# GianniLunardi/VBOC

Hardware: AMD Instinct MI355X
Metric: VBOC boundary OCP solves/sec, triple pendulum, 1/2/4/8 MI355X (higher is better)
Workload: dtype f64

## Files before the change

vboc_amd/csrc/coop.h:

```cpp
#pragma once

#ifndef VBOC_NSF
#define VBOC_NSF 4
#endif
#ifndef VBOC_DF
#define VBOC_DF 2
#endif
#ifndef VBOC_NSV
#define VBOC_NSV 8
#endif
#ifndef VBOC_DV
#define VBOC_DV 6
#endif

namespace vboc {

typedef double dbl2 __attribute__((ext_vector_type(2)));
typedef double dbl4 __attribute__((ext_vector_type(4)));
typedef __attribute__((address_space(1))) dbl2 gdbl2;
typedef __attribute__((address_space(1))) void gvoid;
typedef __attribute__((address_space(3))) void lvoid;

__host__ __device__ constexpr int even_up(int v) { return (v + 1) & ~1; }
#ifndef VBOC_REC_ALIGN
#define VBOC_REC_ALIGN 2
#endif
__host__ __device__ constexpr int rec_up(int v) { return (v + VBOC_REC_ALIGN - 1) / VBOC_REC_ALIGN * VBOC_REC_ALIGN; }

template <int NQ>
struct WaveLayout {
  static constexpr int NX = 2 * NQ, NU = NQ, NZ = 3 * NQ, M0 = NQ + 1;
  static constexpr bool IN_FIRST = NQ <= 3;
  static constexpr int OA = 0, OB = OA + NX * NX, P0 = OB + NX * NU, OE = IN_FIRST ? P0 : P0 + 4 * NZ, OD = OE + NX,
                       ODA = OD + NZ, OZ = IN_FIRST ? ODA + NZ : P0, ODZ = OZ + NZ, OQL = ODZ + NZ, OQU = OQL + NZ,
                       OK = P0 + 6 * NZ + NX, OKF = OK + NU * NX,
                       OLR = IN_FIRST ? OKF + NU + NU * NQ : OKF + NU, OM = IN_FIRST ? OKF + NU : OLR + NU * NU,
                       OY = OKF + NU + NU * NU + NU * NQ, OPE = OY + NU * NQ, OC = OPE + NX,
                       OACL = OC + NX, OX = OACL + NX * NX, OU = OX + NX, OPI = OU + NU, OLL = OPI + NX,
                       OLU = OLL + NZ, OWPI = OLU + NZ, REC = rec_up(OWPI + NX);
  static_assert((IN_FIRST ? OQU : ODA) + NZ == OK, "the fields before K are A, B, e, D, DA, z, dz, lambda_l, lambda_u");
  static_assert(IN_FIRST ? (OM == OKF + NU && OLR == OM + NU * NQ && OY == OLR + NU * NU)
                         : (OLR == OKF + NU && OM == OLR + NU * NU && OY == OM + NU * NQ), "K, k_f, M / chol(Ru), Y");
  static constexpr int W_FAC = OC, W_FIN = even_up(ODA), W_FINV = even_up(ODA + NZ), LO_VEC = OPE, W_VEC = OX - OPE,
                       LO_FWD = OC, W_FWD = OX - OC, W_COS = even_up(OQU + NZ);
  static constexpr int P_FAC = (W_FAC + 127) / 128, P_VEC = (W_VEC + 127) / 128, P_FWD = (W_FWD + 127) / 128,
                       P_COS = (W_COS + 127) / 128;
  static constexpr int P_VMAX = P_VEC > P_FWD ? (P_VEC > P_COS ? P_VEC : P_COS) : (P_FWD > P_COS ? P_FWD : P_COS);
  static constexpr int RSF = NQ <= 3 ? 256 : 128 * P_FAC, NSF = VBOC_NSF, DF = VBOC_DF,
                       RSV = NQ <= 3 ? 128 : 128 * P_VMAX, NSV = VBOC_NSV, DV = VBOC_DV;
  static constexpr int RING_D = NSF * RSF > NSV * RSV ? NSF * RSF : NSV * RSV;
  static constexpr int S_CAP = 4;
  static constexpr int S_VEC = NQ <= 3 ? (64 / (W_VEC / 2) < S_CAP ? 64 / (W_VEC / 2) : S_CAP) : 1,
                       S_FWD = NQ <= 3 ? (64 / (W_FWD / 2) < S_CAP ? 64 / (W_FWD / 2) : S_CAP) : 1, SLACK = S_CAP;
  static_assert(NQ > 3 || (S_VEC * W_VEC <= RSV && S_FWD * W_FWD <= RSV && (NSV & (NSV - 1)) == 0),
                "grouped windows fit one ring slot");
  static_assert(OB % 2 == 0 && OZ % 2 == 0 && OD % 2 == 0 && OK % 2 == 0 && OPE % 2 == 0 && OC % 2 == 0 &&
                    OACL % 2 == 0 && OX % 2 == 0,
                "16-byte aligned field ranges");
  static_assert(W_FAC <= RSF && W_VEC <= RSV && W_FWD <= RSV && W_COS <= RSV, "ring windows fit their slots");
  static_assert(NSF >= DF + 2 && NSV >= DV + 2, "a slot is refilled >= 2 stages after its last read");
  static constexpr int RING = 0, F0 = RING + RING_D, LR0 = F0 + NX * M0, MM0 = LR0 + M0 * M0, Y0 = MM0 + M0 * NQ,
                       PE0 = Y0 + M0 * NQ, P = PE0 + NX, PA = P + NX * NX, PB = PA + NX * NX, APA = PB + NX * NU,
                       RU = APA + NX * NX, S = RU + NU * NU, PI = S + NU * NX, PV = PI + NX * NQ, DXV = PV + 2 * NX,
                       SC = DXV + 2 * NX, LINE = SC + NQ * NQ, ZERO = LINE + NQ, TRASH = ZERO + 16, PAR = TRASH + 64,
                       XS = even_up(PAR + Par<NQ>::COUNT);
  static_assert(M0 * NX <= NX * NX, "stage-0 B'P reuses the PA scratch");
  static constexpr size_t lds_bytes(int nmax) { return ((size_t)XS + (size_t)(nmax + 1) * NX) * sizeof(double); }
  static constexpr size_t region_doubles(int nmax) { return (size_t)REC * (nmax + 1 + SLACK); }
};

struct Dsc {
  int x1, sx1, y1, sy1, x2, sx2, y2, sy2, ini, d1, d2;
  unsigned rel;
  double sg;
};
enum : unsigned { RX1 = 1, RY1 = 2, RX2 = 4, RY2 = 8, RINI = 16, RD1 = 32, RD2 = 64 };

__device__ __forceinline__ double uni(double v) {
  const unsigned long long b = (unsigned long long)__double_as_longlong(v);
  const unsigned lo = __builtin_amdgcn_readfirstlane((unsigned)b);
  const unsigned hi = __builtin_amdgcn_readfirstlane((unsigned)(b >> 32));
  return __longlong_as_double((long long)(((unsigned long long)hi << 32) | lo));
}
__device__ __forceinline__ void vreg(double& v) { asm volatile("" : "+v"(v)); }
__device__ __forceinline__ double rdlane(double v, int lane) {
  const unsigned long long b = (unsigned long long)__double_as_longlong(v);
  const unsigned lo = __builtin_amdgcn_readlane((unsigned)b, lane);
  const unsigned hi = __builtin_amdgcn_readlane((unsigned)(b >> 32), lane);
  return __longlong_as_double((long long)(((unsigned long long)hi << 32) | lo));
}
__device__ __forceinline__ double dbl_of(unsigned hi, unsigned lo) {
  return __longlong_as_double((long long)(((unsigned long long)hi << 32) | lo));
}
template <bool P32>
__device__ __forceinline__ void wswap(double v, double& a, double& b) {
  const unsigned long long u = (unsigned long long)__double_as_longlong(v);
  const unsigned l = (unsigned)u, h = (unsigned)(u >> 32);
  if constexpr (P32) {
    const auto lo = __builtin_amdgcn_permlane32_swap(l, l, false, false);
    const auto hi = __builtin_amdgcn_permlane32_swap(h, h, false, false);
    a = dbl_of(hi[0], lo[0]); b = dbl_of(hi[1], lo[1]);
  } else {
    const auto lo = __builtin_amdgcn_permlane16_swap(l, l, false, false);
    const auto hi = __builtin_amdgcn_permlane16_swap(h, h, false, false);
    a = dbl_of(hi[0], lo[0]); b = dbl_of(hi[1], lo[1]);
  }
}
template <int CTRL>
__device__ __forceinline__ double dppd(double v) {
  const unsigned long long u = (unsigned long long)__double_as_longlong(v);
  const int l = __builtin_amdgcn_update_dpp(0, (int)(unsigned)u, CTRL, 0xF, 0xF, false);
  const int h = __builtin_amdgcn_update_dpp(0, (int)(unsigned)(u >> 32), CTRL, 0xF, 0xF, false);
  return dbl_of((unsigned)h, (unsigned)l);
}
template <class OP>
__device__ __forceinline__ double wred(double v, OP op) {
  double a, b;
  wswap<true>(v, a, b);
  v = op(a, b);
  wswap<false>(v, a, b);
  v = op(a, b);
  v = op(v, dppd<0x128>(v));
  v = op(v, dppd<0x124>(v));
  v = op(v, dppd<0x4E>(v));
  v = op(v, dppd<0xB1>(v));
  return uni(v);
}
__device__ __forceinline__ double wsum(double v) {
  return wred(v, [](double x, double y) { return x + y; });
}
__device__ __forceinline__ double wmaxd(double v) {
  return wred(v, [](double x, double y) { return fmax(x, y); });
}
__device__ __forceinline__ double wmind(double v) {
  return wred(v, [](double x, double y) { return fmin(x, y); });
}

__device__ __forceinline__ void lsync() {
  __builtin_amdgcn_fence(__ATOMIC_RELEASE, "wavefront");
  __builtin_amdgcn_wave_barrier();
  __builtin_amdgcn_fence(__ATOMIC_ACQUIRE, "wavefront");
}

template <int n>
__device__ __forceinline__ bool chol_inv(double (&A)[n * n], double (&id)[n]) {
  bool ok = true;
  UNR for (int j = 0; j < n; ++j) {
    double sj = A[j * n + j];
    UNR for (int k = 0; k < j; ++k) sj -= A[j * n + k] * A[j * n + k];
    ok = ok && (sj > 0.0);
    const double x = sj > 0.0 ? sj : 1.0;
    double r = __builtin_amdgcn_rsq(x);
    UNR for (int it = 0; it < 2; ++it) {
      const double e = fma(-(0.5 * x) * r, r, 0.5);
      r = fma(r, e, r);
    }
    A[j * n + j] = x * r;
    id[j] = r;
    UNR for (int i = j + 1; i < n; ++i) {
      double tt = A[i * n + j];
      UNR for (int k = 0; k < j; ++k) tt -= A[i * n + k] * A[j * n + k];
      A[i * n + j] = tt * r;
    }
  }
  return ok;
}
template <int n>
__device__ __forceinline__ void solve_inv(const double (&L)[n * n], const double (&id)[n], double (&b)[n]) {
  UNR for (int i = 0; i < n; ++i) {
    double tt = b[i];
    UNR for (int k = 0; k < i; ++k) tt -= L[i * n + k] * b[k];
    b[i] = tt * id[i];
  }
  UNR for (int i = n - 1; i >= 0; --i) {
    double tt = b[i];
    UNR for (int k = i + 1; k < n; ++k) tt -= L[k * n + i] * b[k];
    b[i] = tt * id[i];
  }
}

__device__ __forceinline__ void tri(int u, int& i, int& j) {
  i = 0;
  while ((i + 1) * (i + 2) / 2 <= u) ++i;
  j = u - i * (i + 1) / 2;
}

__device__ unsigned long long g_wave_prof[16];
#ifdef VBOC_COOP_PROF
#define CPROF_DECL unsigned long long cp0 = 0, cp1 = 0, cp2 = 0, cp3 = 0, cp4 = 0, cp5 = 0, cp6 = 0, cp7 = 0, cp8 = 0; \
  unsigned long long cp_t = __builtin_amdgcn_s_memtime();
#define CPROF(i) { const unsigned long long n_ = __builtin_amdgcn_s_memtime(); cp##i += n_ - cp_t; cp_t = n_; }
#define CPROF_FLUSH(sq, ip) if (t == 0) { atomicAdd(&g_wave_prof[0], cp0); atomicAdd(&g_wave_prof[1], cp1); \
  atomicAdd(&g_wave_prof[2], cp2); atomicAdd(&g_wave_prof[3], cp3); atomicAdd(&g_wave_prof[4], cp4); \
  atomicAdd(&g_wave_prof[5], cp5); atomicAdd(&g_wave_prof[6], cp6); atomicAdd(&g_wave_prof[7], cp7); \
  atomicAdd(&g_wave_prof[8], cp8); atomicAdd(&g_wave_prof[9], (unsigned long long)(sq)); \
  atomicAdd(&g_wave_prof[10], (unsigned long long)(ip)); }
#else
#define CPROF_DECL
#define CPROF(i)
#define CPROF_FLUSH(sq, ip)
#endif
#if defined(VBOC_COOP_PROF) && defined(VBOC_PROF_SPLIT)
#define SPROF_DECL(P) unsigned long long sp0 = 0, sp1 = 0, sp2 = 0, sp3 = 0, sp4 = 0, sp_t = 0; \
  constexpr bool sp_on = (VBOC_PROF_SPLIT == (P)); if (sp_on) sp_t = __builtin_amdgcn_s_memtime();
#define SPROF(i) if (sp_on) { const unsigned long long n_ = __builtin_amdgcn_s_memtime(); sp##i += n_ - sp_t; sp_t = n_; }
#define SPROF_FLUSH if (sp_on && t == 0) { atomicAdd(&g_wave_prof[11], sp0); atomicAdd(&g_wave_prof[12], sp1); \
  atomicAdd(&g_wave_prof[13], sp2); atomicAdd(&g_wave_prof[14], sp3); atomicAdd(&g_wave_prof[15], sp4); }
#else
#define SPROF_DECL(P)
#define SPROF(i)
#define SPROF_FLUSH
#endif
#ifndef VBOC_REPEAT
#define VBOC_REPEAT 0
#endif

#define VREP(id, stmt) do { stmt; if constexpr (VBOC_REPEAT == (id)) { stmt; } } while (0)

#ifndef VBOC_FUSE
#define VBOC_FUSE 31
#endif

template <int NQ, bool FM = false, bool HC = false>
struct Coop {
  using L = WaveLayout<NQ>;
  using HL = Lane<NQ>;
  static_assert(!HC || (!FM && NQ >= 2 && NQ <= 3), "path constraint: pendulum chains, VALU factorisation");
  using PF = Par<NQ>;
  static constexpr int NX = 2 * NQ, NU = NQ, NZ = 3 * NQ, M0 = NQ + 1, REC = L::REC;
  static constexpr bool FUSE_OK = FM && NQ <= 3 && !HC;
  static constexpr bool FAC1 = FUSE_OK && (VBOC_FUSE & 1), PFUSE = FUSE_OK && (VBOC_FUSE & 2),
                        CCORR = FUSE_OK && (VBOC_FUSE & 4), KFM = FUSE_OK && (VBOC_FUSE & 8);
  static constexpr int OA = L::OA, OB = L::OB, OZ = L::OZ, ODZ = L::ODZ, OQL = L::OQL, OQU = L::OQU,
                       OE = L::OE, OK = L::OK, OKF = L::OKF, OLR = L::OLR, OM = L::OM, OY = L::OY,
                       OPE = L::OPE, OD = L::OD, ODA = L::ODA, OC = L::OC, OACL = L::OACL, OX = L::OX, OU = L::OU,
                       OPI = L::OPI,
                       OLL = L::OLL, OLU = L::OLU, OWPI = L::OWPI;

  double* s;
  gdouble* g;
  const Work& w;
  const Opts& o;
  int t;
  int N;
  double rs, rd0, e00, mu, nbox;

  unsigned lds0;
  gdouble* gh = nullptr;
  int pause_at = -1;

  __device__ Coop(double* s_, gdouble* g_, const Work& w_, const Opts& o_, int t_)
      : s(s_), g(g_), w(w_), o(o_), t(t_), N(0),
        lds0((unsigned)__builtin_amdgcn_readfirstlane((int)(unsigned)(size_t)(lvoid*)s_)) {}

  __device__ __forceinline__ void fresh() { asm volatile("" : "+v"(t)); }

  __device__ __forceinline__ gdouble& st(int k, int off) const { return g[(long long)k * REC + off]; }
  __device__ __forceinline__ gdouble& hcr(int k, int f) const { return gh[(long long)k * HL::FHC + f]; }
  __device__ __forceinline__ bool hc_on(int k) const { return HC && k >= 1 && k < N; }
  __device__ __forceinline__ double hc_eval(const double* x, double* grad) const {
    constexpr double l = Chain<NQ>::l;
    double X = 0.0, Y = 0.0;
    UNR for (int j = 0; j < NQ; ++j) { X += l * sin(x[j]); Y += l * cos(x[j]); }
    const double dx = X - o.hxc, dy = Y - o.hyc;
    if (grad) {
      UNR for (int j = 0; j < NQ; ++j) grad[j] = 2.0 * dx * (l * cos(x[j])) - 2.0 * dy * (l * sin(x[j]));
    }
    return dx * dx + dy * dy;
  }
  template <bool CORR>
  __device__ __forceinline__ void hc_dir(int k, const double* d, double smu, double& dtl, double& dtu, double& dql,
                                         double& dqu) const {
    double cd = 0.0;
    UNR for (int j = 0; j < NQ; ++j) cd += hcr(k, HL::HG + j) * d[j];
    const double htl = hcr(k, HL::HTL), htu = hcr(k, HL::HTU), hql = hcr(k, HL::HQL), hqu = hcr(k, HL::HQU);
    const double rl = rs * hcr(k, HL::HR0L), ru = rs * hcr(k, HL::HR0U);
    const double rcl = CORR ? smu - htl * hql - hcr(k, HL::HATL) * hcr(k, HL::HAQL) : -htl * hql;
    const double rcu = CORR ? smu - htu * hqu - hcr(k, HL::HATU) * hcr(k, HL::HAQU) : -htu * hqu;
    dtl = cd + rl;
    dtu = ru - cd;
    dql = (rcl - hql * dtl) / htl;
    dqu = (rcu - hqu * dtu) / htu;
  }
  __device__ __forceinline__ double& par(int f) const { return s[L::PAR + f]; }
  __device__ __forceinline__ static constexpr int fslot(int slot) { return L::RING + slot * L::RSF; }
  __device__ __forceinline__ static constexpr int vslot(int slot) { return L::RING + slot * L::RSV; }

  template <int TAG>
  __device__ __forceinline__ void dma(int k, int lo, int W, int dst, int part) const {
    const int nc = W / 2;
    const int c = part * 64 + t < nc ? part * 64 + t : nc - 1;
    const gdouble* src = g + (long long)k * REC + lo + 2 * c;
    const unsigned lds = lds0 + 8u * (unsigned)(dst + part * 128);
    unsigned keep;
    asm volatile("s_mov_b32 %0, m0\n\ts_mov_b32 m0, %2\n\ts_nop 0\n\tglobal_load_lds_dwordx4 %1, off\n\ts_mov_b32 m0, %0"
                 : "=&s"(keep)
                 : "v"(src), "s"(lds)
                 : "memory");
  }
  __device__ __forceinline__ void dma_s(const gdouble* base, unsigned voff, int dst) const {
    const unsigned lds = lds0 + 8u * (unsigned)dst;
    const unsigned long long b = (unsigned long long)(size_t)base;
    const unsigned long long bs = ((unsigned long long)(unsigned)__builtin_amdgcn_readfirstlane((int)(unsigned)(b >> 32)) << 32) |
                                  (unsigned)__builtin_amdgcn_readfirstlane((int)(unsigned)b);
    unsigned keep;
    asm volatile("s_mov_b32 %0, m0\n\ts_mov_b32 m0, %3\n\ts_nop 4\n\tglobal_load_lds_dwordx4 %1, %2\n\t"
                 "s_mov_b32 m0, %0"
                 : "=&s"(keep)
                 : "v"(voff), "s"(bs), "s"(lds)
                 : "memory");
  }
  template <int LO, int W, int S>
  __device__ __forceinline__ unsigned grp_off() const {
    constexpr int CH = W / 2;
    const int u = t / CH < S ? t / CH : S - 1;
    const int c = t - u * CH < CH ? t - u * CH : CH - 1;
    return 8u * (unsigned)(u * REC + LO + 2 * c);
  }
  template <int N>
  __device__ __forceinline__ static void vmwait() {
    asm volatile("s_waitcnt vmcnt(%0)" ::"n"(N) : "memory");
  }
  __device__ __forceinline__ static void settle() {
    __builtin_amdgcn_s_waitcnt(0x0F70);
  }
  template <int LO, int HI>
  __device__ __forceinline__ void ring_wb(int slot, int k) const {
    static_assert((HI - LO) / 2 <= 64 && LO % 2 == 0, "one 16-B chunk per lane");
    const dbl2* src = (const dbl2*)(s + fslot(slot));
    gdbl2* dst = (gdbl2*)(g + (long long)k * REC);
    if constexpr (NQ <= 3) {
      constexpr int NCH = (HI - LO) / 2;
      const int c = t < NCH ? t : NCH - 1;
      dst[LO / 2 + c] = src[LO / 2 + c];
      return;
    }
    if (t < (HI - LO) / 2) dst[LO / 2 + t] = src[LO / 2 + t];
  }


  __device__ __forceinline__ bool box(int k, int i, double& lb, double& ub) const {
    lb = -1.0; ub = 1.0;
    if (k == 0) {
      if (i == 0) { lb = par(PF::SLB); ub = par(PF::SUB); return true; }
      if (i < M0) { lb = par(PF::ULB + i - 1); ub = par(PF::UUB + i - 1); return true; }
      return false;
    }
    if (k == N) {
      if (i < NQ) { lb = par(PF::QNLB + i); ub = par(PF::QNUB + i); return true; }
      return false;
    }
    if (i < NX) { lb = par(PF::XLB + i); ub = par(PF::XUB + i); }
    else { lb = par(PF::ULB + i - NX); ub = par(PF::UUB + i - NX); }
    return true;
  }
  __device__ __forceinline__ double dz_init(double lb, double ub, double z) const {
    const double Lo = lb - z, U = ub - z, del = o.push * (U - Lo);
    return fmin(fmax(0.0, Lo + del), U - del);
  }
  __device__ __forceinline__ double cgrad(int k, int i) const { return (k == 0 && i == 0) ? par(PF::CS) : 0.0; }

  template <int LO, int C>
  __device__ __forceinline__ void ldr(int k, double (&d)[2 * C]) const {
    static_assert(LO % 2 == 0, "16-byte aligned range");
    const gdbl2* src = (const gdbl2*)(g + (long long)k * REC + LO);
    UNR for (int c = 0; c < C; ++c) {
      const dbl2 v = src[c];
      d[2 * c] = v.x;
      d[2 * c + 1] = v.y;
    }
  }
  static constexpr int NIP = (4 * NZ + 1) / 2;
  struct IP { double v[2 * NIP]; };
  __device__ __forceinline__ void ld_ip(int k, IP& r) const { ldr<OZ, NIP>(k, r.v); }
  template <int LO, int CNT, bool WIDE = !L::IN_FIRST>
  struct Cov {
    static_assert(LO >= OD && LO + CNT <= OD + 2 * NZ, "a part of the D / DA slots");
    static constexpr int B = WIDE ? OD : (LO & ~1), OFF = LO - B, C = WIDE ? (2 * NZ + 1) / 2 : (OFF + CNT + 1) / 2;
    double v[2 * C];
  };
  template <int LO, int CNT>
  __device__ __forceinline__ void ldc(int k, Cov<LO, CNT>& c) const { ldr<Cov<LO, CNT>::B, Cov<LO, CNT>::C>(k, c.v); }

  struct CS { double tl, tu, itl, itu, ql, qu, dz; bool bx; };
  __device__ __forceinline__ CS comp_r(const IP& r, int k, int i) const {
    CS c;
    double lb, ub;
    c.bx = box(k, i, lb, ub);
    const double z = r.v[i];
    c.dz = r.v[NZ + i]; c.ql = r.v[2 * NZ + i]; c.qu = r.v[3 * NZ + i];
    c.tl = c.dz - (lb - z); c.tu = (ub - z) - c.dz;
    c.itl = c.bx ? 1.0 / c.tl : 0.0;
    c.itu = c.bx ? 1.0 / c.tu : 0.0;
    return c;
  }
  __device__ __forceinline__ CS comp(int k, int i) const {
    CS c;
    double lb, ub;
    c.bx = box(k, i, lb, ub);
    const double z = st(k, OZ + i);
    c.dz = st(k, ODZ + i); c.ql = st(k, OQL + i); c.qu = st(k, OQU + i);
    c.tl = c.dz - (lb - z); c.tu = (ub - z) - c.dz;
    c.itl = c.bx ? 1.0 / c.tl : 0.0;
    c.itu = c.bx ? 1.0 / c.tu : 0.0;
    return c;
  }
  __device__ __forceinline__ static void corr_rhs(const CS& c, double da, double smu, double& rl, double& ru) {
    const double dlla = -c.ql - c.ql * da * c.itl, dlua = -c.qu + c.qu * da * c.itu;
    rl = smu - c.tl * c.ql - da * dlla;
    ru = smu - c.tu * c.qu + da * dlua;
  }

  __device__ __forceinline__ void dnull(Dsc& d) const {
    d.x1 = d.y1 = d.x2 = d.y2 = d.ini = L::ZERO;
    d.sx1 = d.sy1 = d.sx2 = d.sy2 = 0;
    d.d1 = d.d2 = L::TRASH + t;
    d.rel = 0;
    d.sg = 1.0;
  }
  static constexpr int TXC = NX * (NX + 1) / 2, TUC = NU * (NU + 1) / 2, TMC = M0 * (M0 + 1) / 2;
  static constexpr int imax(int a, int b) { return a > b ? a : b; }
  static constexpr int OUTMAX =
      imax(imax(imax(NX * NX + NX * NU + NX + NQ, TXC + TUC + NU * NX + NU * NQ), imax(TXC + NX * NQ + NQ * NQ,
                                                                                      M0 * NX + M0 * NQ + NX + NQ)),
           imax(TMC, NQ * NQ));
  static constexpr int RD = (OUTMAX + 63) / 64;

  template <int L1, int L2, int R>
  __device__ __forceinline__ void dstep(const Dsc (&dd)[R], int kb) const {
    double res[R];
    UNR for (int rr = 0; rr < R; ++rr) {
      const Dsc& d = dd[rr];
      auto ad = [&](int a, unsigned bit) { return a + ((d.rel & bit) ? kb : 0); };
      const int x1 = ad(d.x1, RX1), y1 = ad(d.y1, RY1), x2 = ad(d.x2, RX2), y2 = ad(d.y2, RY2);
      double a1[L1 > 0 ? L1 : 1], b1[L1 > 0 ? L1 : 1], a2[L2 > 0 ? L2 : 1], b2[L2 > 0 ? L2 : 1];
      UNR for (int q = 0; q < L1; ++q) { a1[q] = s[x1 + q * d.sx1]; b1[q] = s[y1 + q * d.sy1]; }
      UNR for (int q = 0; q < L2; ++q) { a2[q] = s[x2 + q * d.sx2]; b2[q] = s[y2 + q * d.sy2]; }
      const double r0 = s[ad(d.ini, RINI)];
      __builtin_amdgcn_sched_barrier(0);
      double s1 = 0.0, s2 = 0.0;
      UNR for (int q = 0; q < L1; ++q) s1 += a1[q] * b1[q];
      UNR for (int q = 0; q < L2; ++q) s2 += a2[q] * b2[q];
      res[rr] = r0 + d.sg * s1 + s2;
    }
    lsync();
    UNR for (int rr = 0; rr < R; ++rr) {
      const Dsc& d = dd[rr];
      auto ad = [&](int a, unsigned bit) { return a + ((d.rel & bit) ? kb : 0); };
      s[ad(d.d1, RD1)] = res[rr];
      s[ad(d.d2, RD2)] = res[rr];
    }
    lsync();
  }
  template <int n>
  __device__ __forceinline__ bool sstep(int ru, int ldst, int rb, int rstr, int db, int dstr, double sgn) const {
    double Lm[n * n], id[n], b[n];
    UNR for (int a = 0; a < n; ++a) b[a] = s[rb + a * rstr];
    UNR for (int e = 0; e < n * n; ++e) Lm[e] = s[ru + e];
    const bool ok = chol_inv<n>(Lm, id);
    solve_inv<n>(Lm, id, b);
    lsync();
    UNR for (int a = 0; a < n; ++a) s[db + a * dstr] = sgn * b[a];
    if (t == 0) {
      UNR for (int e = 0; e < n * n; ++e) s[ldst + e] = Lm[e];
    }
    lsync();
    return ok;
  }

  __device__ __forceinline__ void desc_mid(Dsc (&dd1)[RD], Dsc (&dd2)[RD], Dsc (&dd4)[RD]) const {
    UNR for (int rr = 0; rr < RD; ++rr) desc_mid1(dd1[rr], dd2[rr], dd4[rr], t + 64 * rr);
  }
  __device__ __forceinline__ void desc_mid1(Dsc& d1, Dsc& d2, Dsc& d4, const int lane) const {
    constexpr int P = L::P, PA = L::PA, PB = L::PB, APA = L::APA, RU = L::RU, S = L::S, PI = L::PI, SC = L::SC,
                  LINE = L::LINE;
    constexpr int TX = NX * (NX + 1) / 2, TU = NU * (NU + 1) / 2;
    dnull(d1); dnull(d2); dnull(d4);
    int u = lane;
    if (u < NX * NX) {
      const int i = u / NX, j = u % NX;
      d1.x1 = P + i * NX; d1.sx1 = 1; d1.y1 = OA + j; d1.sy1 = NX; d1.rel = RY1; d1.d1 = d1.d2 = PA + u;
    } else if ((u -= NX * NX) < NX * NU) {
      const int i = u / NU, a = u % NU;
      d1.x1 = P + i * NX; d1.sx1 = 1; d1.y1 = OB + a; d1.sy1 = NU; d1.rel = RY1; d1.d1 = d1.d2 = PB + u;
    } else if ((u -= NX * NU) < NX) {
      d1.x1 = P + u * NX; d1.sx1 = 1; d1.y1 = OE; d1.sy1 = 1; d1.sg = rs; d1.d1 = d1.d2 = OPE + u;
      d1.rel = RY1 | RD1 | RD2;
    } else if ((u -= NX) < NQ) {
      d1.x1 = PI + u; d1.sx1 = NQ; d1.y1 = OE; d1.sy1 = 1; d1.sg = rs; d1.ini = d1.d1 = d1.d2 = LINE + u; d1.rel = RY1;
    }
    u = lane;
    if (u < TX) {
      int i, j;
      tri(u, i, j);
      d2.x1 = OA + i; d2.sx1 = NX; d2.y1 = PA + j; d2.sy1 = NX; d2.rel = RX1;
      if (HC && i < NQ && j < NQ) { d2.ini = OK + i * NQ + j; d2.rel |= RINI; }
      else if (i == j) { d2.ini = OD + i; d2.rel |= RINI; }
      d2.d1 = APA + i * NX + j; d2.d2 = APA + j * NX + i;
    } else if ((u -= TX) < TU) {
      int a, c;
      tri(u, a, c);
      d2.x1 = OB + a; d2.sx1 = NU; d2.y1 = PB + c; d2.sy1 = NU; d2.rel = RX1;
      if (a == c) { d2.ini = OD + NX + a; d2.rel |= RINI; }
      d2.d1 = RU + a * NU + c; d2.d2 = RU + c * NU + a;
    } else if ((u -= TU) < NU * NX) {
      const int a = u / NX, j = u % NX;
      d2.x1 = PB + a; d2.sx1 = NU; d2.y1 = OA + j; d2.sy1 = NX; d2.rel = RY1; d2.d1 = d2.d2 = S + u;
    } else if ((u -= NU * NX) < NU * NQ) {
      const int a = u / NQ, j = u % NQ;
      d2.x1 = OB + a; d2.sx1 = NU; d2.y1 = PI + j; d2.sy1 = NQ; d2.rel = RX1 | RD1 | RD2; d2.d1 = d2.d2 = OY + u;
    }
    u = lane;
    if (u < TX) {
      int i, j;
      tri(u, i, j);
      d4.x2 = S + i; d4.sx2 = NX; d4.y2 = OK + j; d4.sy2 = NX; d4.rel = RY2;
      d4.ini = APA + i * NX + j; d4.d1 = P + i * NX + j; d4.d2 = P + j * NX + i;
    } else if ((u -= TX) < NX * NQ) {
      const int i = u / NQ, j = u % NQ;
      d4.x1 = OA + i; d4.sx1 = NX; d4.y1 = PI + j; d4.sy1 = NQ;
      d4.x2 = OK + i; d4.sx2 = NX; d4.y2 = OY + j; d4.sy2 = NQ;
      d4.rel = RX1 | RX2 | RY2; d4.d1 = d4.d2 = PI + u;
    } else if ((u -= NX * NQ) < NQ * NQ) {
      const int i = u / NQ, j = u % NQ;
      d4.x2 = OY + i; d4.sx2 = NQ; d4.y2 = OM + j; d4.sy2 = NQ; d4.rel = RX2 | RY2;
      d4.ini = d4.d1 = d4.d2 = SC + u;
    }
  }
// ... 121 lines not shown
        }
        UNR for (int a = 0; a < NU; ++a) uk[a] = rec[OU + a];
        rk4_sens<NQ>(h, xk, uk, x1, [&](int i, int c, double v) {
          if (c < NX) rec[OA + i * NX + c] = v;
          else rec[OB + i * NU + (c - NX)] = v;
        });
        UNR for (int i = 0; i < NX; ++i) {
          const double b = x1[i] - st(k + 1, OX + i);
          rec[OE + i] = b;
          eq = fmax(eq, fabs(b));
        }
        if (k == 0) {
          rec[OZ] = sv;
          UNR for (int a = 0; a < NU; ++a) rec[OZ + 1 + a] = uk[a];
          UNR for (int i = M0; i < NZ; ++i) rec[OZ + i] = 0.0;
        } else {
          UNR for (int i = 0; i < NX; ++i) rec[OZ + i] = xk[i];
          UNR for (int a = 0; a < NU; ++a) rec[OZ + NX + a] = uk[a];
        }
        double pik[NX];
        UNR for (int i = 0; i < NX; ++i) pik[i] = rec[OPI + i];
        if (k == 0) {
          double F[NX * M0];
          UNR for (int i = 0; i < NX; ++i) {
            double tt = 0.0;
            UNR for (int j = 0; j < NQ; ++j) tt += rec[OA + i * NX + NQ + j] * par(PF::DIR + j);
            F[i * M0] = tt;
            UNR for (int a = 0; a < NU; ++a) F[i * M0 + 1 + a] = rec[OB + i * NU + a];
          }
          UNR for (int e = 0; e < NX * M0; ++e) s[L::F0 + e] = F[e];
          UNR for (int c = 0; c < M0; ++c) {
            double gr = (c == 0 ? par(PF::CS) : 0.0) - rec[OLL + c] + rec[OLU + c];
            UNR for (int r = 0; r < NX; ++r) gr += F[r * M0 + c] * pik[r];
            stt = fmax(stt, fabs(gr));
          }
        } else {
          double pprev[NX];
          UNR for (int i = 0; i < NX; ++i) pprev[i] = st(k - 1, OPI + i);
          double hg[NQ], hmul = 0.0;
          if constexpr (HC) {
            const double hv = hc_eval(xk, hg);
            hcr(k, HL::HV) = hv;
            UNR for (int j = 0; j < NQ; ++j) hcr(k, HL::HG + j) = hg[j];
            const double hll = hcr(k, HL::HLL), hlu = hcr(k, HL::HLU);
            hmul = hlu - hll;
            inq = fmax(inq, fmax(o.hlh - hv, hv - o.huh));
            cp = fmax(cp, fmax(fabs(hll * (hv - o.hlh)), fabs(hlu * (o.huh - hv))));
          }
          UNR for (int c = 0; c < NZ; ++c) {
            double gr = -rec[OLL + c] + rec[OLU + c];
            if (c < NX) {
              UNR for (int r = 0; r < NX; ++r) gr += rec[OA + r * NX + c] * pik[r];
              gr -= pprev[c];
              if constexpr (HC) {
                if (c < NQ) gr += hg[c < NQ ? c : 0] * hmul;
              }
            } else {
              UNR for (int r = 0; r < NX; ++r) gr += rec[OB + r * NU + (c - NX)] * pik[r];
            }
            stt = fmax(stt, fabs(gr));
          }
        }
        UNR for (int c = 0; c < NZ; ++c) {
          double lb, ub;
          if (!box(k, c, lb, ub)) continue;
          const double z = rec[OZ + c], ll = rec[OLL + c], lu = rec[OLU + c];
          inq = fmax(inq, fmax(lb - z, z - ub));
          cp = fmax(cp, fmax(fabs(ll * (z - lb)), fabs(lu * (ub - z))));
        }
      } else {
        UNR for (int i = 0; i < NX; ++i) rec[OZ + i] = rec[OX + i];
        UNR for (int i = NX; i < NZ; ++i) rec[OZ + i] = 0.0;
        UNR for (int c = 0; c < NX; ++c) {
          const double z = rec[OX + c];
          double gr = -rec[OLL + c] + rec[OLU + c] - st(N - 1, OPI + c);
          if (c >= NQ) {
            gr += par(PF::NU_ + c - NQ);
            eq = fmax(eq, fabs(z - par(PF::VFIN + c - NQ)));
          }
          stt = fmax(stt, fabs(gr));
          if (c < NQ) {
            const double lb = par(PF::QNLB + c), ub = par(PF::QNUB + c);
            const double ll = rec[OLL + c], lu = rec[OLU + c];
            inq = fmax(inq, fmax(lb - z, z - ub));
            cp = fmax(cp, fmax(fabs(ll * (z - lb)), fabs(lu * (ub - z))));
          }
        }
      }
    }
    rstat = wmaxd(stt); req = wmaxd(eq); rineq = wmaxd(inq); rcomp = wmaxd(cp);
    __syncthreads();
  }

  __device__ __forceinline__ void qp_init() {
    fresh();
    double musum = 0.0, nb = 0.0, rd = 0.0, e0 = 0.0;
    for (int k = t; k <= N; k += 64) {
      gdouble* rec = &g[(long long)k * REC];
      double dz[NZ];
      UNR for (int i = 0; i < NZ; ++i) {
        double lb, ub, ql = 0.0, qu = 0.0, d0 = 0.0;
        if (box(k, i, lb, ub)) {
          const double z = rec[OZ + i], Lo = lb - z, U = ub - z;
          d0 = dz_init(lb, ub, z);
          ql = o.mu0 / (d0 - Lo);
          qu = o.mu0 / (U - d0);
          musum += o.mu0 + o.mu0;
          nb += 2.0;
        }
        dz[i] = d0;
        rec[ODZ + i] = d0; rec[OQL + i] = ql; rec[OQU + i] = qu;
        if (!(HC && i < NQ && k >= 1 && k < N)) rd = fmax(rd, fabs(o.lm * d0 + cgrad(k, i) - ql + qu));
      }
      if constexpr (HC) {
        if (hc_on(k)) {
          double hg[NQ], gd = 0.0;
          UNR for (int j = 0; j < NQ; ++j) { hg[j] = hcr(k, HL::HG + j); gd += hg[j] * dz[j]; }
          const double hv = hcr(k, HL::HV), Lh = o.hlh - hv, Uh = o.huh - hv;
          const double tl = fmax(gd - Lh, o.push), tu = fmax(Uh - gd, o.push);
          const double ql = o.mu0 / tl, qu = o.mu0 / tu;
          const double r0l = gd - Lh - tl, r0u = Uh - gd - tu;
          hcr(k, HL::HTL) = tl; hcr(k, HL::HTU) = tu; hcr(k, HL::HQL) = ql; hcr(k, HL::HQU) = qu;
          hcr(k, HL::HR0L) = r0l; hcr(k, HL::HR0U) = r0u;
          musum += tl * ql + tu * qu;
          nb += 2.0;
          e0 = fmax(e0, fmax(fabs(r0l), fabs(r0u)));
          UNR for (int i = 0; i < NQ; ++i)
            rd = fmax(rd, fabs(o.lm * dz[i] + cgrad(k, i) - rec[OQL + i] + rec[OQU + i] + hg[i] * (qu - ql)));
        }
      }
      if (k < N) {
        const gdouble* rn = &g[(long long)(k + 1) * REC];
        UNR for (int i = 0; i < NX; ++i) {
          double lb, ub, dn = 0.0;
          if (box(k + 1, i, lb, ub)) dn = dz_init(lb, ub, rn[OZ + i]);
          double tt = rec[OE + i] - dn;
          if (k == 0) {
            UNR for (int a = 0; a < M0; ++a) tt += s[L::F0 + i * M0 + a] * dz[a];
          } else {
            UNR for (int q = 0; q < NX; ++q) tt += rec[OA + i * NX + q] * dz[q];
            UNR for (int a = 0; a < NU; ++a) tt += rec[OB + i * NU + a] * dz[NX + a];
          }
          rec[OE + i] = tt;
          e0 = fmax(e0, fabs(tt));
        }
      } else {
        UNR for (int j = 0; j < NQ; ++j) {
          const double e = par(PF::VFIN + j) - rec[OZ + NQ + j] - dz[NQ + j];
          par(PF::E0N + j) = e;
          e0 = fmax(e0, fabs(e));
          par(PF::QNU + j) = 0.0;
        }
      }
    }
    nbox = wsum(nb);
    mu = wsum(musum) / nbox;
    rd0 = wmaxd(rd);
    e00 = wmaxd(e0);
    rs = 1.0;
    __syncthreads();
  }

  __device__ __forceinline__ int qp_check() const {
    if (!isfinite(mu)) return -1;
    if (mu < o.qp_tol_comp && rs * rd0 < o.qp_tol_stat && rs * e00 < o.qp_tol_eq) return 0;
    return 1;
  }

  __device__ __forceinline__ void prep_from(const IP& r, int k, gdouble* rec) const {
    UNR for (int i = 0; i < NZ; ++i) {
      const CS c = comp_r(r, k, i);
      rec[OD + i] = o.lm + (c.bx ? c.ql * c.itl + c.qu * c.itu : 0.0);
      rec[ODA + i] = o.lm * c.dz + cgrad(k, i);
    }
  }
  __device__ __forceinline__ void prep_pred() {
    fresh();
    for (int k = t; k <= N; k += 64) {
      IP r;
      ld_ip(k, r);
      __builtin_amdgcn_sched_barrier(0);
      gdouble* rec = &g[(long long)k * REC];
      prep_from(r, k, rec);
      if constexpr (HC) {
        if (hc_on(k)) {
          const double htl = hcr(k, HL::HTL), htu = hcr(k, HL::HTU), hql = hcr(k, HL::HQL), hqu = hcr(k, HL::HQU);
          const double sig = hql / htl + hqu / htu;
          const double gam = hql * (rs * hcr(k, HL::HR0L)) / htl - hqu * (rs * hcr(k, HL::HR0U)) / htu;
          double hg[NQ];
          UNR for (int j = 0; j < NQ; ++j) hg[j] = hcr(k, HL::HG + j);
          UNR for (int i = 0; i < NQ; ++i) {
            UNR for (int j = 0; j < NQ; ++j)
              rec[OK + i * NQ + j] = (i == j ? (double)rec[OD + i] : 0.0) + sig * hg[i] * hg[j];
            rec[ODA + i] += hg[i] * gam;
          }
        }
      }
    }
    __syncthreads();
  }
  __device__ __forceinline__ void prep_corr(double smu) {
    fresh();
    for (int k = t; k <= N; k += 64) {
      IP r;
      Cov<ODA, NZ> da;
      ld_ip(k, r);
      ldc(k, da);
      __builtin_amdgcn_sched_barrier(0);
      gdouble* rec = &g[(long long)k * REC];
      double gv[NZ];
      UNR for (int i = 0; i < NZ; ++i) {
        const CS c = comp_r(r, k, i);
        double gg = o.lm * c.dz + cgrad(k, i);
        if (c.bx) {
          double rl, ru;
          corr_rhs(c, da.v[da.OFF + i], smu, rl, ru);
          gg += -c.ql - rl * c.itl + c.qu + ru * c.itu;
        }
        rec[OD + i] = gg;
        gv[i] = gg;
      }
      if constexpr (CCORR) {
        if (k >= 1 && k < N) vec_const(k, gv);
      }
      if constexpr (HC) {
        if (hc_on(k)) {
          const double htl = hcr(k, HL::HTL), htu = hcr(k, HL::HTU), hql = hcr(k, HL::HQL), hqu = hcr(k, HL::HQU);
          const double rl = rs * hcr(k, HL::HR0L), ru = rs * hcr(k, HL::HR0U);
          const double rcl = smu - htl * hql - hcr(k, HL::HATL) * hcr(k, HL::HAQL);
          const double rcu = smu - htu * hqu - hcr(k, HL::HATU) * hcr(k, HL::HAQU);
          const double gam = -hql + hqu - (rcl - hql * rl) / htl + (rcu - hqu * ru) / htu;
          UNR for (int j = 0; j < NQ; ++j) rec[OD + j] += hcr(k, HL::HG + j) * gam;
        }
      }
    }
    __syncthreads();
  }

  __device__ __forceinline__ bool factor() {
    fresh();
    for (int e = t; e < NX * NX; e += 64) {
      const int i = e / NX, j = e % NX;
      s[L::P + e] = (i == j) ? (double)st(N, OD + i) : 0.0;
    }
    for (int e = t; e < NX * NQ; e += 64) {
      const int i = e / NQ, j = e % NQ;
      s[L::PI + e] = (i == NQ + j) ? 1.0 : 0.0;
    }
    for (int e = t; e < NQ * NQ; e += 64) s[L::SC + e] = 0.0;
    if (t < NQ) s[L::LINE + t] = 0.0;
    constexpr int P = L::P_FAC;
    auto fdma = [&](int j) {
      const int kk = N - 1 - j >= 0 ? N - 1 - j : 0;
      UNR for (int part = 0; part < P; ++part) dma<1>(kk, 0, L::W_FAC, fslot(j % L::NSF), part);
    };
    __syncthreads();
    settle();
    fdma(0);
    fdma(1);
    bool ok = true;
    Dsc d1[RD], d2[RD], d4[RD];
    desc_mid(d1, d2, d4);
    SPROF_DECL(1)
    for (int j = 0; j < N; ++j) {
      const int k = N - 1 - j, kb = fslot(j % L::NSF);
      if (j >= 1) ring_wb<OK, OC>((j - 1) % L::NSF, k + 1);
      fdma(j + 2);
      SPROF(4)
      vmwait<2 * P>();
      SPROF(3)
      if (k >= 1) {
        dstep<NX, 0>(d1, kb);
        SPROF(0)
        dstep<NX, 0>(d2, kb);
        SPROF(1)
        int rb = L::ZERO, rstr = 0, db = L::TRASH + t, dstr = 0;
        double sgn = 1.0;
        if (t < NX) { rb = L::S + t; rstr = NX; db = kb + OK + t; dstr = NX; sgn = -1.0; }
        else if (t < NX + NQ) { rb = kb + OY + (t - NX); rstr = NQ; db = kb + OM + (t - NX); dstr = NQ; }
        const bool okk = sstep<NU>(L::RU, kb + OLR, rb, rstr, db, dstr, sgn);
        ok = ok && okk;
        dstep<NX, NU>(d4, kb);
        SPROF(2)
      } else {
        Dsc z1[RD], z2[RD], z4[RD];
        desc_s0(z1, z2, z4);
        dstep<NX, 0>(z1, kb);
        dstep<NX, 0>(z2, kb);
        int rb = L::ZERO, rstr = 0, db = L::TRASH + t, dstr = 0;
        if (t < NQ) { rb = L::Y0 + t; rstr = NQ; db = L::MM0 + t; dstr = NQ; }
        const bool ok0 = sstep<M0>(L::LR0, L::LR0, rb, rstr, db, dstr, 1.0);
        ok = ok && ok0;
        dstep<0, M0>(z4, kb);
      }
      lsync();
      SPROF(4)
    }
    SPROF_FLUSH
    __syncthreads();
    return ok;
  }

  static constexpr int CE = NX + NU, CP = CE + 1;
#ifndef VBOC_ACL_FUSED_NQ
#define VBOC_ACL_FUSED_NQ (1 << 3)
#endif
  static constexpr bool ACL_FUSED = FM && ((VBOC_ACL_FUSED_NQ >> NQ) & 1);
  static constexpr int FJUNK = L::OX;
  static constexpr bool MFMA_OK = (NX <= 8) && (CP + NQ <= 16) && (FJUNK + 2 * NX + 2 <= L::RSF);
  static constexpr int HR0 = NX >> 2;
#ifndef VBOC_RINV
#define VBOC_RINV 1
#endif
  static constexpr bool RINV = VBOC_RINV && FM && NU == 3;
  static constexpr bool VFUSE = FAC1 && ACL_FUSED && RINV && (VBOC_FUSE & 16);
  static_assert(!VFUSE || (L::W_FINV <= OK && L::W_FINV <= 128), "VFUSE: A .. DA in one LDS-DMA, in front of the outputs");
  static_assert(((NX + NU - 1) >> 2) <= HR0 + 1, "H_u spans two accumulator registers");
  __device__ __forceinline__ static constexpr int hrow(int row) { return (row & 3) + 4 * ((row >> 2) - HR0); }
  __device__ __forceinline__ void acl_slot(int sl) {
    const int kb = fslot(sl);
    const int tt = t < NX * NX ? t : NX * NX - 1;
    const int q = tt / NX, i = tt - q * NX;
    double av = s[kb + OA + q * NX + i], bv[NU], kv[NU];
    UNR for (int c = 0; c < NU; ++c) { bv[c] = s[kb + OB + q * NU + c]; kv[c] = s[kb + OK + c * NX + i]; }
    __builtin_amdgcn_sched_barrier(0);
    UNR for (int c = 0; c < NU; ++c) av += bv[c] * kv[c];
    s[kb + OACL + tt] = av;
  }

  __device__ __forceinline__ bool factor_mfma() {
    static_assert(MFMA_OK, "stage blocks fit one 16x16 FP64 MFMA tile");
    fresh();
#if defined(VBOC_PROF_SPLIT) && VBOC_PROF_SPLIT == 5
    constexpr int FSPL = 5;
#else
    constexpr int FSPL = 4;
#endif
#define FS4(i) if constexpr (FSPL == 4) { SPROF(i) }
#define FS5(i) if constexpr (FSPL == 5) { SPROF(i) }
    SPROF_DECL(FSPL)
    const int c = t & 15, g = t >> 4;
    constexpr int HS = L::XS;
    dbl4 Dm;
    UNR for (int r = 0; r < 4; ++r) {
      const int row = g + 4 * r;
      double v = 0.0;
      if (row < NX && c == row) v = st(N, OD + row);
      if (row < NX && c >= CP && c < CP + NQ && row == NQ + (c - CP)) v = 1.0;
      Dm[r] = v;
    }
    constexpr int WF = VFUSE ? L::W_FINV : (FAC1 ? L::W_FIN : L::W_FAC), P = (WF + 127) / 128;
    static_assert(!FAC1 || P == 1, "the factorisation's inputs fit one LDS-DMA");
    auto fdma = [&](int j) {
      const int kk = N - 1 - j >= 0 ? N - 1 - j : 0;
      UNR for (int part = 0; part < P; ++part) dma<1>(kk, 0, WF, fslot(j % L::NSF), part);
    };
    int goff[2], gb[2];
    double gm[2];
    UNR for (int q = 0; q < 2; ++q) {
      const int row = 4 * q + g;
      int off = L::ZERO, b = 0;
      double m = 0.0;
      if (row < NX) {
        if (c < NX) { off = OA + row * NX + c; m = 1.0; b = 1; }
        else if (c < CE) { off = OB + row * NU + (c - NX); m = 1.0; b = 1; }
        else if (c == CE) { off = OE + row; m = rs; b = 1; }
      }
      goff[q] = off;
      gb[q] = b;
      gm[q] = m;
    }
    const int hoff = c < CE ? OD + c : L::ZERO, hb = c < CE ? 1 : 0;
    double hm[4], cm[4];
    UNR for (int r = 0; r < 4; ++r) {
      const int row = g + 4 * r;
      hm[r] = (c < CE && row == c) ? 1.0 : 0.0;
      cm[r] = (c >= CP && c < CP + NQ && (row == CE || (row >= CP && row < CP + NQ))) ? 1.0 : 0.0;
    }
    const double pim = (c >= CP && c < CP + NQ) ? 1.0 : 0.0;
    const bool zc = c < NX || (c >= CP && c < CP + NQ);
    double zm[NU];
    UNR for (int a = 0; a < NU; ++a) zm[a] = (zc && g == a) ? 1.0 : 0.0;
    const int kofs = (g == 0 && c < NX) ? OK + c : FJUNK;
    const int mofs = (g == 0 && c >= CP && c < CP + NQ) ? OM + (c - CP) : FJUNK;
    const int pofs = (c == CE) ? OPE + g : FJUNK;
    int yofs = FJUNK, ysrc = HS;
    if (t < NU * NQ) {
      const int a = t / NQ, jj = t % NQ, row = NX + a;
      yofs = OY + t;
      ysrc = HS + hrow(row) * 16 + CP + jj;
    }
    __syncthreads();
    settle();
    fdma(0);
    fdma(1);
    bool ok = true;
    double pcur = 0.0, kfv = 0.0;
    const int kfo = t < NU ? OKF + t : FJUNK;
    if constexpr (VFUSE) pcur = st(N, ODA + (t < NX ? t : NX - 1));
    auto vstep = [&](int sl) {
      const int kb = fslot(sl);
      const int i = t < NX ? t : NX - 1, a = t < NU ? t : NU - 1;
      double gu[NU], kk[NU], lr[NU], ac[NX], pe[NX], bb[NX];
      const double gx = s[kb + ODA + i], gua = s[kb + ODA + NX + a];
      UNR for (int q = 0; q < NU; ++q) {
        gu[q] = s[kb + ODA + NX + q];
        kk[q] = s[kb + OK + q * NX + i];
        lr[q] = s[kb + OLR + a * NU + q];
      }
      UNR for (int q = 0; q < NX; ++q) {
        ac[q] = s[kb + OACL + q * NX + i];
        pe[q] = s[kb + OPE + q];
        bb[q] = s[kb + OB + q * NU + a];
      }
      double pv[NX];
      UNR for (int q = 0; q < NX; ++q) pv[q] = rdlane(pcur, q);
      double c = gx;
      UNR for (int q = 0; q < NU; ++q) c += kk[q] * gu[q];
      UNR for (int q = 0; q < NX; ++q) c += ac[q] * pe[q];
      double p0 = c, p1 = 0.0;
      UNR for (int q = 0; q < NX; q += 2) p0 += ac[q] * pv[q];
      UNR for (int q = 1; q < NX; q += 2) p1 += ac[q] * pv[q];
      double x = gua;
      UNR for (int q = 0; q < NX; ++q) x += bb[q] * (pe[q] + pv[q]);
      double kf = 0.0;
      UNR for (int b = 0; b < NU; ++b) kf += lr[b] * rdlane(x, b);
      kfv = -kf;
      pcur = p0 + p1;
    };
    auto wb_prev = [&](int j, int k) {
      if constexpr (VFUSE) {
        acl_slot((j - 1) % L::NSF);
        vstep((j - 1) % L::NSF);
      } else if constexpr (ACL_FUSED) {
        acl_slot((j - 1) % L::NSF);
        ring_wb<OK, L::OX>((j - 1) % L::NSF, k + 1);
      } else {
        ring_wb<OK, OC>((j - 1) % L::NSF, k + 1);
      }
    };
    for (int j = 0; j < N - 1; ++j) {
      const int k = N - 1 - j, kb = fslot(j % L::NSF);
      if (j >= 1) wb_prev(j, k);
      FS5(0)
      fdma(j + 2);
      FS5(1)
      vmwait<2 * P>();
      FS4(0)
      FS5(2)
      const double r0 = s[kb * gb[0] + goff[0]], r1 = s[kb * gb[1] + goff[1]], hv = s[kb * hb + hoff];
      double g0 = r0 * gm[0], g1 = r1 * gm[1];
      vreg(g0);
      vreg(g1);
      double p0 = Dm[0], p1 = Dm[1];
      vreg(p0);
      vreg(p1);
      dbl4 pg = {0.0, 0.0, 0.0, 0.0};
      pg = __builtin_amdgcn_mfma_f64_16x16x4f64(p0, g0, pg, 0, 0, 0);
      pg = __builtin_amdgcn_mfma_f64_16x16x4f64(p1, g1, pg, 0, 0, 0);
      dbl4 h = {0.0, 0.0, 0.0, 0.0};
      UNR for (int r = 0; r < 4; ++r) h[r] = fma(Dm[r], cm[r], hv * hm[r]);
      double b0 = fma(Dm[0], pim, pg[0]), b1 = fma(Dm[1], pim, pg[1]);
      vreg(b0);
      vreg(b1);
      h = __builtin_amdgcn_mfma_f64_16x16x4f64(g0, b0, h, 0, 0, 0);
      h = __builtin_amdgcn_mfma_f64_16x16x4f64(g1, b1, h, 0, 0, 0);
      FS4(1)
      s[HS + g * 16 + c] = h[HR0];
      if (HR0 + 1 < 4) s[HS + (4 + g) * 16 + c] = h[HR0 + 1 < 4 ? HR0 + 1 : 3];
      double Lm[NU * NU], id[NU], hu[NU];
      UNR for (int a = 0; a < NU; ++a) {
        const int ia = hrow(NX + a);
        UNR for (int b = 0; b <= a; ++b) {
          const double v = s[HS + ia * 16 + NX + b];
          Lm[a * NU + b] = v;
          Lm[b * NU + a] = v;
        }
        hu[a] = s[HS + ia * 16 + c];
      }
      const double yv = s[ysrc];
      double w[NU];
      if constexpr (RINV) {
        const double a = Lm[0], b = Lm[1], c = Lm[2], d = Lm[4], e = Lm[5], f = Lm[8];
        const double c00 = d * f - e * e, c01 = c * e - b * f, c02 = b * e - c * d;
        const double c11 = a * f - c * c, c12 = b * c - a * e, c22 = a * d - b * b;
        const double det = a * c00 + b * c01 + c * c02;
        ok = ok && (a > 0.0) && (c22 > 0.0) && (det > 0.0);
        double r = __builtin_amdgcn_rcp(det);
        UNR for (int it = 0; it < 2; ++it) r = fma(r, fma(-det, r, 1.0), r);
        Lm[0] = c00 * r; Lm[1] = Lm[3] = c01 * r; Lm[2] = Lm[6] = c02 * r;
        Lm[4] = c11 * r; Lm[5] = Lm[7] = c12 * r; Lm[8] = c22 * r;
        UNR for (int i = 0; i < NU; ++i) w[i] = Lm[i * NU] * hu[0] + Lm[i * NU + 1] * hu[1] + Lm[i * NU + 2] * hu[2];
        double zs = 0.0, ws = 0.0;
        UNR for (int i = 0; i < NU; ++i) { zs = fma(hu[i], zm[i], zs); ws = fma(w[i], zm[i], ws); }
        double nz = -zs;
        vreg(ws);
        vreg(nz);
        Dm = __builtin_amdgcn_mfma_f64_16x16x4f64(nz, ws, h, 0, 0, 0);
      } else {
      const bool okk = chol_inv<NU>(Lm, id);
      ok = ok && okk;
      double z[NU], zs = 0.0;
      UNR for (int a = 0; a < NU; ++a) {
        double tt = hu[a];
        UNR for (int b = 0; b < a; ++b) tt -= Lm[a * NU + b] * z[b];
        z[a] = tt * id[a];
        zs = fma(z[a], zm[a], zs);
      }
      double nz = -zs;
      vreg(zs);
      vreg(nz);
      Dm = __builtin_amdgcn_mfma_f64_16x16x4f64(nz, zs, h, 0, 0, 0);
      UNR for (int a = NU - 1; a >= 0; --a) {
        double tt = z[a];
        UNR for (int b = a + 1; b < NU; ++b) tt -= Lm[b * NU + a] * w[b];
        w[a] = tt * id[a];
      }
      }
      asm volatile("" : "+v"(Dm));
      FS4(2)
      UNR for (int a = 0; a < NU; ++a) {
        s[kb + kofs + a * NX] = -w[a];
        s[kb + mofs + a * NQ] = w[a];
      }
      UNR for (int e = 0; e < NU * NU; ++e) s[kb + OLR + e] = Lm[e];
      s[kb + yofs] = yv;
      s[kb + pofs] = pg[0];
      s[kb + pofs + 4] = pg[1];
      if constexpr (VFUSE) {
        if (j >= 1) {
          s[fslot((j - 1) % L::NSF) + kfo] = kfv;
          ring_wb<OK, L::OX>((j - 1) % L::NSF, k + 1);
        }
      }
      lsync();
      FS4(3)
      FS5(3)
    }
    UNR for (int r = 0; r < 4; ++r) {
      const int row = g + 4 * r;
      if (row < NX && c < NX) s[L::P + row * NX + c] = Dm[r];
      if (row < NX && c >= CP && c < CP + NQ) s[L::PI + row * NQ + (c - CP)] = Dm[r];
      if (row >= CP && row < CP + NQ && c >= CP && c < CP + NQ) s[L::SC + (row - CP) * NQ + (c - CP)] = -Dm[r];
      if (row == CE && c >= CP && c < CP + NQ) s[L::LINE + (c - CP)] = Dm[r];
    }
    lsync();
    {
      const int j = N - 1, kb = fslot(j % L::NSF);
      if (j >= 1) {
        if constexpr (VFUSE) {
          acl_slot((j - 1) % L::NSF);
          vstep((j - 1) % L::NSF);
          s[fslot((j - 1) % L::NSF) + kfo] = kfv;
          ring_wb<OK, L::OX>((j - 1) % L::NSF, 1);
        } else if constexpr (ACL_FUSED) {
          acl_slot((j - 1) % L::NSF);
          ring_wb<OK, L::OX>((j - 1) % L::NSF, 1);
        } else {
          ring_wb<OK, OC>((j - 1) % L::NSF, 1);
        }
      }
      if constexpr (VFUSE) {
        if (t < NX) s[L::PV + t] = pcur;
      }
      vmwait<0>();
      Dsc z1[RD], z2[RD], z4[RD];
      desc_s0(z1, z2, z4);
      dstep<NX, 0>(z1, kb);
      dstep<NX, 0>(z2, kb);
      int rb = L::ZERO, rstr = 0, db = L::TRASH + t, dstr = 0;
      if (t < NQ) { rb = L::Y0 + t; rstr = NQ; db = L::MM0 + t; dstr = NQ; }
      const bool ok0 = sstep<M0>(L::LR0, L::LR0, rb, rstr, db, dstr, 1.0);
      ok = ok && ok0;
      dstep<0, M0>(z4, kb);
      lsync();
    }
    __syncthreads();
    SPROF(4)
    SPROF_FLUSH
#undef FS4
#undef FS5
    return ok;
  }

  __device__ __forceinline__ void acl_pass() {
    fresh();
    constexpr int NAB = (NX * NX + NX * NU) / 2, NKK = (NU * NX) / 2;
    for (int k = 1 + t; k < N; k += 64) {
      double ab[2 * NAB], kk[2 * NKK];
      ldr<OA, NAB>(k, ab);
      ldr<OK, NKK>(k, kk);
      __builtin_amdgcn_sched_barrier(0);
      gdbl2* dst = (gdbl2*)(g + (long long)k * REC + OACL);
      UNR for (int e = 0; e < NX * NX; e += 2) {
        double v[2];
        UNR for (int h2 = 0; h2 < 2; ++h2) {
          const int q = (e + h2) / NX, i = (e + h2) % NX;
          double a = ab[q * NX + i];
          UNR for (int c = 0; c < NU; ++c) a += ab[NX * NX + q * NU + c] * kk[c * NX + i];
          v[h2] = a;
        }
        dbl2 vv;
        vv.x = v[0];
        vv.y = v[1];
        dst[e / 2] = vv;
      }
    }
    __syncthreads();
  }

  __device__ __forceinline__ void vec_const(int k, const double* gv) const {
    constexpr int NKK = (NU * NX) / 2;
    double kk[2 * NKK], ac[NX * NX], pe[NX];
    ldr<OK, NKK>(k, kk);
    ldr<OACL, NX * NX / 2>(k, ac);
    ldr<OPE, NX / 2>(k, pe);
    gdbl2* dst = (gdbl2*)(g + (long long)k * REC + OC);
    double cv[NX];
    UNR for (int i = 0; i < NX; ++i) {
      double c = gv[i];
      UNR for (int q = 0; q < NU; ++q) c += kk[q * NX + i] * gv[NX + q];
      UNR for (int q = 0; q < NX; ++q) c += ac[q * NX + i] * pe[q];
      cv[i] = c;
    }
    UNR for (int i = 0; i < NX; i += 2) {
      dbl2 vv;
      vv.x = cv[i];
      vv.y = cv[i + 1];
      dst[i / 2] = vv;
    }
  }
  template <int OG, bool PRE = true, bool SWEPT = false>
  __device__ __forceinline__ bool vec(double (&w0)[M0], double (&nun)[NQ]) {
    fresh();
    SPROF_DECL(2)
    if constexpr (PRE && !SWEPT) {
      constexpr int NKK = (NU * NX) / 2;
      for (int k = 1 + t; k < N; k += 64) {
        Cov<OG, NZ> gg;
        double kk[2 * NKK], ac[NX * NX], pe[NX];
        ldc(k, gg);
        ldr<OK, NKK>(k, kk);
        ldr<OACL, NX * NX / 2>(k, ac);
        ldr<OPE, NX / 2>(k, pe);
        __builtin_amdgcn_sched_barrier(0);
        constexpr int go = Cov<OG, NZ>::OFF;
        gdbl2* dst = (gdbl2*)(g + (long long)k * REC + OC);
        double cv[NX];
        UNR for (int i = 0; i < NX; ++i) {
          double c = gg.v[go + i];
          UNR for (int q = 0; q < NU; ++q) c += kk[q * NX + i] * gg.v[go + NX + q];
          UNR for (int q = 0; q < NX; ++q) c += ac[q * NX + i] * pe[q];
          cv[i] = c;
        }
        UNR for (int i = 0; i < NX; i += 2) {
          dbl2 vv;
          vv.x = cv[i];
          vv.y = cv[i + 1];
          dst[i / 2] = vv;
        }
      }
      __syncthreads();
    }
    SPROF(0)
    if constexpr (!SWEPT) {
    double pcur = st(N, OG + (t < NX ? t : NX - 1));
    if (t < NX) s[L::PV + t] = pcur;
    const int cnt = N - 1;
    __syncthreads();
    if constexpr (L::S_VEC > 1) {
      constexpr int S = L::S_VEC, W = L::W_VEC;
      const int ng = (cnt + S - 1) / S;
      const unsigned voff = grp_off<L::LO_VEC, W, S>();
      auto gdma = [&](int j) {
        const int G = ng - 1 - j >= 0 ? ng - 1 - j : 0;
        dma_s(g + (long long)(1 + G * S) * REC, voff, vslot(j & (L::NSV - 1)));
      };
      const int i = t < NX ? t : NX - 1;
      const int xm = t < NX ? NX : 0, xb = t < NX ? L::XS + t : L::TRASH + t;
      double pv[NX];
      UNR for (int q = 0; q < NX; ++q) pv[q] = rdlane(pcur, q);
      settle();
      if (ng >= 1) {
        UNR for (int d = 0; d < L::DV; ++d) gdma(d);
      }
      for (int j = 0; j < ng; ++j) {
        const int G = ng - 1 - j;
        gdma(j + L::DV);
        double acl[S][NX], cc[S], pe[S];
        vmwait<L::DV>();
        const int kb = vslot(j & (L::NSV - 1));
        UNR for (int u = 0; u < S; ++u) {
          UNR for (int q = 0; q < NX; ++q) acl[u][q] = s[kb + u * W + (OACL - OPE) + q * NX + i];
          cc[u] = s[kb + u * W + (OC - OPE) + i];
          pe[u] = s[kb + u * W + i];
        }
        __builtin_amdgcn_sched_barrier(0);
        UNR for (int u = S - 1; u >= 0; --u) {
          const int k = 1 + G * S + u;
          if (k > cnt) continue;
          double p0 = cc[u], p1 = 0.0;
          UNR for (int q = 0; q < NX; q += 2) p0 += acl[u][q] * pv[q];
          UNR for (int q = 1; q < NX; q += 2) p1 += acl[u][q] * pv[q];
          s[xb + k * xm] = pe[u] + pcur;
          pcur = p0 + p1;
          UNR for (int q = 0; q < NX; ++q) pv[q] = rdlane(pcur, q);
        }
      }
    } else {
    constexpr int PV = L::P_VEC;
    auto vdma = [&](int j) {
      const int kk = N - 1 - j >= 1 ? N - 1 - j : 1;
      UNR for (int part = 0; part < PV; ++part) dma<2>(kk, L::LO_VEC, L::W_VEC, vslot(j % L::NSV), part);
    };
    auto vld = [&](int kb, double (&acl)[NX], double& cc, double& pe) {
      const int i = t < NX ? t : NX - 1;
      UNR for (int q = 0; q < NX; ++q) acl[q] = s[kb + (OACL - OPE) + q * NX + i];
      cc = s[kb + (OC - OPE) + i];
      pe = s[kb + i];
    };
    double acl[NX], cc = 0.0, pe = 0.0;
    settle();
    if (cnt >= 1) {
      UNR for (int d = 0; d < L::DV; ++d) vdma(d);
      vmwait<(L::DV - 1) * PV>();
      vld(vslot(0), acl, cc, pe);
    }
    double pv[NX];
    UNR for (int q = 0; q < NX; ++q) pv[q] = rdlane(pcur, q);
    for (int j = 0; j < cnt; ++j) {
      const int k = N - 1 - j;
      vdma(j + L::DV);
      vmwait<(L::DV - 1) * PV>();
      double an[NX], cn, pn;
      vld(vslot((j + 1) % L::NSV), an, cn, pn);
      __builtin_amdgcn_sched_barrier(0);
      double p0 = cc, p1 = 0.0;
      UNR for (int q = 0; q < NX; q += 2) p0 += acl[q] * pv[q];
      UNR for (int q = 1; q < NX; q += 2) p1 += acl[q] * pv[q];
      if (t < NX) s[L::XS + k * NX + t] = pe + pcur;
      pcur = p0 + p1;
      UNR for (int q = 0; q < NX; ++q) pv[q] = rdlane(pcur, q);
      UNR for (int q = 0; q < NX; ++q) acl[q] = an[q];
      cc = cn;
      pe = pn;
    }
    }
    if (t < NX) s[L::PV + t] = pcur;
    __syncthreads();
    }
    SPROF(1)
    double lin[NQ];
    UNR for (int j = 0; j < NQ; ++j) lin[j] = 0.0;
    constexpr int NBB = (NX * NU + 1) / 2, NLY = (OPE - (OLR & ~1) + 1) / 2;
    if constexpr (SWEPT) {
      constexpr int F0_ = OKF & ~1, NF = (OKF + NU - F0_ + 1) / 2, Y0_ = OY & ~1, NY = (OPE - Y0_ + 1) / 2;
      for (int k = 1 + t; k < N; k += 64) {
        double kf[2 * NF], yy[2 * NY];
        ldr<F0_, NF>(k, kf);
        ldr<Y0_, NY>(k, yy);
        __builtin_amdgcn_sched_barrier(0);
        UNR for (int j = 0; j < NQ; ++j)
          UNR for (int a = 0; a < NU; ++a) lin[j] += yy[(OY - Y0_) + a * NQ + j] * kf[(OKF - F0_) + a];
      }
    } else
    for (int k = 1 + t; k < N; k += 64) {
      double bb[2 * NBB], ly[2 * NLY];
      Cov<OG + NX, NU> gg;
      ldr<OB, NBB>(k, bb);
      ldr<(OLR & ~1), NLY>(k, ly);
      ldc(k, gg);
      __builtin_amdgcn_sched_barrier(0);
      constexpr int LR_ = OLR - (OLR & ~1), Y_ = OY - (OLR & ~1);
      double r[NU], Lm[NU * NU];
      UNR for (int a = 0; a < NU; ++a) {
        double x = gg.v[gg.OFF + a];
        UNR for (int i = 0; i < NX; ++i) x += bb[i * NU + a] * s[L::XS + k * NX + i];
        r[a] = x;
      }
      UNR for (int e = 0; e < NU * NU; ++e) Lm[e] = ly[LR_ + e];
      if constexpr (RINV) {
        double q[NU];
        UNR for (int a = 0; a < NU; ++a) {
          q[a] = 0.0;
          UNR for (int b = 0; b < NU; ++b) q[a] += Lm[a * NU + b] * r[b];
        }
        UNR for (int a = 0; a < NU; ++a) r[a] = q[a];
      } else {
        chol_solve<NU>(Lm, r);
      }
      UNR for (int a = 0; a < NU; ++a) {
        r[a] = -r[a];
        st(k, OKF + a) = r[a];
      }
      UNR for (int j = 0; j < NQ; ++j)
        UNR for (int a = 0; a < NU; ++a) lin[j] += ly[Y_ + a * NQ + j] * r[a];
    }
    UNR for (int j = 0; j < NQ; ++j) lin[j] = wsum(lin[j]);
    SPROF(2)
    {
      double v[NX], Lm[M0 * M0];
      UNR for (int i = 0; i < NX; ++i) v[i] = s[L::PE0 + i] + s[L::PV + i];
      UNR for (int a = 0; a < M0; ++a) {
        double x = st(0, OG + a);
        UNR for (int i = 0; i < NX; ++i) x += s[L::F0 + i * M0 + a] * v[i];
        w0[a] = x;
      }
      UNR for (int e = 0; e < M0 * M0; ++e) Lm[e] = s[L::LR0 + e];
      chol_solve<M0>(Lm, w0);
      UNR for (int a = 0; a < M0; ++a) w0[a] = -w0[a];
      UNR for (int j = 0; j < NQ; ++j)
        UNR for (int a = 0; a < M0; ++a) lin[j] += s[L::Y0 + a * NQ + j] * w0[a];
    }
    double Sl[NQ * NQ];
    UNR for (int e = 0; e < NQ * NQ; ++e) Sl[e] = s[L::SC + e];
    const bool ok = chol<NQ>(Sl);
    UNR for (int j = 0; j < NQ; ++j) nun[j] = lin[j] + s[L::LINE + j] - rs * par(PF::E0N + j);
    chol_solve<NQ>(Sl, nun);
    __syncthreads();
    SPROF(3)
    SPROF_FLUSH
    return ok;
  }

  template <bool CORR>
  __device__ __forceinline__ void fwd(const double (&w0in)[M0], const double (&nun)[NQ], double smu, double& amax, double& c0,
                      double& c1, double& c2) {
    fresh();
    constexpr int OT = CORR ? OD : ODA;
#if defined(VBOC_PROF_SPLIT) && VBOC_PROF_SPLIT == 6
    constexpr int WSPL = 6;
#else
    constexpr int WSPL = 3;
#endif
#define W3(i) if constexpr (WSPL == 3) { SPROF(i) }
#define W6(i) if constexpr (WSPL == 6) { SPROF(i) }
    SPROF_DECL(WSPL)
    {
      double w0[M0];
      UNR for (int a = 0; a < M0; ++a) {
        double x = w0in[a];
        UNR for (int j = 0; j < NQ; ++j) x -= s[L::MM0 + a * NQ + j] * nun[j];
        w0[a] = x;
      }
      if (t == 0) {
        UNR for (int i = 0; i < NZ; ++i) st(0, OT + i) = i < M0 ? w0[i < M0 ? i : 0] : 0.0;

      }
      if (t < NX) {
        double x = rs * st(0, OE + t);
        UNR for (int a = 0; a < M0; ++a) x += s[L::F0 + t * M0 + a] * w0[a];
        s[L::XS + NX + t] = x;
        s[L::DXV + t] = x;
      }
    }
    W3(0)
    {
      constexpr int NBB = (NX * NU + 1) / 2, NFM = (OM + NU * NQ - OKF + 1) / 2;
      for (int k = 1 + t; k < N; k += 64) {
        double e[NX], bb[2 * NBB], fm[2 * NFM];
        ldr<OE, NX / 2>(k, e);
        ldr<OB, NBB>(k, bb);
        ldr<OKF, NFM>(k, fm);
        __builtin_amdgcn_sched_barrier(0);
        double kfm[NU];
        UNR for (int a = 0; a < NU; ++a) {
          double x = fm[a];
          UNR for (int j = 0; j < NQ; ++j) x -= fm[(OM - OKF) + a * NQ + j] * nun[j];
          kfm[a] = x;
        }
        if constexpr (KFM) {
          UNR for (int a = 0; a < NU; ++a) st(k, OKF + a) = kfm[a];
        }
        gdbl2* dst = (gdbl2*)(g + (long long)k * REC + OC);
        UNR for (int i = 0; i < NX; i += 2) {
          double v[2];
          UNR for (int h2 = 0; h2 < 2; ++h2) {
            double c = rs * e[i + h2];
            UNR for (int a = 0; a < NU; ++a) c += bb[(i + h2) * NU + a] * kfm[a];
            v[h2] = c;
          }
          dbl2 vv;
          vv.x = v[0];
          vv.y = v[1];
          dst[i / 2] = vv;
        }
      }
      __syncthreads();
    }
    W3(1)
    const int cnt = N - 1;
    __syncthreads();
    if constexpr (L::S_FWD > 1) {
      constexpr int S = L::S_FWD, W = L::W_FWD;
      const int ng = (cnt + S - 1) / S;
      const unsigned voff = grp_off<L::LO_FWD, W, S>();
      auto gdma = [&](int j) {
        const int G = j < ng ? j : ng - 1;
        dma_s(g + (long long)(1 + G * S) * REC, voff, vslot(j & (L::NSV - 1)));
      };
      const int i = t < NX ? t : NX - 1;
      const int xm = t < NX ? NX : 0, xb = t < NX ? L::XS + NX + t : L::TRASH + t;
      double dx[NX];
      UNR for (int q = 0; q < NX; ++q) dx[q] = s[L::DXV + q];
      settle();
      if (ng >= 1) {
        UNR for (int d = 0; d < L::DV; ++d) gdma(d);
      }
      for (int j = 0; j < ng; ++j) {
        gdma(j + L::DV);
        double acl[S][NX], cc[S];
        vmwait<L::DV>();
        const int kb = vslot(j & (L::NSV - 1));
        UNR for (int u = 0; u < S; ++u) {
          UNR for (int q = 0; q < NX; ++q) acl[u][q] = s[kb + u * W + (OACL - OC) + i * NX + q];
          cc[u] = s[kb + u * W + i];
        }
        __builtin_amdgcn_sched_barrier(0);
        UNR for (int u = 0; u < S; ++u) {
          const int k = 1 + j * S + u;
          if (k > cnt) break;
          double p0 = cc[u], p1 = 0.0;
          UNR for (int q = 0; q < NX; q += 2) p0 += acl[u][q] * dx[q];
          UNR for (int q = 1; q < NX; q += 2) p1 += acl[u][q] * dx[q];
          const double dn = p0 + p1;
          s[xb + k * xm] = dn;
          UNR for (int q = 0; q < NX; ++q) dx[q] = rdlane(dn, q);
        }
      }
    } else {
    constexpr int PW = L::P_FWD;
    auto wdma = [&](int j) {
      const int kk = 1 + j < N ? 1 + j : N - 1;
      UNR for (int part = 0; part < PW; ++part) dma<4>(kk, L::LO_FWD, L::W_FWD, vslot(j % L::NSV), part);
    };
    auto fld = [&](int kb, double (&acl)[NX], double& cc) {
      const int i = t < NX ? t : NX - 1;
      UNR for (int q = 0; q < NX; ++q) acl[q] = s[kb + (OACL - OC) + i * NX + q];
      cc = s[kb + i];
    };
    {
      double acl[NX], cc = 0.0;
      settle();
      if (cnt >= 1) {
        UNR for (int d = 0; d < L::DV; ++d) wdma(d);
        vmwait<(L::DV - 1) * PW>();
        fld(vslot(0), acl, cc);
      }
      double dx[NX];
      UNR for (int q = 0; q < NX; ++q) dx[q] = s[L::DXV + q];
      for (int j = 0; j < cnt; ++j) {
        const int k = 1 + j;
        wdma(j + L::DV);
        vmwait<(L::DV - 1) * PW>();
        double an[NX], cn;
        fld(vslot((j + 1) % L::NSV), an, cn);
        __builtin_amdgcn_sched_barrier(0);
        double p0 = cc, p1 = 0.0;
        UNR for (int q = 0; q < NX; q += 2) p0 += acl[q] * dx[q];
        UNR for (int q = 1; q < NX; q += 2) p1 += acl[q] * dx[q];
        const double dn = p0 + p1;
        if (t < NX) s[L::XS + (k + 1) * NX + t] = dn;
        UNR for (int q = 0; q < NX; ++q) dx[q] = rdlane(dn, q);
        UNR for (int q = 0; q < NX; ++q) acl[q] = an[q];
        cc = cn;
      }
    }
    }
    __syncthreads();
    W3(2)
    W6(4)
    typename Lane<NQ>::MinRatio mr{1.0, CORR ? o.tau : 1.0};
    double a0 = 0.0, a1 = 0.0, a2 = 0.0;
    constexpr int NKM = KFM ? (OKF + NU - OK + 1) / 2 : (OY - OK + 1) / 2;
    for (int k = t; k <= N; k += 64) {
      IP r;
      double km[2 * NKM];
      Cov<ODA, NZ> da;
      const int kk = (k > 0 && k < N) ? k : 1 < N ? 1 : 0;
      ld_ip(k, r);
      ldr<OK, NKM>(kk, km);
      if (CORR) ldc(k, da);
      __builtin_amdgcn_sched_barrier(0);
      W6(0)
      gdouble* rec = &g[(long long)k * REC];
      double d[NZ];
      if (k == 0) {
        UNR for (int i = 0; i < NZ; ++i) d[i] = rec[OT + i];
      } else {
        UNR for (int i = 0; i < NX; ++i) d[i] = s[L::XS + k * NX + i];
        UNR for (int a = 0; a < NU; ++a) {
          double x = 0.0;
          if (k < N) {
            x = km[OKF - OK + a];
            if constexpr (!KFM) {
              UNR for (int j = 0; j < NQ; ++j) x -= km[OM - OK + a * NQ + j] * nun[j];
            }
            UNR for (int i = 0; i < NX; ++i) x += km[a * NX + i] * d[i];
          }
          d[NX + a] = x;
        }
        UNR for (int i = 0; i < NZ; ++i) rec[OT + i] = d[i];
      }
      W6(1)
      UNR for (int i = 0; i < NZ; ++i) {
        const CS c = comp_r(r, k, i);
        if (!c.bx) continue;
        double dll, dlu;
        if (!CORR) {
          dll = -c.ql - c.ql * d[i] * c.itl;
          dlu = -c.qu + c.qu * d[i] * c.itu;
          a0 += c.tl * c.ql + c.tu * c.qu;
          a1 += c.tl * dll + d[i] * c.ql + c.tu * dlu - d[i] * c.qu;
          a2 += d[i] * dll - d[i] * dlu;
        } else {
          double rl, ru;
          corr_rhs(c, da.v[da.OFF + i], smu, rl, ru);
          dll = (rl - c.ql * d[i]) * c.itl;
          dlu = (ru + c.qu * d[i]) * c.itu;
        }
        mr.add(c.tl, d[i]);
        mr.add(c.tu, -d[i]);
        mr.add(c.ql, dll);
        mr.add(c.qu, dlu);
      }
      if constexpr (HC) {
        if (hc_on(k)) {
          double dtl, dtu, dql, dqu;
          hc_dir<CORR>(k, d, smu, dtl, dtu, dql, dqu);
          const double htl = hcr(k, HL::HTL), htu = hcr(k, HL::HTU), hql = hcr(k, HL::HQL), hqu = hcr(k, HL::HQU);
          if (!CORR) {
            hcr(k, HL::HATL) = dtl; hcr(k, HL::HATU) = dtu; hcr(k, HL::HAQL) = dql; hcr(k, HL::HAQU) = dqu;
            a0 += htl * hql + htu * hqu;
            a1 += htl * dql + dtl * hql + htu * dqu + dtu * hqu;
            a2 += dtl * dql + dtu * dqu;
          }
          mr.add(htl, dtl);
          mr.add(htu, dtu);
          mr.add(hql, dql);
          mr.add(hqu, dqu);
        }
      }
      W6(2)
    }
    amax = wmind(mr.value());
    c0 = wsum(a0); c1 = wsum(a1); c2 = wsum(a2);
    __syncthreads();
    W3(3)
    W6(3)
    SPROF_FLUSH
#undef W3
#undef W6
  }

  __device__ __forceinline__ void update(double alpha, double smu) {
    fresh();
    double musum = 0.0;
    for (int k = t; k <= N; k += 64) {
      IP r;
      double dd[2 * ((2 * NZ + 1) / 2)];
      ld_ip(k, r);
      ldr<OD, (2 * NZ + 1) / 2>(k, dd);
      __builtin_amdgcn_sched_barrier(0);
      gdouble* rec = &g[(long long)k * REC];
      IP rn;
      if constexpr (PFUSE) rn = r;
      UNR for (int i = 0; i < NZ; ++i) {
        const CS c = comp_r(r, k, i);
        const double d = dd[i];
        const double dzn = c.dz + alpha * d;
        rec[ODZ + i] = dzn;
        if constexpr (PFUSE) rn.v[NZ + i] = dzn;
        if (!c.bx) continue;
        double rl, ru;
        corr_rhs(c, dd[NZ + i], smu, rl, ru);
        const double dll = (rl - c.ql * d) * c.itl, dlu = (ru + c.qu * d) * c.itu;
        const double qln = c.ql + alpha * dll, qun = c.qu + alpha * dlu;
        rec[OQL + i] = qln;
        rec[OQU + i] = qun;
        if constexpr (PFUSE) { rn.v[2 * NZ + i] = qln; rn.v[3 * NZ + i] = qun; }
        musum += (c.tl + alpha * d) * qln + (c.tu - alpha * d) * qun;
      }
      if constexpr (PFUSE) prep_from(rn, k, rec);
      if constexpr (HC) {
        if (hc_on(k)) {
          double dtl, dtu, dql, dqu;
          hc_dir<true>(k, dd, smu, dtl, dtu, dql, dqu);
          const double tl = hcr(k, HL::HTL) + alpha * dtl, tu = hcr(k, HL::HTU) + alpha * dtu;
          const double ql = hcr(k, HL::HQL) + alpha * dql, qu = hcr(k, HL::HQU) + alpha * dqu;
          hcr(k, HL::HTL) = tl; hcr(k, HL::HTU) = tu; hcr(k, HL::HQL) = ql; hcr(k, HL::HQU) = qu;
          musum += tl * ql + tu * qu;
        }
      }
    }
    mu = wsum(musum) / nbox;
    __syncthreads();
  }

  __device__ __forceinline__ bool costate() {
    fresh();
    if constexpr (HC) {
      for (int k = 1 + t; k < N; k += 64) {
        const double m = hcr(k, HL::HQU) - hcr(k, HL::HQL);
        UNR for (int j = 0; j < NQ; ++j) st(k, OB + j) = hcr(k, HL::HG + j) * m;
      }
      __syncthreads();
    }
    bool fin = true;
    if (t < NX) {
      const int i = t;
      const double dz = st(N, ODZ + i);
      const double lam = o.lm * dz - st(N, OQL + i) + st(N, OQU + i) +
                         (i >= NQ ? par(PF::QNU + (i >= NQ ? i - NQ : 0)) : 0.0);
      s[L::XS + (N - 1) * NX + i] = lam;
      s[L::DXV + i] = lam;
      fin = isfinite(dz);
    }
    fin = __ballot(!fin) == 0ull;
    const int cnt = N - 1;
    __syncthreads();
    constexpr int PC = L::P_COS;
    auto cdma = [&](int j) {
      const int kk = N - 1 - j >= 1 ? N - 1 - j : 1;
      UNR for (int part = 0; part < PC; ++part) dma<8>(kk, 0, L::W_COS, vslot(j % L::NSV), part);
    };
    auto cterms = [&](int kb, double (&ac)[NX], double& cc) {
      const int i = t < NX ? t : NX - 1;
      cc = o.lm * s[kb + ODZ + i] - s[kb + OQL + i] + s[kb + OQU + i];
      if constexpr (HC) cc += i < NQ ? s[kb + OB + (i < NQ ? i : 0)] : 0.0;
      UNR for (int q = 0; q < NX; ++q) ac[q] = s[kb + OA + q * NX + i];
    };
    double ac[NX], cc = 0.0;
    settle();
    if (cnt >= 1) {
      UNR for (int d = 0; d < L::DV; ++d) cdma(d);
      vmwait<(L::DV - 1) * PC>();
      cterms(vslot(0), ac, cc);
    }
    for (int j = 0; j < cnt; ++j) {
      const int k = N - 1 - j;
      const int rb = L::DXV + (j & 1) * NX, wb = L::DXV + ((j + 1) & 1) * NX;
      cdma(j + L::DV);
      vmwait<(L::DV - 1) * PC>();
      double lam[NX], an[NX], cn;
      UNR for (int q = 0; q < NX; ++q) lam[q] = s[rb + q];
      cterms(vslot((j + 1) % L::NSV), an, cn);
      __builtin_amdgcn_sched_barrier(0);
      double p0 = cc, p1 = 0.0;
      UNR for (int q = 0; q < NX; q += 2) p0 += ac[q] * lam[q];
      UNR for (int q = 1; q < NX; q += 2) p1 += ac[q] * lam[q];
      const double x = p0 + p1;
      if (t < NX) {
        s[wb + t] = x;
        s[L::XS + (k - 1) * NX + t] = x;
      }
      UNR for (int q = 0; q < NX; ++q) ac[q] = an[q];
      cc = cn;
      lsync();
    }
    __syncthreads();
    for (int k = t; k < N; k += 64) {
      UNR for (int i = 0; i < NX; ++i) st(k, ODA + i) = s[L::XS + k * NX + i];
    }
    __syncthreads();
    return fin;
  }

  __device__ __forceinline__ void update_weights() {
    fresh();
    double lmax = 0.0;
    for (int k = t; k <= N; k += 64) {
      if (k < N) {
        UNR for (int i = 0; i < NX; ++i) st(k, OWPI + i) = Lane<NQ>::wupd(st(k, OWPI + i), st(k, ODA + i));
      }
      UNR for (int i = 0; i < NZ; ++i) lmax = fmax(lmax, fmax((double)st(k, OQL + i), (double)st(k, OQU + i)));
      if constexpr (HC) {
        if (hc_on(k)) lmax = fmax(lmax, fmax((double)hcr(k, HL::HQL), (double)hcr(k, HL::HQU)));
      }
    }
    lmax = wmaxd(lmax);
    if (t == 0) {
      UNR for (int j = 0; j < NQ; ++j) par(PF::WNU + j) = Lane<NQ>::wupd(par(PF::WNU + j), par(PF::QNU + j));
      par(PF::WBND) = Lane<NQ>::wupd(par(PF::WBND), lmax);
    }
    __syncthreads();
  }

  __device__ __forceinline__ double merit(double alpha) {
    fresh();
    const double h = par(PF::H);
    const double sv = par(PF::S) + alpha * st(0, ODZ);
    double val = 0.0, viol = 0.0;
    constexpr bool UNI = NQ == 4;
    for (int k0 = UNI ? 0 : t; k0 <= N; k0 += 64) {
      const bool live = !UNI || k0 + t <= N;
      const int k = UNI ? (live ? k0 + t : N) : k0;
      auto acc = [live](double& a, double x) { a = live ? a + x : a; };
      const gdouble* rec = &g[(long long)k * REC];
      UNR for (int i = 0; i < NZ; ++i) {
        double lb, ub;
        if (!box(k, i, lb, ub)) continue;
        const double v = rec[OZ + i] + alpha * rec[ODZ + i];
        acc(viol, fmax(0.0, lb - v) + fmax(0.0, v - ub));
      }
      if constexpr (HC) {
        if (hc_on(k)) {
          double xq[NQ];
          UNR for (int j = 0; j < NQ; ++j) xq[j] = rec[OZ + j] + alpha * rec[ODZ + j];
          const double hv = hc_eval(xq, nullptr);
          acc(viol, fmax(0.0, o.hlh - hv) + fmax(0.0, hv - o.huh));
        }
      }
      if (k > 0) {
        const gdouble* rp = &g[(long long)(k - 1) * REC];
        double xp[NX], up[NU], phi[NX];
        if (k == 1) {
          UNR for (int j = 0; j < NQ; ++j) { xp[j] = par(PF::Q0 + j); xp[NQ + j] = sv * par(PF::DIR + j); }
          UNR for (int a = 0; a < NU; ++a) up[a] = rp[OZ + 1 + a] + alpha * rp[ODZ + 1 + a];
        } else {
          UNR for (int i = 0; i < NX; ++i) xp[i] = rp[OZ + i] + alpha * rp[ODZ + i];
          UNR for (int a = 0; a < NU; ++a) up[a] = rp[OZ + NX + a] + alpha * rp[ODZ + NX + a];
        }
        rk4<NQ>(h, xp, up, phi);
        UNR for (int i = 0; i < NX; ++i) {
          const double xn = rec[OZ + i] + alpha * rec[ODZ + i];
          acc(val, rp[OWPI + i] * fabs(phi[i] - xn));
        }
        if (k == N) {
          UNR for (int j = 0; j < NQ; ++j)
            acc(val, par(PF::WNU + j) * fabs(rec[OZ + NQ + j] + alpha * rec[ODZ + NQ + j] - par(PF::VFIN + j)));
        }
      }
    }
    return par(PF::CS) * sv + par(PF::CCONST) + wsum(val) + par(PF::WBND) * wsum(viol);
  }

  __device__ __forceinline__ void apply(double alpha) {
    fresh();
    for (int k = t; k <= N; k += 64) {
      gdouble* rec = &g[(long long)k * REC];
      if (k == 0) {
        UNR for (int a = 0; a < NU; ++a) rec[OU + a] += alpha * rec[ODZ + 1 + a];
      } else {
        UNR for (int i = 0; i < NX; ++i) rec[OX + i] += alpha * rec[ODZ + i];
        if (k < N) {
          UNR for (int a = 0; a < NU; ++a) rec[OU + a] += alpha * rec[ODZ + NX + a];
        }
      }
      UNR for (int i = 0; i < NZ; ++i) {
        rec[OLL + i] += alpha * (rec[OQL + i] - rec[OLL + i]);
        rec[OLU + i] += alpha * (rec[OQU + i] - rec[OLU + i]);
      }
      if constexpr (HC) {
        if (hc_on(k)) {
          hcr(k, HL::HLL) += alpha * (hcr(k, HL::HQL) - hcr(k, HL::HLL));
          hcr(k, HL::HLU) += alpha * (hcr(k, HL::HQU) - hcr(k, HL::HLU));
        }
      }
      if (k < N) {
        UNR for (int i = 0; i < NX; ++i) rec[OPI + i] += alpha * (rec[ODA + i] - rec[OPI + i]);
      }
    }
    __syncthreads();
    if (t == 0) {
      par(PF::S) += alpha * st(0, ODZ);
      UNR for (int j = 0; j < NQ; ++j) par(PF::NU_ + j) += alpha * (par(PF::QNU + j) - par(PF::NU_ + j));
    }
    __syncthreads();
  }

  __device__ __forceinline__ void store(const Inputs& in, int pid, int status, int it, int qit) {
    fresh();
    constexpr int NXR = NX + 1;
    double* xo = in.xo + (long long)pid * (in.nmax + 1) * NXR;
    double* uo = in.uo + (long long)pid * in.nmax * NU;
    const double sv = par(PF::S), h = par(PF::H);
    for (int k = t; k <= N; k += 64) {
      UNR for (int i = 0; i < NX; ++i) {
        const double v = (k == 0) ? (i < NQ ? par(PF::Q0 + i) : sv * par(PF::DIR + (i - NQ + (i < NQ ? NQ : 0))))
                                  : (double)st(k, OX + i);
        xo[(long long)k * NXR + i] = v;
      }
      xo[(long long)k * NXR + NX] = h;
      if (k < N) {
        UNR for (int a = 0; a < NU; ++a) uo[(long long)k * NU + a] = st(k, OU + a);
      }
    }
    if (t == 0) {
      in.status[pid] = status;
      in.cost[pid] = par(PF::CS) * sv + par(PF::CCONST);
      in.sqp_iter[pid] = it;
      in.qp_iter[pid] = qit;
    }
  }

  template <bool PAUSE = false>
  __device__ __forceinline__ int run(int& it, int& qit) {
    for (int e = t; e < 16; e += 64) s[L::ZERO + e] = 0.0;
    __syncthreads();
    int status = -1;
    CPROF_DECL
    const int it0 = it;
    int qtot = 0;
    for (;;) {
      if constexpr (PAUSE) {
        if (it == pause_at) { status = -2; break; }
      }
      double rstat, req, rineq, rcomp;
      linearize(rstat, req, rineq, rcomp);
      CPROF(0)
      if (!isfinite(rstat) || !isfinite(req)) status = 1;
      else if (rstat < o.tol_stat && req < o.tol_eq && rineq < o.tol_ineq && rcomp < o.tol_comp) status = 0;
      else if (it >= o.max_iter) status = 2;
      if (status >= 0) break;
      qp_init();
      CPROF(1)
      int qcur = 0, qst = 1;
      double w0[M0], nun[NQ];
      for (;;) {
        int q = qp_check();
        if (q == 1 && qcur >= o.qp_max_iter) q = 2;
        if (q != 1) { qst = q; break; }
        if (!PFUSE || qcur == 0) VREP(1, prep_pred());
        CPROF(2)
        bool okf;
        if constexpr (FM) VREP(2, okf = factor_mfma());
        else VREP(2, okf = factor());
        if constexpr (!ACL_FUSED) VREP(3, acl_pass());
        CPROF(3)
        bool okv;
        VREP(4, (okv = vec<ODA, true, VFUSE>(w0, nun)));
        CPROF(4)
        if (!(okf && okv)) { qst = -1; break; }
        double aa, c0, c1, c2;
        VREP(5, fwd<false>(w0, nun, 0.0, aa, c0, c1, c2));
        CPROF(5)
        const double muaff = (c0 + aa * (c1 + aa * c2)) / nbox;
        double sig = muaff / mu;
        sig = fmin(1.0, sig * sig * sig);
        const double smu = sig * mu;
        VREP(6, prep_corr(smu));
        CPROF(2)
        bool okc;
        VREP(7, (okc = vec<OD, !CCORR>(w0, nun)));
        if (!okc) { qst = -1; break; }
        CPROF(4)
        double amax;
        VREP(8, fwd<true>(w0, nun, smu, amax, c0, c1, c2));
        CPROF(5)
        const double alpha = fmin(1.0, o.tau * amax);
        update(alpha, smu);
        if (t == 0) {
          UNR for (int j = 0; j < NQ; ++j) par(PF::QNU + j) += alpha * (nun[j] - par(PF::QNU + j));
        }
        __syncthreads();
        rs *= (1.0 - alpha);
        ++qcur;
        CPROF(6)
      }
      qit += qcur;
      qtot += qcur;
      if (qst < 0 || !costate()) { status = 4; break; }
      CPROF(7)
      update_weights();
      double alpha = 1.0;
      const double phi0 = merit(0.0);
      for (;;) {
        const double pa = merit(alpha);
        if (pa < phi0) break;
        if (alpha * o.alpha_red < o.alpha_min) break;
        alpha *= o.alpha_red;
      }
      apply(alpha);
      CPROF(8)
      ++it;
      if (!isfinite(par(PF::S))) { status = 1; break; }
    }
    CPROF_FLUSH(it - it0, qtot)
    (void)it0;
    return status;
  }
};


template <int NQ>
struct WavesPerEu { static constexpr int v = NQ <= 3 ? 2 : 1; };

template <int NQ, bool FM, bool HC = false>
__global__ __launch_bounds__(64) __attribute__((amdgpu_waves_per_eu(WavesPerEu<NQ>::v, WavesPerEu<NQ>::v)))
void k_wave(Work w, Opts o, Inputs in, SlotState ss, WaveJobs jb) {
  extern __shared__ __attribute__((aligned(16))) double smem[];
  const int t = (int)threadIdx.x;
  Coop<NQ, FM, HC> C(smem, gptr(jb.regions) + (long long)blockIdx.x * jb.region_doubles, w, o, t);
  if constexpr (HC) C.gh = gptr(jb.hc) + (long long)blockIdx.x * jb.hc_doubles;
  for (;;) {
    unsigned idx = 0;
    if (t == 0) idx = atomicAdd(jb.next, 1u);
    idx = (unsigned)__builtin_amdgcn_readfirstlane((int)__shfl((int)idx, 0));
    if (idx >= (unsigned)jb.count) break;
    int pid, it = 0, qit = 0;
    unsigned slot = 0;
    if (jb.list) {
      slot = (unsigned)__builtin_amdgcn_readfirstlane(jb.list[idx]);
      pid = ss(IS_PID, slot);
      it = ss(IS_IT, slot);
      qit = ss(IS_QIT, slot);
      C.from_slot(ss, slot);
    } else {
      pid = (int)idx;
      Lane<NQ> chk(w, o, 0u);
      if (!chk.supported(in, pid)) {
        if (t == 0) {
          in.status[pid] = 5;
          in.cost[pid] = NAN;
          in.sqp_iter[pid] = 0;
          in.qp_iter[pid] = 0;
          atomicAdd(ss.done, 1u);
        }
        continue;
      }
      if constexpr (HC) {
        double q0[NQ];
        UNR for (int j = 0; j < NQ; ++j) q0[j] = in.lbx0[(long long)pid * (2 * NQ + 1) + j];
        const double h0 = C.hc_eval(q0, nullptr);
        if (!(h0 >= o.hlh && h0 <= o.huh)) {
          if (t == 0) {
            in.status[pid] = 4;
            in.cost[pid] = NAN;
            in.sqp_iter[pid] = 0;
            in.qp_iter[pid] = 0;
            atomicAdd(ss.done, 1u);
          }
          continue;
        }
      }
      C.from_inputs(in, pid);
    }
    const int status = C.run(it, qit);
    C.store(in, pid, status, it, qit);
    __syncthreads();
    if (t == 0) {
      if (jb.list) {
        ss(IS_PID, slot) = -1;
        ss(IS_PH, slot) = 0;
      }
      atomicAdd(ss.done, 1u);
    }
  }
  if constexpr (NQ == 3 && FM && !HC && Coop<NQ, FM, HC>::VFUSE) asm volatile(".rept 96\n\ts_nop 0\n\t.endr");
}

__global__ void k_list(SlotState ss, int* list, unsigned* cnt) {
  const unsigned slot = blockIdx.x * blockDim.x + threadIdx.x;
  if (ss(IS_PID, slot) >= 0 && ss(IS_PH, slot) == 1) list[atomicAdd(cnt, 1u)] = (int)slot;
}

}
```

vboc_amd/csrc/vboc_solver.hip:

```cpp
#include <hip/hip_runtime.h>

#include <chrono>
#include <cmath>
#include <cstdlib>
#include <cstdio>
#include <cstring>
#include <string>
#include <vector>

#include "../../include/vboc.h"
#include "model.h"

#define UNR _Pragma("unroll")
#ifdef VBOC_WAVES
#define VBOC_WPE __attribute__((amdgpu_waves_per_eu(VBOC_WAVES, VBOC_WAVES)))
#else
#define VBOC_WPE
#endif

namespace vboc {

struct Opts {
  double tol_stat, tol_eq, tol_ineq, tol_comp;
  double qp_tol_stat, qp_tol_eq, qp_tol_comp;
// ... 1041 lines not shown
          gdouble& pi = at(w.PI, FPI, k, i);
          pi += alpha * (at(w.QPI, FPI, k, i) - pi);
        }
      }
    }
    UNR for (int j = 0; j < NQ; ++j) par(PF::NU_ + j) += alpha * (par(PF::QNU + j) - par(PF::NU_ + j));
  }
};

enum { IS_PID = 0, IS_IT, IS_QIT, IS_N, IS_PH, IS_QST, IS_QCUR, IS_COUNT };

struct SlotState {
  int* ist;
  unsigned* done;
  unsigned* qp_active;
  unsigned long long* work;
  long long S;
  __device__ __forceinline__ int& operator()(int f, unsigned slot) const { return ist[(long long)f * S + slot]; }
};

template <int NQ>
__device__ __forceinline__ void finish(Lane<NQ>& L, const Inputs& in, const SlotState& ss, int status) {
  const unsigned sl = L.slot;
  L.store_result(in, ss(IS_PID, sl), status, ss(IS_IT, sl), ss(IS_QIT, sl));
  ss(IS_PID, sl) = -1;
  ss(IS_PH, sl) = 0;
  atomicAdd(ss.done, 1u);
}

template <int NQ>
__global__ __launch_bounds__(256) void k_refill(Work w, Opts o, Inputs in, SlotState ss) {
  const unsigned slot = blockIdx.x * blockDim.x + threadIdx.x;
  const int lane = threadIdx.x & 63;
  int pid = ss(IS_PID, slot);
  const unsigned long long need = __ballot(pid == -1);
  if (!need) return;
  const int leader = __ffsll((unsigned long long)need) - 1;
  unsigned int base = 0;
  if (lane == leader) base = atomicAdd(in.head, (unsigned int)__popcll(need));
  base = __shfl(base, leader);
  if (pid != -1) return;
  const unsigned int cand = base + (unsigned)__popcll(need & ((1ull << lane) - 1ull));
  if (cand >= (unsigned int)in.B) {
    ss(IS_PID, slot) = -2;
    return;
  }
  Lane<NQ> L(w, o, slot);
  if (!L.supported(in, (int)cand)) {
    in.status[cand] = 5;
    in.cost[cand] = NAN;
    in.sqp_iter[cand] = 0;
    in.qp_iter[cand] = 0;
    atomicAdd(ss.done, 1u);
    ss(IS_PID, slot) = -1;
    return;
  }
  if (o.hc) {
    constexpr int NXR = 2 * NQ + 1;
    double q0[NQ];
    UNR for (int j = 0; j < NQ; ++j) q0[j] = in.lbx0[(long long)cand * NXR + j];
    const double h0 = L.hc_eval(q0, nullptr);
    if (!(h0 >= o.hlh && h0 <= o.huh)) {
      in.status[cand] = 4;
      in.cost[cand] = NAN;
      in.sqp_iter[cand] = 0;
      in.qp_iter[cand] = 0;
      atomicAdd(ss.done, 1u);
      ss(IS_PID, slot) = -1;
      return;
    }
  }
  L.load(in, (int)cand);
  ss(IS_PID, slot) = (int)cand;
  ss(IS_IT, slot) = 0;
  ss(IS_QIT, slot) = 0;
  ss(IS_N, slot) = L.N;
  ss(IS_PH, slot) = 1;
}

template <int NQ>
__device__ __forceinline__ bool prologue(Lane<NQ>& L, const SlotState& ss, int ph) {
  const bool act = ss(IS_PH, L.slot) == ph;
  L.N = act ? ss(IS_N, L.slot) : 0;
  L.Nw = wave_max(L.N);
  return act;
}

template <int NQ>
__global__ __launch_bounds__(256) VBOC_WPE void k_sens(Work w, Opts o, Inputs in, SlotState ss) {
  Lane<NQ> L(w, o, blockIdx.x * blockDim.x + threadIdx.x);
  if (!prologue(L, ss, 1)) return;
  L.sens();
}

template <int NQ>
__global__ __launch_bounds__(256) VBOC_WPE void k_resid(Work w, Opts o, Inputs in, SlotState ss) {
  Lane<NQ> L(w, o, blockIdx.x * blockDim.x + threadIdx.x);
  if (!prologue(L, ss, 1)) return;
  double rstat, req, rineq, rcomp;
  L.residuals(rstat, req, rineq, rcomp);
  int status = -1;
  if (!isfinite(rstat) || !isfinite(req)) status = 1;
  else if (rstat < o.tol_stat && req < o.tol_eq && rineq < o.tol_ineq && rcomp < o.tol_comp) status = 0;
  else if (ss(IS_IT, L.slot) >= o.max_iter) status = 2;
  if (status >= 0) finish(L, in, ss, status);
  else ss(IS_PH, L.slot) = 2;
}

template <int NQ>
__device__ __forceinline__ bool qp_prologue(Lane<NQ>& L, const SlotState& ss) {
  const bool act = ss(IS_PH, L.slot) == 2 && ss(IS_QST, L.slot) == 1;
  L.N = act ? ss(IS_N, L.slot) : 0;
  L.Nw = wave_max(L.N);
  if (act) L.qp_load_scalars();
  return act;
}

template <int NQ>
__global__ __launch_bounds__(256) VBOC_WPE void k_qp_init(Work w, Opts o, Inputs in, SlotState ss) {
  Lane<NQ> L(w, o, blockIdx.x * blockDim.x + threadIdx.x);
  if (!prologue(L, ss, 2)) return;
  L.qp_init();
  ss(IS_QST, L.slot) = 1;
  ss(IS_QCUR, L.slot) = 0;
  atomicAdd(ss.qp_active, 1u);
}

template <int NQ>
__global__ __launch_bounds__(256) VBOC_WPE void k_qp_factor(Work w, Opts o, Inputs in, SlotState ss) {
  Lane<NQ> L(w, o, blockIdx.x * blockDim.x + threadIdx.x);
  const bool act = qp_prologue(L, ss);
  int st = 0;
  if (act) {
    st = L.qp_check();
    if (st == 1 && ss(IS_QCUR, L.slot) >= o.qp_max_iter) st = 2;
  }
  unsigned long long n = (act && st == 1) ? (unsigned long long)(L.N - 1) : 0ull;
  UNR for (int off = 32; off >= 1; off >>= 1) n += __shfl_xor(n, off);
  if ((threadIdx.x & 63) == 0 && n) atomicAdd(ss.work, n);
  if (!act) return;
  if (st == 1 && !L.qp_factor()) st = -1;
  if (st != 1) {
    ss(IS_QST, L.slot) = st;
    atomicSub(ss.qp_active, 1u);
  }
}

template <int NQ>
__global__ __launch_bounds__(256) VBOC_WPE void k_qp_fpred(Work w, Opts o, Inputs in, SlotState ss) {
  Lane<NQ> L(w, o, blockIdx.x * blockDim.x + threadIdx.x);
  if (!qp_prologue(L, ss)) return;
  L.qp_fpred();
}

template <int NQ>
__global__ __launch_bounds__(256) VBOC_WPE void k_qp_bcorr(Work w, Opts o, Inputs in, SlotState ss) {
  Lane<NQ> L(w, o, blockIdx.x * blockDim.x + threadIdx.x);
  if (!qp_prologue(L, ss)) return;
  if (!L.qp_bcorr()) {
    ss(IS_QST, L.slot) = -1;
    atomicSub(ss.qp_active, 1u);
  }
}

template <int NQ>
__global__ __launch_bounds__(256) VBOC_WPE void k_qp_fcorr(Work w, Opts o, Inputs in, SlotState ss) {
  Lane<NQ> L(w, o, blockIdx.x * blockDim.x + threadIdx.x);
  if (!qp_prologue(L, ss)) return;
  L.qp_fcorr();
}

template <int NQ>
__global__ __launch_bounds__(256) VBOC_WPE void k_qp_update(Work w, Opts o, Inputs in, SlotState ss) {
  Lane<NQ> L(w, o, blockIdx.x * blockDim.x + threadIdx.x);
  if (!qp_prologue(L, ss)) return;
  L.qp_update();
  ss(IS_QCUR, L.slot) += 1;
}

template <int NQ>
__global__ __launch_bounds__(256) VBOC_WPE void k_qp_fin(Work w, Opts o, Inputs in, SlotState ss) {
  Lane<NQ> L(w, o, blockIdx.x * blockDim.x + threadIdx.x);
  if (!prologue(L, ss, 2)) return;
  ss(IS_QIT, L.slot) += ss(IS_QCUR, L.slot);
  const int qs = ss(IS_QST, L.slot);
  if (qs < 0 || !L.qp_costate()) finish(L, in, ss, 4);
  else ss(IS_PH, L.slot) = 3;
}

template <int NQ>
__global__ __launch_bounds__(256) VBOC_WPE void k_ls(Work w, Opts o, Inputs in, SlotState ss) {
  Lane<NQ> L(w, o, blockIdx.x * blockDim.x + threadIdx.x);
  if (!prologue(L, ss, 3)) return;
  L.update_weights();
  const double phi0 = L.merit(0.0);
  double alpha = 1.0;
  for (;;) {
    const double pa = L.merit(alpha);
    if (pa < phi0) break;
    if (alpha * o.alpha_red < o.alpha_min) break;
    alpha *= o.alpha_red;
  }
  L.apply_step(alpha);
  ss(IS_IT, L.slot) += 1;
  if (!isfinite((double)L.par(Par<NQ>::S))) finish(L, in, ss, 1);
  else ss(IS_PH, L.slot) = 1;
}

__global__ void k_slots_init(int* ist, long long S) {
  const long long i = (long long)blockIdx.x * blockDim.x + threadIdx.x;
  if (i >= S) return;
  ist[IS_PID * S + i] = -1;
  ist[IS_PH * S + i] = 0;
  ist[IS_N * S + i] = 0;
}

template <int NQ>
__global__ __launch_bounds__(256) void rk4_kernel(int B, double T, const double* __restrict__ x,
                                                  const double* __restrict__ u, double* __restrict__ xo) {
  const int b = blockIdx.x * blockDim.x + threadIdx.x;
  if (b >= B) return;
  constexpr int NX = 2 * NQ;
  double xi[NX], ui[NQ], x1[NX];
  UNR for (int i = 0; i < NX; ++i) xi[i] = x[(long long)b * NX + i];
  UNR for (int a = 0; a < NQ; ++a) ui[a] = u[(long long)b * NQ + a];
  rk4<NQ>(T, xi, ui, x1);
  UNR for (int i = 0; i < NX; ++i) xo[(long long)b * NX + i] = x1[i];
}

template <int NQ>
__global__ __launch_bounds__(256) void rk4_sens_kernel(int B, double T, const double* __restrict__ x,
                                                       const double* __restrict__ u, double* __restrict__ xo,
                                                       double* __restrict__ A, double* __restrict__ Bm) {
  const int b = blockIdx.x * blockDim.x + threadIdx.x;
  if (b >= B) return;
  constexpr int NX = 2 * NQ;
  double xi[NX], ui[NQ], x1[NX];
  UNR for (int i = 0; i < NX; ++i) xi[i] = x[(long long)b * NX + i];
  UNR for (int a = 0; a < NQ; ++a) ui[a] = u[(long long)b * NQ + a];
  rk4_sens<NQ>(T, xi, ui, x1, [&](int i, int c, double v) {
    if (c < NX) A[(long long)b * NX * NX + i * NX + c] = v;
    else Bm[(long long)b * NX * NQ + i * NQ + (c - NX)] = v;
  });
  UNR for (int i = 0; i < NX; ++i) xo[(long long)b * NX + i] = x1[i];
}

struct WaveJobs {
  const int* list;
  int count;
  unsigned* next;
  double* regions;
  long long region_doubles;
  double* hc = nullptr;
  long long hc_doubles = 0;
};

}

#include "coop.h"
#include "ft.h"
#include "dg.h"
#include "hjr.h"

using namespace vboc;
static thread_local std::string g_err;
static int fail(int code, const std::string& msg) {
  g_err = msg;
  return code;
}
#define HIPCHK(expr)                                                                          \
  do {                                                                                        \
    hipError_t e_ = (expr);                                                                   \
    if (e_ != hipSuccess) return fail(VBOC_ERR_HIP, std::string(#expr ": ") + hipGetErrorString(e_)); \
  } while (0)

struct vboc_solver {
  int nq, nmax, device;
  long long slots;
  Opts o;
  Work w;
  void* pool = nullptr;
  size_t pool_bytes = 0;
  unsigned int* head = nullptr;
  int* ist = nullptr;
  unsigned int* host_done = nullptr;
  hipEvent_t ev0 = nullptr, ev1 = nullptr;
  int launches = 0;
  bool profile = false;
  std::vector<hipEvent_t> pev;
  int npev = 0;
  double fact_ms = 0.0;
  long long fact_calls = 0;
  unsigned long long fact_stages = 0;
  void* stage = nullptr;
  size_t stage_bytes = 0;
  int* list = nullptr;
  double coop_threshold = 8192;
  bool wave_all = true;
  bool factor_mfma = true;
  double* regions = nullptr;
  long long n_regions = 0, region_doubles = 0, group_cap = 0;
  double mall_mib = 256.0;
  size_t wave_lds = 0;
  bool coop_ok = false;
  long long coop_count = 0;
  double* ft_regions = nullptr;
  size_t ft_bytes = 0;
  double* dg_scratch = nullptr;
  size_t dg_bytes = 0;
  DgJobs* dg_jobs = nullptr;
  Inputs* dg_in = nullptr;
  TtJobs* tt_jobs = nullptr;
  bool tt_attr[2] = {false, false};
  bool dg_attr[4] = {false, false, false, false};
  int dg_fail_mod = 0;
  bool dg_speculate = true;
  int dg_spec_early = 0;
  int dg_spec_pause = 300;
  int dg_spec_first = 2;
  bool dg_spec_crit = false;
  int dg_spec_window = 0;
  double* wave_hc = nullptr;
  long long wave_hc_doubles = 0;
  bool hc_wave = true;
  void* dg_spec = nullptr;
  size_t dg_spec_bytes = 0;
  void* mpc_buf = nullptr;
  size_t mpc_bytes = 0;
  void* al_buf = nullptr;
  size_t al_bytes = 0;
  bool dg_park = true;
  int dg_park_window = 0;
  int dg_park_hi = 100;
  int dg_round = 0;
  void* dg_park_buf = nullptr;
  size_t dg_park_bytes = 0;
  bool dg_busy = false;
  long long last_groups = 0;
};

static void default_opts(Opts& o) {
  o.tol_stat = 1e-3; o.tol_eq = 1e-6; o.tol_ineq = 1e-6; o.tol_comp = 1e-6;
  o.qp_tol_stat = 1e-3; o.qp_tol_eq = 1e-8; o.qp_tol_comp = 1e-8;
  o.alpha_min = 1e-2; o.alpha_red = 0.3; o.lm = 1e-5;
  o.mu0 = 1.0; o.push = 1e-2; o.tau = 0.995;
  o.max_iter = 1000; o.qp_max_iter = 100;
  o.hc = 0; o.hxc = o.hyc = o.hlh = o.huh = 0.0;
}

static int par_count(int nq) {
  return nq == 1 ? Par<1>::COUNT : (nq == 2 ? Par<2>::COUNT : (nq == 3 ? Par<3>::COUNT : Par<4>::COUNT));
}

static inline size_t ev(size_t f) { return (f + 1) & ~(size_t)1; }

static size_t work_doubles_per_slot(int nq, int nmax) {
  const size_t NX = 2 * nq, NU = nq, NZ = 3 * nq, M0 = nq + 1;
  const size_t per_stage = ev(NX)  + ev(NU) + ev(NX)  + 2 * ev(NZ) + ev(NX)  + ev(NX * NX) +
                           ev(NX * NU) + ev(NX) + 3 * ev(NZ) + ev(NX)  + ev(NU * NX) + ev(NU) + ev(NU * NU) +
                           2 * ev(NU * nq) + ev(NX)  + 2 * ev(NZ) + ev(NX);
  const size_t per_slot = ev(NX * M0) + ev(M0 * M0) + 2 * ev(M0 * nq) + ev(NX) + ev(par_count(nq));
  return per_stage * (size_t)(nmax + 1) + per_slot;
}

static hipError_t prof_flush(vboc_solver* h, hipStream_t st) {
  if (!h->npev) return hipSuccess;
  hipError_t e = hipStreamSynchronize(st);
  if (e != hipSuccess) return e;
  for (int i = 0; i < h->npev; ++i) {
    float f = 0.f;
    e = hipEventElapsedTime(&f, h->pev[2 * i], h->pev[2 * i + 1]);
    if (e != hipSuccess) return e;
    h->fact_ms += f;
  }
  h->fact_calls += h->npev;
  h->npev = 0;
  return hipSuccess;
}

template <int NQ>
static hipError_t launch_round(vboc_solver* h, dim3 grid, dim3 block, hipStream_t st, const Work& w, const Opts& o,
                               const Inputs& in, const SlotState& ss) {
  hipLaunchKernelGGL(k_refill<NQ>, grid, block, 0, st, w, o, in, ss);
  hipLaunchKernelGGL(k_sens<NQ>, grid, block, 0, st, w, o, in, ss);
  hipLaunchKernelGGL(k_resid<NQ>, grid, block, 0, st, w, o, in, ss);
  hipError_t e = hipMemsetAsync(ss.qp_active, 0, sizeof(unsigned), st);
  if (e != hipSuccess) return e;
  hipLaunchKernelGGL(k_qp_init<NQ>, grid, block, 0, st, w, o, in, ss);
  h->launches += 5;
  for (int it = 0; it <= o.qp_max_iter; ++it) {
    if (h->profile) {
      if ((size_t)(2 * h->npev + 2) > h->pev.size()) {
        e = prof_flush(h, st);
        if (e != hipSuccess) return e;
      }
      e = hipEventRecord(h->pev[2 * h->npev], st);
      if (e != hipSuccess) return e;
    }
    hipLaunchKernelGGL(k_qp_factor<NQ>, grid, block, 0, st, w, o, in, ss);
    if (h->profile) {
      e = hipEventRecord(h->pev[2 * h->npev + 1], st);
      if (e != hipSuccess) return e;
      ++h->npev;
    }
    ++h->launches;
    if (it >= 6 && (it & 1) == 0) {
      e = hipMemcpyAsync(h->host_done + 1, ss.qp_active, sizeof(unsigned), hipMemcpyDeviceToHost, st);
      if (e == hipSuccess) e = hipStreamSynchronize(st);
      if (e != hipSuccess) return e;
      if (h->host_done[1] == 0) break;
    }
    if (it == o.qp_max_iter) break;
    hipLaunchKernelGGL(k_qp_fpred<NQ>, grid, block, 0, st, w, o, in, ss);
    hipLaunchKernelGGL(k_qp_bcorr<NQ>, grid, block, 0, st, w, o, in, ss);
    hipLaunchKernelGGL(k_qp_fcorr<NQ>, grid, block, 0, st, w, o, in, ss);
    hipLaunchKernelGGL(k_qp_update<NQ>, grid, block, 0, st, w, o, in, ss);
    h->launches += 4;
  }
  hipLaunchKernelGGL(k_qp_fin<NQ>, grid, block, 0, st, w, o, in, ss);
  hipLaunchKernelGGL(k_ls<NQ>, grid, block, 0, st, w, o, in, ss);
  h->launches += 2;
  return hipGetLastError();
}

template <int NQ>
static int launch_ft(vboc_solver* h, const Inputs& in, hipStream_t st, const MpcArgs& mp = MpcArgs{}) {
  const long long rd = mp.on ? FtL<NQ, true>::region_doubles(in.nmax) : FtL<NQ, false>::region_doubles(in.nmax);
  long long groups = in.B < 1024 ? in.B : 1024;
  const size_t need = (size_t)groups * (size_t)rd * sizeof(double);
  if (need > h->ft_bytes) {
    if (h->ft_regions) (void)hipFree(h->ft_regions);
    h->ft_regions = nullptr;
    h->ft_bytes = 0;
    if (hipMalloc(&h->ft_regions, need) != hipSuccess) return -1;
    h->ft_bytes = need;
  }
  if constexpr (NQ == 3) {
    if (mp.on) {
      hipLaunchKernelGGL((k_ft<NQ, true>), dim3((unsigned)groups), dim3(64), 0, st, h->o, in, h->ft_regions, rd, h->head,
                         mp);
      return hipGetLastError() == hipSuccess ? 0 : -2;
    }
  }
  if (mp.on) return -2;
  hipLaunchKernelGGL((k_ft<NQ, false>), dim3((unsigned)groups), dim3(64), 0, st, h->o, in, h->ft_regions, rd, h->head,
                     mp);
  return hipGetLastError() == hipSuccess ? 0 : -2;
}

static long long wave_group_budget(const vboc_solver* h, int nmax) {
  const long long hot = (long long)(h->nq == 1 ? WaveLayout<1>::OX
                                    : (h->nq == 2 ? WaveLayout<2>::OX : (h->nq == 3 ? WaveLayout<3>::OX : WaveLayout<4>::OX))) *
                        (long long)(nmax + 1) * (long long)sizeof(double);
  const long long g = (long long)(0.92 * h->mall_mib * 1024.0 * 1024.0) / (hot > 0 ? hot : 1);
  return g < 256 ? 256 : g;
}

static hipError_t launch_wave(vboc_solver* h, const WaveJobs& jb, long long jobs, hipStream_t st, const Work& w,
                              const Inputs& in, const SlotState& ss) {
  long long groups = jobs < h->n_regions ? jobs : h->n_regions;
  const long long cap = h->group_cap > 0 ? h->group_cap : (h->mall_mib > 0 ? wave_group_budget(h, in.nmax) : 0);
  if (cap > 0 && groups > cap) groups = cap;
  if (groups < 1) return hipSuccess;
  h->last_groups = groups;
  const dim3 grid((unsigned)groups), block(64);
  switch (h->nq) {
    case 1:
      if (h->factor_mfma) hipLaunchKernelGGL((k_wave<1, true>), grid, block, h->wave_lds, st, w, h->o, in, ss, jb);
      else hipLaunchKernelGGL((k_wave<1, false>), grid, block, h->wave_lds, st, w, h->o, in, ss, jb);
      break;
    case 2:
      if (h->o.hc) hipLaunchKernelGGL((k_wave<2, false, true>), grid, block, h->wave_lds, st, w, h->o, in, ss, jb);
      else if (h->factor_mfma) hipLaunchKernelGGL((k_wave<2, true>), grid, block, h->wave_lds, st, w, h->o, in, ss, jb);
      else hipLaunchKernelGGL((k_wave<2, false>), grid, block, h->wave_lds, st, w, h->o, in, ss, jb);
      break;
    case 3:
      if (h->factor_mfma) hipLaunchKernelGGL((k_wave<3, true>), grid, block, h->wave_lds, st, w, h->o, in, ss, jb);
      else hipLaunchKernelGGL((k_wave<3, false>), grid, block, h->wave_lds, st, w, h->o, in, ss, jb);
      break;
    default: hipLaunchKernelGGL((k_wave<4, false>), grid, block, h->wave_lds, st, w, h->o, in, ss, jb); break;
  }
  return hipGetLastError();
}

template <int NQ, bool FM>
static hipError_t launch_dg(vboc_solver* h, const DgJobs& J, const Inputs& in, long long groups, hipStream_t st,
                           bool testing = false) {
  const void* fn = testing ? (const void*)k_ts<NQ, FM> : (const void*)k_dg<NQ, FM>;
  bool& attr = h->dg_attr[(FM ? 1 : 0) + (testing ? 2 : 0)];
  if (!attr) {
    hipError_t e = hipFuncSetAttribute(fn, hipFuncAttributeMaxDynamicSharedMemorySize, (int)h->wave_lds);
    if (e != hipSuccess) return e;
    attr = true;
  }
  WaveJobs jb{nullptr, J.count, J.next, h->regions, h->region_doubles};
  hipError_t e = hipMemcpyAsync(h->dg_jobs, &J, sizeof(DgJobs), hipMemcpyHostToDevice, st);
  if (e == hipSuccess) e = hipMemcpyAsync(h->dg_in, &in, sizeof(Inputs), hipMemcpyHostToDevice, st);
  if (e == hipSuccess) e = hipStreamSynchronize(st);
  if (e != hipSuccess) return e;
  if (testing)
    hipLaunchKernelGGL((k_ts<NQ, FM>), dim3((unsigned)groups), dim3(64), h->wave_lds, st, h->w, h->o, in,
                       (const Inputs*)h->dg_in, (const DgJobs*)h->dg_jobs, jb);
  else
    hipLaunchKernelGGL((k_dg<NQ, FM>), dim3((unsigned)groups), dim3(64), h->wave_lds, st, h->w, h->o, in,
                       (const Inputs*)h->dg_in, (const DgJobs*)h->dg_jobs, jb);
  return hipGetLastError();
}

template <int NQ, bool FM, bool HC>
static hipError_t launch_tt(vboc_solver* h, const TtJobs& J, const Inputs& in, long long groups, hipStream_t st) {
  const void* fn = (const void*)k_tt<NQ, FM, HC>;
  bool& attr = h->tt_attr[NQ == 4 ? 1 : 0];
  if (!attr) {
    hipError_t e = hipFuncSetAttribute(fn, hipFuncAttributeMaxDynamicSharedMemorySize, (int)h->wave_lds);
    if (e != hipSuccess) return e;
    attr = true;
  }
  WaveJobs jb{nullptr, J.count, J.next, h->regions, h->region_doubles, HC ? h->wave_hc : nullptr,
              HC ? h->wave_hc_doubles : 0};
  hipError_t e = hipMemcpyAsync(h->tt_jobs, &J, sizeof(TtJobs), hipMemcpyHostToDevice, st);
  if (e == hipSuccess) e = hipMemcpyAsync(h->dg_in, &in, sizeof(Inputs), hipMemcpyHostToDevice, st);
  if (e == hipSuccess) e = hipStreamSynchronize(st);
  if (e != hipSuccess) return e;
  hipLaunchKernelGGL((k_tt<NQ, FM, HC>), dim3((unsigned)groups), dim3(64), h->wave_lds, st, h->w, h->o, in,
                     (const Inputs*)h->dg_in, (const TtJobs*)h->tt_jobs, jb);
  return hipGetLastError();
}

static bool busy(const vboc_solver* h, const char* who) {
  if (!h || !h->dg_busy) return false;
  fail(VBOC_ERR_ARG, std::string(who) + ": a vboc_data_generation_async launch is still running on this handle "
                                        "(call vboc_data_generation_wait first)");
  return true;
}

extern "C" {

const char* vboc_last_error(void) { return g_err.c_str(); }

int vboc_create(int nq, int nmax, int slots, int device, vboc_handle* out) {
  if (!out) return fail(VBOC_ERR_ARG, "vboc_create: out is NULL");
  *out = nullptr;
  if (nq < 1 || nq > 4) return fail(VBOC_ERR_ARG, "vboc_create: nq must be 1, 2, 3 (pendulum chains) or 4 (UR5)");
  if (nmax < 1) return fail(VBOC_ERR_ARG, "vboc_create: nmax must be >= 1");
  HIPCHK(hipSetDevice(device));
  vboc_solver* h = new vboc_solver();
  h->nq = nq; h->nmax = nmax; h->device = device;
  h->factor_mfma = nq <= 3;
  default_opts(h->o);
  if (nq == 4) {
    h->o.lm = 1e-2;
    h->coop_threshold = 0;
  }
  if (slots <= 0) slots = 64 * 1024;
  if (slots > (1 << 30)) return fail(VBOC_ERR_ARG, "vboc_create: too many slots");
  slots = ((slots + 255) / 256) * 256;
  h->slots = slots;
  const size_t per_slot = work_doubles_per_slot(nq, nmax);
  h->pool_bytes = per_slot * (size_t)slots * sizeof(double);
  hipError_t e = hipMalloc(&h->pool, h->pool_bytes);
  if (e != hipSuccess) {
    delete h;
    return fail(VBOC_ERR_NOMEM, std::string("vboc_create: hipMalloc workspace: ") + hipGetErrorString(e));
  }
  e = hipMalloc((void**)&h->head, 256);
  if (e == hipSuccess) e = hipMalloc((void**)&h->ist, sizeof(int) * IS_COUNT * (size_t)slots);
  if (e == hipSuccess) e = hipMalloc((void**)&h->list, sizeof(int) * (size_t)slots);
  if (e == hipSuccess) e = hipHostMalloc((void**)&h->host_done, 64);
  if (e != hipSuccess) {
    vboc_destroy(h);
    return fail(VBOC_ERR_NOMEM, "vboc_create: hipMalloc queue / slot state");
  }
  (void)hipEventCreate(&h->ev0);
  (void)hipEventCreate(&h->ev1);
  {
    const void* fn = nq == 1 ? (const void*)k_wave<1, false>
                             : (nq == 2 ? (const void*)k_wave<2, false>
                                        : (nq == 3 ? (const void*)k_wave<3, false> : (const void*)k_wave<4, false>));
    h->wave_lds = nq == 1 ? WaveLayout<1>::lds_bytes(nmax)
                          : (nq == 2 ? WaveLayout<2>::lds_bytes(nmax)
                                     : (nq == 3 ? WaveLayout<3>::lds_bytes(nmax) : WaveLayout<4>::lds_bytes(nmax)));
    h->region_doubles = nq == 1 ? (long long)WaveLayout<1>::region_doubles(nmax)
                                : (nq == 2 ? (long long)WaveLayout<2>::region_doubles(nmax)
                                           : (nq == 3 ? (long long)WaveLayout<3>::region_doubles(nmax)
                                                      : (long long)WaveLayout<4>::region_doubles(nmax)));
    int per_cu = 0, cus = 0;
    hipDeviceProp_t prop;
    if (hipOccupancyMaxActiveBlocksPerMultiprocessor(&per_cu, fn, 64, h->wave_lds) == hipSuccess &&
        hipGetDeviceProperties(&prop, device) == hipSuccess) {
      cus = prop.multiProcessorCount;
    }
    (void)hipGetLastError();
    if (per_cu < 1) per_cu = 1;
    if (cus < 1) cus = 256;
    h->n_regions = (long long)per_cu * cus;
    if (h->n_regions > 16384) h->n_regions = 16384;
    if (h->wave_lds > 160 * 1024) h->n_regions = 0;
    h->coop_ok = h->n_regions > 0 &&
                 hipFuncSetAttribute(fn, hipFuncAttributeMaxDynamicSharedMemorySize, (int)h->wave_lds) == hipSuccess &&
                 hipMalloc((void**)&h->regions, sizeof(double) * (size_t)h->region_doubles * (size_t)h->n_regions) ==
                     hipSuccess;
    (void)hipGetLastError();
  }
  const int NX = 2 * nq, NU = nq, NZ = 3 * nq, M0 = nq + 1;
  const size_t st = (size_t)(nmax + 1) * slots;
  double* p = (double*)h->pool;
  auto take = [&](size_t fields_per_stage) { double* r = p; p += ev(fields_per_stage) * st; return r; };
  auto take0 = [&](size_t fields) { double* r = p; p += ev(fields) * (size_t)slots; return r; };
  Work& w = h->w;
  w.S = slots;
  w.HC = nullptr;
  w.X = take(NX); w.U = take(NU); w.PI = take(NX); w.LL = take(NZ); w.LU = take(NZ); w.WPI = take(NX);
  w.A = take(NX * NX); w.Bm = take(NX * NU); w.BD = take(NX);
  w.DZ = take(NZ); w.QL = take(NZ); w.QU = take(NZ); w.E0 = take(NX);
  w.K = take(NU * NX); w.KF = take(NU); w.LR = take(NU * NU); w.M = take(NU * nq); w.Y = take(NU * nq);
  w.PE = take(NX); w.D = take(NZ); w.DAFF = take(NZ); w.QPI = take(NX);
  w.F0 = take0(NX * M0); w.LR0 = take0(M0 * M0); w.M0 = take0(M0 * nq); w.Y0 = take0(M0 * nq); w.PE0 = take0(NX);
  w.PAR = take0(par_count(nq));
  if ((size_t)((char*)p - (char*)h->pool) != h->pool_bytes) {
    vboc_destroy(h);
    return fail(VBOC_ERR_ARG, "vboc_create: internal workspace size mismatch");
  }
  *out = h;
  return VBOC_OK;
}

int vboc_destroy(vboc_handle h) {
  if (!h) return VBOC_OK;
  (void)hipSetDevice(h->device);
  if (h->dg_busy && h->ev1) (void)hipEventSynchronize(h->ev1);
  if (h->pool) (void)hipFree(h->pool);
  if (h->head) (void)hipFree(h->head);
  if (h->ist) (void)hipFree(h->ist);
  if (h->w.HC) (void)hipFree(h->w.HC);
  if (h->wave_hc) (void)hipFree(h->wave_hc);
  if (h->list) (void)hipFree(h->list);
  if (h->regions) (void)hipFree(h->regions);
  if (h->host_done) (void)hipHostFree(h->host_done);
  if (h->stage) (void)hipFree(h->stage);
  if (h->ft_regions) (void)hipFree(h->ft_regions);
  if (h->dg_scratch) (void)hipFree(h->dg_scratch);
  if (h->dg_jobs) (void)hipFree(h->dg_jobs);
  if (h->dg_in) (void)hipFree(h->dg_in);
  if (h->tt_jobs) (void)hipFree(h->tt_jobs);
  if (h->dg_spec) (void)hipFree(h->dg_spec);
  if (h->dg_park_buf) (void)hipFree(h->dg_park_buf);
  if (h->mpc_buf) (void)hipFree(h->mpc_buf);
  if (h->al_buf) (void)hipFree(h->al_buf);
  if (h->ev0) (void)hipEventDestroy(h->ev0);
  if (h->ev1) (void)hipEventDestroy(h->ev1);
  for (auto ev : h->pev) (void)hipEventDestroy(ev);
  delete h;
  return VBOC_OK;
}

int vboc_set_option(vboc_handle h, const char* f, double v) {
  if (busy(h, "vboc_set_option")) return VBOC_ERR_ARG;
  if (!h || !f) return fail(VBOC_ERR_ARG, "vboc_set_option: NULL argument");
  Opts& o = h->o;
  const std::string s(f);
  if (s == "nlp_solver_tol_stat") o.tol_stat = v;
  else if (s == "nlp_solver_tol_eq") o.tol_eq = v;
  else if (s == "nlp_solver_tol_ineq") o.tol_ineq = v;
  else if (s == "nlp_solver_tol_comp") o.tol_comp = v;
  else if (s == "nlp_solver_max_iter") o.max_iter = (int)v;
  else if (s == "qp_solver_iter_max") o.qp_max_iter = (int)v;
  else if (s == "qp_solver_tol_stat") o.qp_tol_stat = v;
  else if (s == "qp_solver_tol_eq") o.qp_tol_eq = v;
  else if (s == "qp_solver_tol_comp") o.qp_tol_comp = v;
  else if (s == "levenberg_marquardt") o.lm = v;
  else if (s == "alpha_min") o.alpha_min = v;
  else if (s == "alpha_reduction") o.alpha_red = v;
  else if (s == "ipm_mu0") o.mu0 = v;
  else if (s == "ipm_push") o.push = v;
  else if (s == "ipm_tau") o.tau = v;
  else if (s == "coop_threshold") h->coop_threshold = v;
  else if (s == "wave_all") {
    h->wave_all = v != 0.0;
  }
  else if (s == "factor_mfma") h->factor_mfma = v != 0.0 && h->nq <= 3;
  else if (s == "wave_groups") h->group_cap = (long long)v;
  else if (s == "mall_mib") h->mall_mib = v;
  else if (s == "dg_fail_mod") h->dg_fail_mod = (int)v;
  else if (s == "dg_speculate") h->dg_speculate = v != 0.0;
  else if (s == "dg_spec_early") h->dg_spec_early = v > 0.0 ? (int)v : 0;
  else if (s == "dg_spec_pause") h->dg_spec_pause = v > 0.0 ? (int)v : 0;
  else if (s == "dg_spec_first") h->dg_spec_first = v >= 2.0 ? 2 : (v != 0.0 ? 1 : 0);
  else if (s == "dg_spec_crit") h->dg_spec_crit = v != 0.0;
  else if (s == "dg_spec_window") h->dg_spec_window = v > 0.0 ? (v < 9.0 ? (int)v : 9) : 0;
  else if (s == "dg_park") h->dg_park = v != 0.0;
  else if (s == "dg_park_window") h->dg_park_window = v > 0.0 ? (int)v : 0;
  else if (s == "dg_park_hi") h->dg_park_hi = v > 0.0 ? (int)v : 0;
  else if (s == "dg_round") h->dg_round = v > 0.0 ? (int)v : 0;
  else if (s == "hc_wave") h->hc_wave = v != 0.0;
  else if (s == "profile_kernels") {
    h->profile = v != 0.0;
    if (h->profile && h->pev.empty()) {
      h->pev.resize(2 * 4096);
      for (auto& ev : h->pev)
        if (hipEventCreate(&ev) != hipSuccess) return fail(VBOC_ERR_HIP, "vboc_set_option: hipEventCreate");
    }
  } else return fail(VBOC_ERR_ARG, "vboc_set_option: unknown field '" + s + "'");
  return VBOC_OK;
}

int vboc_get_option(vboc_handle h, const char* f, double* v) {
  if (!h || !f || !v) return fail(VBOC_ERR_ARG, "vboc_get_option: NULL argument");
  const Opts& o = h->o;
  const std::string s(f);
  if (s == "nlp_solver_tol_stat") *v = o.tol_stat;
  else if (s == "nlp_solver_tol_eq") *v = o.tol_eq;
  else if (s == "nlp_solver_tol_ineq") *v = o.tol_ineq;
  else if (s == "nlp_solver_tol_comp") *v = o.tol_comp;
  else if (s == "nlp_solver_max_iter") *v = o.max_iter;
  else if (s == "qp_solver_iter_max") *v = o.qp_max_iter;
  else if (s == "qp_solver_tol_stat") *v = o.qp_tol_stat;
  else if (s == "qp_solver_tol_eq") *v = o.qp_tol_eq;
  else if (s == "qp_solver_tol_comp") *v = o.qp_tol_comp;
  else if (s == "levenberg_marquardt") *v = o.lm;
  else if (s == "alpha_min") *v = o.alpha_min;
  else if (s == "alpha_reduction") *v = o.alpha_red;
  else if (s == "ipm_mu0") *v = o.mu0;
  else if (s == "ipm_push") *v = o.push;
  else if (s == "ipm_tau") *v = o.tau;
  else if (s == "coop_threshold") *v = h->coop_threshold;
  else if (s == "coop_available") *v = h->coop_ok ? 1.0 : 0.0;
  else if (s == "wave_all") *v = h->wave_all ? 1.0 : 0.0;
  else if (s == "dg_speculate") *v = h->dg_speculate ? 1.0 : 0.0;
  else if (s == "dg_spec_early") *v = (double)h->dg_spec_early;
  else if (s == "dg_spec_pause") *v = (double)h->dg_spec_pause;
  else if (s == "dg_spec_first") *v = (double)h->dg_spec_first;
  else if (s == "dg_spec_crit") *v = h->dg_spec_crit ? 1.0 : 0.0;
  else if (s == "dg_spec_window") *v = (double)h->dg_spec_window;
  else if (s == "dg_park") *v = h->dg_park ? 1.0 : 0.0;
  else if (s == "dg_park_window") *v = (double)h->dg_park_window;
  else if (s == "dg_park_hi") *v = (double)h->dg_park_hi;
  else if (s == "dg_round") *v = (double)h->dg_round;
  else if (s == "hc_wave") *v = h->hc_wave ? 1.0 : 0.0;
  else if (s == "factor_mfma") *v = h->factor_mfma ? 1.0 : 0.0;
  else if (s == "wave_groups") *v = (double)h->n_regions;
  else if (s == "last_groups") *v = (double)h->last_groups;
  else if (s == "dg_busy") *v = h->dg_busy ? 1.0 : 0.0;
  else if (s == "mall_mib") *v = h->mall_mib;
  else if (s == "coop_problems") *v = (double)h->coop_count;
  else if (s == "slots") *v = (double)h->slots;
  else if (s == "workspace_bytes") *v = (double)h->pool_bytes;
  else return fail(VBOC_ERR_ARG, "vboc_get_option: unknown field '" + s + "'");
  return VBOC_OK;
}

int vboc_set_path_constraint(vboc_handle h, int kind, double x_c, double y_c, double lh, double uh) {
  if (busy(h, "vboc_set_path_constraint")) return VBOC_ERR_ARG;
  if (!h) return fail(VBOC_ERR_ARG, "vboc_set_path_constraint: NULL handle");
  if (kind == 0) { h->o.hc = 0; return VBOC_OK; }
  if (kind != 1) return fail(VBOC_ERR_ARG, "vboc_set_path_constraint: unknown kind");
  if (h->nq != 2 && h->nq != 3)
    return fail(VBOC_ERR_UNSUPPORTED, "vboc_set_path_constraint: the keep-out circle needs a pendulum chain (nq 2 or 3)");
  if (!(lh <= uh)) return fail(VBOC_ERR_ARG, "vboc_set_path_constraint: lh > uh");
  if (!h->w.HC) {
    const size_t f = h->nq == 2 ? (size_t)Lane<2>::FHC : (size_t)Lane<3>::FHC;
    HIPCHK(hipSetDevice(h->device));
    const hipError_t e = hipMalloc((void**)&h->w.HC, sizeof(double) * ev(f) * (size_t)(h->nmax + 1) * (size_t)h->slots);
    if (e != hipSuccess) {
      h->w.HC = nullptr;
      return fail(VBOC_ERR_NOMEM, "vboc_set_path_constraint: hipMalloc constraint rows");
    }
  }
  if (!h->wave_hc && h->coop_ok && h->nq == 2) {
    const long long f = (long long)Lane<2>::FHC;
    h->wave_hc_doubles = f * (long long)(h->nmax + 1);
    if (hipMalloc((void**)&h->wave_hc, sizeof(double) * (size_t)h->wave_hc_doubles * (size_t)h->n_regions) != hipSuccess) {
      h->wave_hc = nullptr;
      (void)hipGetLastError();
    }
  }
  h->o.hc = 1; h->o.hxc = x_c; h->o.hyc = y_c; h->o.hlh = lh; h->o.huh = uh;
  return VBOC_OK;
}

int vboc_solve_batch(vboc_handle h, const vboc_batch_t* b, void* stream) {
  if (busy(h, "vboc_solve_batch")) return VBOC_ERR_ARG;
  if (!h || !b) return fail(VBOC_ERR_ARG, "vboc_solve_batch: NULL argument");
  if (b->B < 0) return fail(VBOC_ERR_ARG, "vboc_solve_batch: B < 0");
  if (b->nmax > h->nmax || b->nmax < 1)
    return fail(VBOC_ERR_ARG, "vboc_solve_batch: batch nmax exceeds the handle's nmax");
  if (b->B == 0) { h->launches = 0; return VBOC_OK; }
  const void* ptrs[] = {b->N, b->x_guess, b->u_guess, b->p, b->lbx, b->ubx, b->lbu, b->ubu, b->lbx_0, b->ubx_0,
                        b->lbx_e, b->ubx_e, b->status, b->x_out, b->u_out, b->cost, b->sqp_iter, b->qp_iter};
  for (const void* q : ptrs)
    if (!q) return fail(VBOC_ERR_ARG, "vboc_solve_batch: NULL array in batch");
  HIPCHK(hipSetDevice(h->device));
  hipStream_t st = (hipStream_t)stream;
  Inputs in;
  in.B = b->B; in.nmax = b->nmax; in.N = b->N;
  in.xg = b->x_guess; in.ug = b->u_guess; in.p = b->p; in.lbx = b->lbx; in.ubx = b->ubx; in.lbu = b->lbu;
  in.ubu = b->ubu; in.lbx0 = b->lbx_0; in.ubx0 = b->ubx_0; in.lbxe = b->lbx_e; in.ubxe = b->ubx_e;
  in.status = b->status; in.xo = b->x_out; in.uo = b->u_out; in.cost = b->cost; in.sqp_iter = b->sqp_iter;
  in.qp_iter = b->qp_iter; in.head = h->head;
  HIPCHK(hipMemsetAsync(h->head, 0, 256, st));
  h->fact_ms = 0.0;
  h->fact_calls = 0;
  h->fact_stages = 0;
  h->npev = 0;
  h->coop_count = 0;
  long long lanes = ((long long)b->B + 255) / 256 * 256;
  if (lanes > h->slots) lanes = h->slots;
  Work w = h->w;
  SlotState ss{h->ist, h->head + 1, h->head + 2, (unsigned long long*)(h->head + 4), h->slots};
  const dim3 grid((unsigned)(lanes / 256)), block(256);
  HIPCHK(hipEventRecord(h->ev0, st));
  const bool hc_ok = !h->o.hc || (h->hc_wave && h->wave_hc);
  if (h->wave_all && h->coop_ok && hc_ok) {
    WaveJobs jb{nullptr, b->B, h->head, h->regions, h->region_doubles, h->wave_hc, h->wave_hc_doubles};
    h->launches = 1;
    h->coop_count = b->B;
    HIPCHK(launch_wave(h, jb, (long long)b->B, st, w, in, ss));
    HIPCHK(hipEventRecord(h->ev1, st));
    HIPCHK(hipStreamSynchronize(st));
    HIPCHK(hipMemcpy(h->host_done, h->head + 1, sizeof(unsigned), hipMemcpyDeviceToHost));
    if (*h->host_done != (unsigned)b->B) return fail(VBOC_ERR_HIP, "vboc_solve_batch: wave solver did not finish");
    return VBOC_OK;
  }
  hipLaunchKernelGGL(k_slots_init, dim3((unsigned)((h->slots + 255) / 256)), block, 0, st, h->ist, h->slots);
  const int chunk = 4;
  long long rounds = 0;
  h->launches = 1;
  const bool progress = getenv("VBOC_PROGRESS") != nullptr;
  auto t_start = std::chrono::steady_clock::now();
  unsigned last_print = 0;
  for (;;) {
    for (int r = 0; r < chunk; ++r) {
      hipError_t le;
      switch (h->nq) {
        case 1: le = launch_round<1>(h, grid, block, st, w, h->o, in, ss); break;
        case 2: le = launch_round<2>(h, grid, block, st, w, h->o, in, ss); break;
        case 3: le = launch_round<3>(h, grid, block, st, w, h->o, in, ss); break;
        default: le = launch_round<4>(h, grid, block, st, w, h->o, in, ss); break;
      }
      if (le != hipSuccess) return fail(VBOC_ERR_HIP, std::string("vboc_solve_batch: ") + hipGetErrorString(le));
    }
    rounds += chunk;
    HIPCHK(hipGetLastError());
    HIPCHK(hipMemcpyAsync(h->host_done + 4, h->head, 2 * sizeof(unsigned), hipMemcpyDeviceToHost, st));
    HIPCHK(hipStreamSynchronize(st));
    h->host_done[0] = h->host_done[5];
    const unsigned pulled = h->host_done[4] < (unsigned)b->B ? h->host_done[4] : (unsigned)b->B;
    if (h->coop_ok && h->coop_threshold > 0 && !h->o.hc && h->host_done[4] >= (unsigned)b->B &&
        (double)(pulled - h->host_done[0]) <= h->coop_threshold && h->host_done[0] < (unsigned)b->B) {
      HIPCHK(hipMemsetAsync(h->head + 3, 0, sizeof(unsigned), st));
      hipLaunchKernelGGL(k_list, grid, block, 0, st, ss, h->list, h->head + 3);
      HIPCHK(hipMemcpyAsync(h->host_done + 2, h->head + 3, sizeof(unsigned), hipMemcpyDeviceToHost, st));
      HIPCHK(hipStreamSynchronize(st));
      const unsigned n = h->host_done[2];
      h->coop_count = n;
      if (n) {
        HIPCHK(hipMemsetAsync(h->head + 5, 0, sizeof(unsigned), st));
        WaveJobs jb{h->list, (int)n, h->head + 5, h->regions, h->region_doubles};
        HIPCHK(launch_wave(h, jb, (long long)n, st, w, in, ss));
        h->launches += 2;
      }
      HIPCHK(hipMemcpyAsync(h->host_done, h->head + 1, sizeof(unsigned), hipMemcpyDeviceToHost, st));
      HIPCHK(hipStreamSynchronize(st));
      if (progress) {
        const double ms = std::chrono::duration<double, std::milli>(std::chrono::steady_clock::now() - t_start).count();
        fprintf(stderr, "[vboc] %.1f ms cooperative tail: %u problems, done %u / %d\n", ms, n, *h->host_done, b->B);
      }
      if (*h->host_done < (unsigned)b->B) return fail(VBOC_ERR_HIP, "vboc_solve_batch: cooperative tail did not finish");
    }
    if (progress && (*h->host_done - last_print >= (unsigned)b->B / 20 || *h->host_done >= (unsigned)b->B ||
                     rounds % 64 == 0)) {
      const double ms = std::chrono::duration<double, std::milli>(std::chrono::steady_clock::now() - t_start).count();
      fprintf(stderr, "[vboc] %.1f ms rounds %lld done %u / %d\n", ms, rounds, *h->host_done, b->B);
      last_print = *h->host_done;
    }
    if (*h->host_done >= (unsigned)b->B) break;
    if (rounds > 4LL * (h->o.max_iter + 2) * ((b->B + lanes - 1) / lanes + 1))
      return fail(VBOC_ERR_HIP, "vboc_solve_batch: solver did not drain (internal error)");
  }
  HIPCHK(hipGetLastError());
  HIPCHK(hipEventRecord(h->ev1, st));
  if (h->profile) HIPCHK(prof_flush(h, st));
  HIPCHK(hipMemcpyAsync(&h->fact_stages, h->head + 4, sizeof(unsigned long long), hipMemcpyDeviceToHost, st));
  HIPCHK(hipStreamSynchronize(st));
  return VBOC_OK;
}

int vboc_debug_counters(unsigned long long* out16) {
  if (!out16) return fail(VBOC_ERR_ARG, "vboc_debug_counters: NULL argument");
  HIPCHK(hipMemcpyFromSymbol(out16, HIP_SYMBOL(g_wave_prof), 16 * sizeof(unsigned long long)));
  static const unsigned long long zero[16] = {0};
  HIPCHK(hipMemcpyToSymbol(HIP_SYMBOL(g_wave_prof), zero, sizeof(zero)));
  return VBOC_OK;
}

int vboc_last_kernel_ms(vboc_handle h, double* ms, int* launches) {
  if (!h || !ms) return fail(VBOC_ERR_ARG, "vboc_last_kernel_ms: NULL argument");
  float f = 0.0f;
  HIPCHK(hipEventSynchronize(h->ev1));
  HIPCHK(hipEventElapsedTime(&f, h->ev0, h->ev1));
  *ms = f;
// ... 32 lines not shown
  in.ubu = b->ubu; in.lbx0 = b->lbx_0; in.ubx0 = b->ubx_0; in.lbxe = b->lbx_e; in.ubxe = b->ubx_e;
  in.status = b->status; in.xo = b->x_out; in.uo = b->u_out; in.cost = b->cost; in.sqp_iter = b->sqp_iter;
  in.qp_iter = b->qp_iter; in.head = h->head;
  HIPCHK(hipMemsetAsync(h->head, 0, 256, st));
  HIPCHK(hipEventRecord(h->ev0, st));
  int rc;
  switch (h->nq) {
    case 1: rc = launch_ft<1>(h, in, st); break;
    case 2: rc = launch_ft<2>(h, in, st); break;
    case 3: rc = launch_ft<3>(h, in, st); break;
    default: return fail(VBOC_ERR_UNSUPPORTED, "vboc_solve_batch_ft: the free-time OCP is defined for the pendulum chains only");
  }
  if (rc == -1) return fail(VBOC_ERR_NOMEM, "vboc_solve_batch_ft: hipMalloc of the stage regions");
  if (rc) return fail(VBOC_ERR_HIP, std::string("vboc_solve_batch_ft: ") + hipGetErrorString(hipGetLastError()));
  HIPCHK(hipEventRecord(h->ev1, st));
  h->launches = 1;
  return VBOC_OK;
}

static int solve_host(vboc_handle h, const vboc_batch_t* b, bool ft) {
  if (!h || !b) return fail(VBOC_ERR_ARG, "vboc_solve_batch_host: NULL argument");
  if (b->B == 0) return VBOC_OK;
  HIPCHK(hipSetDevice(h->device));
  const int nq = h->nq, NXR = 2 * nq + 1, NU = nq, NP = nq + 1;
  const size_t B = b->B, Nn = b->nmax;
  const size_t sz_xg = B * (Nn + 1) * NXR, sz_ug = B * Nn * NU;
  const size_t dbl = sz_xg * 2 + sz_ug * 2 + B * NP + B * NXR * 6 + B * NU * 2 + B ;
  const size_t ints = B * 4;
  const size_t need = dbl * sizeof(double) + ints * sizeof(int) + 256;
  if (need > h->stage_bytes) {
    if (h->stage) (void)hipFree(h->stage);
    h->stage = nullptr;
    h->stage_bytes = 0;
    hipError_t e = hipMalloc(&h->stage, need);
    if (e != hipSuccess) return fail(VBOC_ERR_NOMEM, "vboc_solve_batch_host: hipMalloc staging");
    h->stage_bytes = need;
  }
  double* d = (double*)h->stage;
  hipError_t cerr = hipSuccess;
  auto put = [&](const double* src, size_t n) -> double* {
    double* r = d;
    d += n;
    if (src && cerr == hipSuccess) cerr = hipMemcpy(r, src, n * sizeof(double), hipMemcpyHostToDevice);
    return r;
  };
  vboc_batch_t db = *b;
  db.x_guess = put(b->x_guess, sz_xg);
  db.u_guess = put(b->u_guess, sz_ug);
  db.p = put(b->p, B * NP);
  db.lbx = put(b->lbx, B * NXR); db.ubx = put(b->ubx, B * NXR);
  db.lbu = put(b->lbu, B * NU); db.ubu = put(b->ubu, B * NU);
  db.lbx_0 = put(b->lbx_0, B * NXR); db.ubx_0 = put(b->ubx_0, B * NXR);
  db.lbx_e = put(b->lbx_e, B * NXR); db.ubx_e = put(b->ubx_e, B * NXR);
  db.x_out = put(b->x_out, sz_xg);
  db.u_out = put(b->u_out, sz_ug);
  db.cost = put(nullptr, B);
  int* ip = (int*)d;
  db.N = ip; ip += B;
  db.status = ip; ip += B;
  db.sqp_iter = ip; ip += B;
  db.qp_iter = ip; ip += B;
  HIPCHK(cerr);
  HIPCHK(hipMemcpy((void*)db.N, b->N, B * sizeof(int), hipMemcpyHostToDevice));
  int rc = ft ? vboc_solve_batch_ft(h, &db, nullptr) : vboc_solve_batch(h, &db, nullptr);
  if (rc) return rc;
  HIPCHK(hipDeviceSynchronize());
  HIPCHK(hipMemcpy(b->x_out, db.x_out, sz_xg * sizeof(double), hipMemcpyDeviceToHost));
  HIPCHK(hipMemcpy(b->u_out, db.u_out, sz_ug * sizeof(double), hipMemcpyDeviceToHost));
  HIPCHK(hipMemcpy(b->cost, db.cost, B * sizeof(double), hipMemcpyDeviceToHost));
  HIPCHK(hipMemcpy(b->status, db.status, B * sizeof(int), hipMemcpyDeviceToHost));
  HIPCHK(hipMemcpy(b->sqp_iter, db.sqp_iter, B * sizeof(int), hipMemcpyDeviceToHost));
  HIPCHK(hipMemcpy(b->qp_iter, db.qp_iter, B * sizeof(int), hipMemcpyDeviceToHost));
  return VBOC_OK;
}

__global__ void k_mpc_prep(int B, int N, int nq, double hstep, const double* __restrict__ x0,
                           const double* __restrict__ xg6, const double* lbx, const double* ubx, const double* lbu,
                           const double* ubu, const double* lbxe, const double* ubxe, double* xg7, double* lbx7,
                           double* ubx7, double* lbu_b, double* ubu_b, double* lbx0, double* ubx0, double* lbxe7,
                           double* ubxe7, double* p, int* Nb) {
  const int n2 = 2 * nq, nx = n2 + 1;
  const long long tot = (long long)B * (N + 1);
  for (long long e = blockIdx.x * (long long)blockDim.x + threadIdx.x; e < tot; e += (long long)gridDim.x * blockDim.x) {
    const long long b = e / (N + 1);
    for (int i = 0; i < n2; ++i) xg7[e * nx + i] = xg6[e * n2 + i];
    xg7[e * nx + n2] = hstep;
    if (e % (N + 1) == 0) {
      Nb[b] = N;
      for (int i = 0; i < n2; ++i) {
        lbx7[b * nx + i] = lbx[i]; ubx7[b * nx + i] = ubx[i];
        lbxe7[b * nx + i] = lbxe[i]; ubxe7[b * nx + i] = ubxe[i];
        lbx0[b * nx + i] = ubx0[b * nx + i] = x0[b * n2 + i];
      }
      lbx7[b * nx + n2] = lbxe7[b * nx + n2] = -INFINITY;
      ubx7[b * nx + n2] = ubxe7[b * nx + n2] = INFINITY;
      lbx0[b * nx + n2] = ubx0[b * nx + n2] = hstep;
      for (int a = 0; a < nq; ++a) { lbu_b[b * nq + a] = lbu[a]; ubu_b[b * nq + a] = ubu[a]; }
      for (int a = 0; a <= nq; ++a) p[b * (nq + 1) + a] = 0.0;
    }
  }
}
__global__ void k_mpc_strip(long long tot, int nq, const double* __restrict__ xo7, double* __restrict__ xo6) {
  const int n2 = 2 * nq, nx = n2 + 1;
  for (long long e = blockIdx.x * (long long)blockDim.x + threadIdx.x; e < tot; e += (long long)gridDim.x * blockDim.x)
    for (int i = 0; i < n2; ++i) xo6[e * n2 + i] = xo7[e * nx + i];
}
__global__ void k_transpose(int H, const double* __restrict__ a, double* __restrict__ at) {
  for (long long e = blockIdx.x * (long long)blockDim.x + threadIdx.x; e < (long long)H * H; e += (long long)gridDim.x * blockDim.x)
    at[(e % H) * H + e / H] = a[e];
}

static int mpc_solve(vboc_handle h, const vboc_mpc_batch_t* b, const vboc_mpc_soft_t* sf, void* stream,
                     const std::string& W, int qcf = 0);

int vboc_mpc_solve_batch(vboc_handle h, const vboc_mpc_batch_t* b, void* stream) {
  return mpc_solve(h, b, nullptr, stream, "vboc_mpc_solve_batch");
}

__global__ void k_al_guess(int B, int N, int nq, const double* __restrict__ x0, double* __restrict__ xg,
                           double* __restrict__ ug) {
  const int n2 = 2 * nq;
  const long long tot = (long long)B * (N + 1);
  for (long long e = blockIdx.x * (long long)blockDim.x + threadIdx.x; e < tot; e += (long long)gridDim.x * blockDim.x) {
    const long long b = e / (N + 1), k = e % (N + 1);
    for (int i = 0; i < n2; ++i) xg[e * n2 + i] = i < nq ? x0[b * n2 + i] : 0.0;
    if (k < N)
      for (int a = 0; a < nq; ++a) ug[(b * N + k) * nq + a] = 0.0;
  }
}
__global__ void k_al_label(int B, const int* __restrict__ status, int* __restrict__ label) {
  for (int b = blockIdx.x * blockDim.x + threadIdx.x; b < B; b += gridDim.x * blockDim.x)
    label[b] = status[b] == 0 ? 1 : (status[b] == 4 ? 0 : 2);
}

int vboc_al_solve_batch(vboc_handle h, const vboc_al_batch_t* b, void* stream) {
  const std::string W = "vboc_al_solve_batch";
  if (!h || !b) return fail(VBOC_ERR_ARG, W + ": NULL argument");
  if (busy(h, W.c_str())) return VBOC_ERR_ARG;
  if (b->B < 0 || b->N < 1 || b->N > h->nmax) return fail(VBOC_ERR_ARG, W + ": needs B >= 0 and 1 <= N <= nmax");
  if (b->B == 0) { h->launches = 0; return VBOC_OK; }
  const void* ptrs[] = {b->x0, b->lbx, b->ubx, b->lbu, b->ubu, b->lbx_e, b->ubx_e, b->W, b->We, b->label,
                        b->status, b->x_out, b->u_out, b->qp_iter};
  for (const void* q : ptrs)
    if (!q) return fail(VBOC_ERR_ARG, W + ": NULL array in batch");
  if (h->nq != 3) return fail(VBOC_ERR_UNSUPPORTED, W + ": the AL labelling OCP is the triple pendulum's (nq = 3)");
  HIPCHK(hipSetDevice(h->device));
  hipStream_t st = (hipStream_t)stream;
  constexpr int NQ = 3;
  const size_t B = (size_t)b->B, N = (size_t)b->N;
  const size_t need = (B * (N + 1) * 2 * NQ + B * N * NQ + B) * sizeof(double) + B * sizeof(int) + 256;
  if (need > h->al_bytes) {
    if (h->al_buf) (void)hipFree(h->al_buf);
    h->al_buf = nullptr;
    h->al_bytes = 0;
    if (hipMalloc(&h->al_buf, need) != hipSuccess) return fail(VBOC_ERR_NOMEM, W + ": hipMalloc of the guesses");
    h->al_bytes = need;
  }
  double* xg = (double*)h->al_buf;
  double* ug = xg + B * (N + 1) * 2 * NQ;
  double* cost = ug + B * N * NQ;
  int* sqp = (int*)(cost + B);
  hipLaunchKernelGGL(k_al_guess, dim3(256), dim3(256), 0, st, b->B, b->N, NQ, b->x0, xg, ug);
  HIPCHK(hipGetLastError());
  static const double zero[3 * NQ] = {0.0};
  vboc_mpc_batch_t m{};
  m.B = b->B; m.N = b->N; m.rti = 1; m.hidden = 0; m.h = b->h; m.cost_scale = b->cost_scale;
  m.x0 = b->x0; m.x_guess = b->x_guess ? b->x_guess : xg; m.u_guess = ug;
  m.lbx = b->lbx; m.ubx = b->ubx; m.lbu = b->lbu; m.ubu = b->ubu; m.lbx_e = b->lbx_e; m.ubx_e = b->ubx_e;
  m.W = b->W; m.We = b->We; m.yref = zero; m.yref_e = zero;
  m.status = b->status; m.x_out = b->x_out; m.u_out = b->u_out; m.cost = cost; m.sqp_iter = sqp;
  m.qp_iter = b->qp_iter; m.h_out = nullptr;
  const int rc = mpc_solve(h, &m, nullptr, stream, W, 1);
  if (rc != VBOC_OK) return rc;
  hipLaunchKernelGGL(k_al_label, dim3(64), dim3(256), 0, st, b->B, b->status, b->label);
  HIPCHK(hipGetLastError());
  return VBOC_OK;
}

int vboc_mpc_soft_solve_batch(vboc_handle h, const vboc_mpc_batch_t* b, const vboc_mpc_soft_t* soft, void* stream) {
  const std::string W = "vboc_mpc_soft_solve_batch";
  if (!soft) return fail(VBOC_ERR_ARG, W + ": NULL soft-constraint description");
  if (b && b->B > 0 && !soft->Zl) return fail(VBOC_ERR_ARG, W + ": NULL Zl (the per-stage slack weights)");
  if (b && b->hidden <= 0) return fail(VBOC_ERR_ARG, W + ": the soft rows need the network (hidden > 0)");
  if (!(soft->safety_margin < 100.0)) return fail(VBOC_ERR_ARG, W + ": safety_margin must be < 100");
  return mpc_solve(h, b, soft, stream, W);
}

static int mpc_solve(vboc_handle h, const vboc_mpc_batch_t* b, const vboc_mpc_soft_t* sf, void* stream,
                     const std::string& W, int qcf) {
  if (busy(h, W.c_str())) return VBOC_ERR_ARG;
  if (!h || !b) return fail(VBOC_ERR_ARG, W + ": NULL argument");
  if (h->nq != 3) return fail(VBOC_ERR_UNSUPPORTED, W + ": the Safe-MPC OCP is the triple pendulum's (nq = 3)");
  if (h->o.hc) return fail(VBOC_ERR_UNSUPPORTED, W + ": no path constraint in the Safe-MPC OCP (clear it first)");
  if (b->B < 0 || b->N < 1 || b->N > h->nmax) return fail(VBOC_ERR_ARG, W + ": needs B >= 0 and 1 <= N <= nmax");
  if (b->hidden < 0 || b->hidden > FT_NN_MAX) return fail(VBOC_ERR_ARG, W + ": hidden must be in [0, 512]");
  if (!(b->h > 0.0)) return fail(VBOC_ERR_ARG, W + ": the time step must be positive");
  if (b->B == 0) { h->launches = 0; return VBOC_OK; }
  const void* ptrs[] = {b->x0, b->x_guess, b->u_guess, b->lbx, b->ubx, b->lbu, b->ubu, b->lbx_e, b->ubx_e, b->W,
                        b->We, b->yref, b->yref_e, b->status, b->x_out, b->u_out, b->cost, b->sqp_iter, b->qp_iter};
  for (const void* q : ptrs)
    if (!q) return fail(VBOC_ERR_ARG, W + ": NULL array in batch");
  if (b->hidden > 0 && (!b->W0 || !b->b0 || !b->W1 || !b->b1 || !b->W2 || !b->b2))
    return fail(VBOC_ERR_ARG, W + ": NULL network parameter");
  HIPCHK(hipSetDevice(h->device));
  hipStream_t st = (hipStream_t)stream;
  constexpr int NQ = 3, NX = 2 * NQ + 1, NU = NQ;
  const size_t B = (size_t)b->B, N = (size_t)b->N, H = (size_t)b->hidden;
  const size_t dbl = B * (N + 1) * NX * 2 + B * NX * 6 + B * NU * 2 + B * (NQ + 1) + H * H;
  const size_t need = dbl * sizeof(double) + B * sizeof(int) + 512;
  if (need > h->mpc_bytes) {
    if (h->mpc_buf) (void)hipFree(h->mpc_buf);
    h->mpc_buf = nullptr;
    h->mpc_bytes = 0;
    if (hipMalloc(&h->mpc_buf, need) != hipSuccess) return fail(VBOC_ERR_NOMEM, W + ": hipMalloc of the batch inputs");
    h->mpc_bytes = need;
  }
  double* d = (double*)h->mpc_buf;
  auto take = [&](size_t n) { double* r = d; d += (n + 1) & ~(size_t)1; return r; };
  double* xg7 = take(B * (N + 1) * NX);
  double* xo7 = take(B * (N + 1) * NX);
  double *lbx7 = take(B * NX), *ubx7 = take(B * NX), *lbx0 = take(B * NX), *ubx0 = take(B * NX);
  double *lbxe7 = take(B * NX), *ubxe7 = take(B * NX), *lbu_b = take(B * NU), *ubu_b = take(B * NU);
  double* pp = take(B * (NQ + 1));
  double* w1t = take(H * H);
  int* Nb = (int*)d;
  hipLaunchKernelGGL(k_mpc_prep, dim3(256), dim3(256), 0, st, b->B, b->N, NQ, b->h, b->x0, b->x_guess, b->lbx, b->ubx,
                     b->lbu, b->ubu, b->lbx_e, b->ubx_e, xg7, lbx7, ubx7, lbu_b, ubu_b, lbx0, ubx0, lbxe7, ubxe7, pp,
                     Nb);
  MpcArgs mp{};
  mp.on = 1; mp.rti = b->rti ? 1 : 0; mp.hid = b->hidden; mp.cs = b->cost_scale; mp.qcf = qcf;
  const double *Wh = b->W, *Weh = b->We, *yr = b->yref, *yre = b->yref_e;
  for (int i = 0; i < 2 * NQ; ++i) { mp.wq[i] = Wh[i]; mp.yr[i] = yr[i]; mp.we[i] = Weh[i]; mp.yre[i] = yre[i]; }
  mp.wq[2 * NQ] = mp.yr[2 * NQ] = mp.we[2 * NQ] = mp.yre[2 * NQ] = 0.0;
  for (int a = 0; a < NU; ++a) { mp.wq[NX + a] = Wh[2 * NQ + a]; mp.yr[NX + a] = yr[2 * NQ + a]; }
  if (b->hidden > 0) {
    hipLaunchKernelGGL(k_transpose, dim3(256), dim3(256), 0, st, b->hidden, b->W1, w1t);
    mp.W0 = b->W0; mp.b0 = b->b0; mp.W1 = b->W1; mp.W1T = w1t; mp.b1 = b->b1; mp.W2 = b->W2; mp.b2 = b->b2;
    mp.mean = b->mean; mp.std = b->std; mp.lh = b->lh; mp.uh = b->uh;
  }
  mp.hrow = b->h_out;
  mp.soft = 0; mp.sm = 100.0; mp.zl = mp.Zl = mp.Wb = mp.Web = nullptr;
  if (sf) {
    mp.soft = 1; mp.sm = 100.0 - sf->safety_margin;
    mp.zl = sf->zl; mp.Zl = sf->Zl; mp.Wb = sf->W_b; mp.Web = sf->We_b;
  }
  Inputs in;
  in.B = b->B; in.nmax = b->N; in.N = Nb;
  in.xg = xg7; in.ug = b->u_guess; in.p = pp; in.lbx = lbx7; in.ubx = ubx7; in.lbu = lbu_b; in.ubu = ubu_b;
  in.lbx0 = lbx0; in.ubx0 = ubx0; in.lbxe = lbxe7; in.ubxe = ubxe7;
  in.status = b->status; in.xo = xo7; in.uo = b->u_out; in.cost = b->cost; in.sqp_iter = b->sqp_iter;
  in.qp_iter = b->qp_iter; in.head = h->head;
  HIPCHK(hipMemsetAsync(h->head, 0, 256, st));
  HIPCHK(hipEventRecord(h->ev0, st));
  const int rc = launch_ft<NQ>(h, in, st, mp);
  if (rc == -1) return fail(VBOC_ERR_NOMEM, W + ": hipMalloc of the stage regions");
  if (rc) return fail(VBOC_ERR_HIP, W + ": " + hipGetErrorString(hipGetLastError()));
  HIPCHK(hipEventRecord(h->ev1, st));
  hipLaunchKernelGGL(k_mpc_strip, dim3(256), dim3(256), 0, st, (long long)(B * (N + 1)), NQ, xo7, b->x_out);
  HIPCHK(hipGetLastError());
  h->launches = 1;
  return VBOC_OK;
}

int vboc_solve_batch_host(vboc_handle h, const vboc_batch_t* b) { return solve_host(h, b, false); }
int vboc_solve_batch_ft_host(vboc_handle h, const vboc_batch_t* b) { return solve_host(h, b, true); }

static int dg_wait(vboc_handle h, vboc_dg_batch_t* b, hipStream_t st);

int vboc_data_generation(vboc_handle h, vboc_dg_batch_t* b, void* stream) {
  const int rc = vboc_data_generation_async(h, b, nullptr, nullptr, stream);
  if (rc != VBOC_OK || !b || b->B == 0) return rc;
  return dg_wait(h, b, (hipStream_t)stream);
}

int vboc_data_generation_wait(vboc_handle h, vboc_dg_batch_t* b, void* stream) {
  if (!h || !b) return fail(VBOC_ERR_ARG, "vboc_data_generation_wait: NULL argument");
  if (b->B == 0) return VBOC_OK;
  return dg_wait(h, b, (hipStream_t)stream);
}

static int dg_prepare(vboc_handle h, vboc_dg_batch_t* b, int* done_flag, const int* cancel, hipStream_t st,
                      bool testing, int max_restarts, const char* who) {
  const std::string W(who);
  if (busy(h, who)) return VBOC_ERR_ARG;
  if (h->nq != 2 && h->nq != 3)
    return fail(VBOC_ERR_UNSUPPORTED, W + ": defined for the double (nq = 2) and triple (nq = 3) pendulum");
  if (h->o.hc)
    return fail(VBOC_ERR_UNSUPPORTED, W + ": the boundary OCP of this driver has no path constraint (clear it first)");
  if (b->B < 0) return fail(VBOC_ERR_ARG, W + ": B < 0");
  b->rows_used = 0;
  if (b->B == 0) return VBOC_OK;
  if (b->N_start < 2 || b->N_start + 12 > h->nmax)
    return fail(VBOC_ERR_ARG, W + ": needs 2 <= N_start and N_start + 12 <= the handle's nmax "
                              "(horizon extension +9, verification horizons up to N - 1 + 4)");
  if (!b->ids || !b->rows || !b->row_off || !b->row_cnt || !b->stats ||
      (!testing && h->nq == 2 && (!b->ic || !b->ic_slot)))
    return fail(VBOC_ERR_ARG, W + ": NULL array");
  if (testing && b->rows_cap < b->B) return fail(VBOC_ERR_ARG, W + ": rows_cap < B (one row per problem)");
  if (testing && max_restarts < 0) return fail(VBOC_ERR_ARG, W + ": max_restarts < 0");
  if (!h->coop_ok) return fail(VBOC_ERR_HIP, W + ": wave solver unavailable on this device");
  HIPCHK(hipSetDevice(h->device));
  long long groups = b->B < h->n_regions ? b->B : h->n_regions;
  const long long cap = h->group_cap > 0 ? h->group_cap
                                         : (h->mall_mib > 0 ? wave_group_budget(h, b->N_start + 10) : 0);
  if (cap > 0 && groups > cap) groups = cap;
  h->last_groups = groups;
  const int nq = h->nq, NXR = 2 * nq + 1, NU = nq, NP = nq + 1, NX = 2 * nq, nm = h->nmax;
  const int vr_cap = 2 * nm + 2;
  const size_t st_bytes = nq == 2 ? (sizeof(DgState<2>) > sizeof(TsState<2>) ? sizeof(DgState<2>) : sizeof(TsState<2>))
                                  : (sizeof(DgState<3>) > sizeof(TsState<3>) ? sizeof(DgState<3>) : sizeof(TsState<3>));
  const int st_d = (int)((st_bytes + 15) / 16 * 2);
  const size_t G = (size_t)groups;
  const size_t dbl = G * ((size_t)(nm + 1) * NXR * 3 + (size_t)nm * NU * 2 + (size_t)(nm + 1) * NU + NP + 6 * NXR +
                          2 * NU + 1 + (size_t)vr_cap * NX + st_d) + 64;
  const size_t need = dbl * sizeof(double) + 4 * G * sizeof(int) + 256;
  if (need > h->dg_bytes) {
    if (h->dg_scratch) (void)hipFree(h->dg_scratch);
    h->dg_scratch = nullptr;
    h->dg_bytes = 0;
    if (hipMalloc((void**)&h->dg_scratch, need) != hipSuccess)
      return fail(VBOC_ERR_NOMEM, W + ": hipMalloc of the state-machine records");
    h->dg_bytes = need;
  }
  if (!h->dg_jobs && hipMalloc((void**)&h->dg_jobs, sizeof(DgJobs)) != hipSuccess)
    return fail(VBOC_ERR_NOMEM, W + ": hipMalloc of the job descriptor");
  if (!h->dg_in && hipMalloc((void**)&h->dg_in, sizeof(Inputs)) != hipSuccess)
    return fail(VBOC_ERR_NOMEM, W + ": hipMalloc of the batch descriptor");
  double* d = h->dg_scratch;
  auto take = [&](size_t n) { double* r = d; d += (n + 1) & ~(size_t)1; return r; };
  Inputs in;
  in.B = (int)groups; in.nmax = nm; in.head = nullptr;
  double* xg = take(G * (nm + 1) * NXR); double* ug = take(G * nm * NU); double* pp = take(G * NP);
  double* lbx = take(G * NXR); double* ubx = take(G * NXR); double* lbu = take(G * NU); double* ubu = take(G * NU);
  double* lbx0 = take(G * NXR); double* ubx0 = take(G * NXR); double* lbxe = take(G * NXR); double* ubxe = take(G * NXR);
  in.xg = xg; in.ug = ug; in.p = pp; in.lbx = lbx; in.ubx = ubx; in.lbu = lbu; in.ubu = ubu;
  in.lbx0 = lbx0; in.ubx0 = ubx0; in.lbxe = lbxe; in.ubxe = ubxe;
  in.xo = take(G * (nm + 1) * NXR); in.uo = take(G * nm * NU); in.cost = take(G);
  DgJobs J;
  J.xs = take(G * (nm + 1) * NXR); J.us = take(G * (nm + 1) * NU); J.vr = take(G * vr_cap * NX);
  J.st = take(G * st_d);
  J.vr_cap = vr_cap; J.st_doubles = st_d;
  int* ip = (int*)d;
  in.N = ip; ip += G;
  in.status = ip; ip += G;
  in.sqp_iter = ip; ip += G;
  in.qp_iter = ip; ip += G;
  if ((size_t)((char*)ip - (char*)h->dg_scratch) > need) return fail(VBOC_ERR_ARG, W + ": internal size error");
  J.ids = b->ids; J.count = b->B; J.N_start = b->N_start; J.nmax = nm; J.seed = b->seed;
  J.fail_mod = h->dg_fail_mod;
  J.max_restarts = max_restarts;
  J.fmt_scale = nq == 2 ? 1e4 : 1e3;
  J.q_min = b->q_min; J.q_max = b->q_max; J.v_max = b->v_max; J.u_max = b->u_max; J.dt = b->dt; J.tol = b->tol;
  J.eps = b->eps; J.g = b->g; J.l1 = b->l1; J.l2 = b->l2; J.m1 = b->m1; J.m2 = b->m2;
  J.rows = b->rows; J.rows_cap = b->rows_cap; J.row_off = b->row_off; J.row_cnt = b->row_cnt;
  J.ic = (!testing && h->nq == 2) ? b->ic : nullptr; J.ic_slot = (!testing && h->nq == 2) ? b->ic_slot : nullptr;
  J.stats = b->stats;
  J.done_flag = done_flag; J.cancel = cancel;
  J.next = h->head; J.done = h->head + 1; J.err = h->head + 2; J.rows_next = (unsigned long long*)(h->head + 4);
  J.spec_ev_next = h->head + 6; J.spec_q_tail = h->head + 7; J.spec_q_head = h->head + 8;
  J.spec_count = (unsigned long long*)(h->head + 10);
  J.spec_events = 0; J.spec_stride = 0; J.spec = nullptr; J.spec_early = h->dg_spec_early; J.spec_pause = h->dg_spec_pause; J.spec_first = (h->dg_spec_first == 1 || (h->dg_spec_first == 2 && (long long)b->B < 128 * groups)) ? 1 : 0;
  J.spec_claim = J.spec_done = J.spec_cancel = J.spec_q = J.spec_eq = nullptr;
  J.spec_window = 0; J.spec_eq_tail = h->head + 20; J.spec_eq_head = h->head + 21;
  J.spec_crit = 0; J.t_launch = (unsigned long long*)(h->head + 22);
  size_t spec_ctl = 0;
  if (h->dg_speculate && !testing) {
    const int E = b->B < 8192 ? b->B : 8192;
    const long long res = DG_SPEC_RH + (long long)(nm + 1) * NXR + (long long)nm * NU;
    const long long stride = DG_SPEC_HDR + DG_SPEC_JOBS * res;
    spec_ctl = sizeof(int) * ((size_t)E * (2 * (DG_SPEC_JOBS + 1) + 1 + 2 * DG_SPEC_JOBS));
    const size_t sneed = spec_ctl + sizeof(double) * (size_t)E * (size_t)stride + 256;
    if (sneed > h->dg_spec_bytes) {
      if (h->dg_spec) (void)hipFree(h->dg_spec);
      h->dg_spec = nullptr;
      h->dg_spec_bytes = 0;
      if (hipMalloc(&h->dg_spec, sneed) != hipSuccess)
        return fail(VBOC_ERR_NOMEM, W + ": hipMalloc of the speculation pool");
      h->dg_spec_bytes = sneed;
    }
    int* ci = (int*)h->dg_spec;
    J.spec_claim = ci; ci += (size_t)E * (DG_SPEC_JOBS + 1);
    J.spec_done = ci; ci += (size_t)E * (DG_SPEC_JOBS + 1);
    J.spec_cancel = ci; ci += E;
    J.spec_q = ci; ci += (size_t)E * DG_SPEC_JOBS;
    J.spec_eq = ci;
    J.spec_window = h->dg_spec_window;
    J.spec_crit = h->dg_spec_crit ? 1 : 0;
    J.spec = (double*)((char*)h->dg_spec + ((spec_ctl + 255) & ~(size_t)255));
    J.spec_events = E; J.spec_stride = (int)stride;
    HIPCHK(hipMemsetAsync(h->dg_spec, 0, spec_ctl, st));
  }
  J.park_res = nullptr; J.park_q = nullptr; J.park_stride = 0;
  J.park_window = 0; J.park_hi_it = h->dg_park_hi;
  J.round_n = done_flag ? h->dg_round : 0;
  J.park_tail = h->head + 16; J.park_head = h->head + 18;
  if (h->dg_park && !testing) {
    const int stride = (8 + (b->N_start + 1) * NXR + b->N_start * NU + 1) & ~1;
    const size_t qbytes = ((sizeof(int) * 2 * (size_t)b->B) + 255) & ~(size_t)255;
    const size_t pneed = qbytes + sizeof(double) * (size_t)stride * (size_t)b->B;
    if (pneed > h->dg_park_bytes) {
      if (h->dg_park_buf) (void)hipFree(h->dg_park_buf);
      h->dg_park_buf = nullptr;
      h->dg_park_bytes = 0;
      if (hipMalloc(&h->dg_park_buf, pneed) != hipSuccess)
        return fail(VBOC_ERR_NOMEM, W + ": hipMalloc of the parked first solves");
      h->dg_park_bytes = pneed;
    }
    J.park_q = (int*)h->dg_park_buf;
    J.park_res = (double*)((char*)h->dg_park_buf + qbytes);
    J.park_stride = stride;
    J.park_window = h->dg_park_window > 0 ? h->dg_park_window : (done_flag ? (int)(groups < b->B ? groups : b->B) : b->B);
    HIPCHK(hipMemsetAsync(h->dg_park_buf, 0, sizeof(int) * 2 * (size_t)b->B, st));
  }
  HIPCHK(hipMemsetAsync(h->head, 0, 256, st));
  HIPCHK(hipEventRecord(h->ev0, st));
  hipError_t e;
  if (h->nq == 2)
    e = h->factor_mfma ? launch_dg<2, true>(h, J, in, groups, st, testing) : launch_dg<2, false>(h, J, in, groups, st, testing);
  else
    e = h->factor_mfma ? launch_dg<3, true>(h, J, in, groups, st, testing) : launch_dg<3, false>(h, J, in, groups, st, testing);
  if (e != hipSuccess) return fail(VBOC_ERR_HIP, W + ": " + hipGetErrorString(e));
  HIPCHK(hipEventRecord(h->ev1, st));
  h->launches = 1;
  h->coop_count = b->B;
  return VBOC_OK;
}

int vboc_data_generation_async(vboc_handle h, vboc_dg_batch_t* b, int* done_flag, const int* cancel, void* stream) {
  if (!h || !b) return fail(VBOC_ERR_ARG, "vboc_data_generation: NULL argument");
  const int rc = dg_prepare(h, b, done_flag, cancel, (hipStream_t)stream, false, 0, "vboc_data_generation");
  if (rc == VBOC_OK && b->B > 0) h->dg_busy = true;
  return rc;
}

int vboc_testing(vboc_handle h, vboc_dg_batch_t* b, int max_restarts, void* stream) {
  if (!h || !b) return fail(VBOC_ERR_ARG, "vboc_testing: NULL argument");
  const int rc = dg_prepare(h, b, nullptr, nullptr, (hipStream_t)stream, true, max_restarts, "vboc_testing");
  if (rc != VBOC_OK || b->B == 0) return rc;
  return dg_wait(h, b, (hipStream_t)stream);
}

int vboc_testing_test(vboc_handle h, vboc_tt_batch_t* b, void* stream) {
  if (busy(h, "vboc_testing_test")) return VBOC_ERR_ARG;
  if (!h || !b) return fail(VBOC_ERR_ARG, "vboc_testing_test: NULL argument");
  const bool cart = h->nq == 2 && h->o.hc, arm = h->nq == 4;
  if (!cart && !arm)
    return fail(VBOC_ERR_UNSUPPORTED, "vboc_testing_test: defined for the UR5 arm (nq = 4) and the Cartesian double "
                                      "pendulum (nq = 2 with the path constraint set)");
  if (cart && !(h->hc_wave && h->wave_hc))
    return fail(VBOC_ERR_UNSUPPORTED, "vboc_testing_test: the Cartesian constraint needs the wave solver (hc_wave)");
  if (b->B < 0) return fail(VBOC_ERR_ARG, "vboc_testing_test: B < 0");
  if (b->B == 0) return VBOC_OK;
  if (b->N_start < 2 || b->N_start + 2 > h->nmax) return fail(VBOC_ERR_ARG, "vboc_testing_test: needs 2 <= N_start < nmax - 1");
  if (!b->ids || !b->rows || !b->row_cnt || !b->stats) return fail(VBOC_ERR_ARG, "vboc_testing_test: NULL array");
  if (!h->coop_ok) return fail(VBOC_ERR_HIP, "vboc_testing_test: wave solver unavailable on this device");
  HIPCHK(hipSetDevice(h->device));
  hipStream_t st = (hipStream_t)stream;
  long long groups = b->B < h->n_regions ? b->B : h->n_regions;
  const long long cap = h->group_cap > 0 ? h->group_cap : (h->mall_mib > 0 ? wave_group_budget(h, b->N_start + 10) : 0);
  if (cap > 0 && groups > cap) groups = cap;
  h->last_groups = groups;
  const int nq = h->nq, NXR = 2 * nq + 1, NU = nq, NP = nq + 1, nm = h->nmax;
  const int st_d = (int)((sizeof(TtState<4>) + 15) / 16 * 2);
  const size_t G = (size_t)groups;
  const size_t dbl = G * ((size_t)(nm + 1) * NXR * 2 + (size_t)nm * NU * 2 + NP + 6 * NXR + 2 * NU + 1 + st_d) + 64;
  const size_t need = dbl * sizeof(double) + 4 * G * sizeof(int) + 256;
  if (need > h->dg_bytes) {
    if (h->dg_scratch) (void)hipFree(h->dg_scratch);
    h->dg_scratch = nullptr;
    h->dg_bytes = 0;
    if (hipMalloc((void**)&h->dg_scratch, need) != hipSuccess)
      return fail(VBOC_ERR_NOMEM, "vboc_testing_test: hipMalloc of the per-problem records");
    h->dg_bytes = need;
  }
  if (!h->tt_jobs && hipMalloc((void**)&h->tt_jobs, sizeof(TtJobs)) != hipSuccess)
    return fail(VBOC_ERR_NOMEM, "vboc_testing_test: hipMalloc of the job descriptor");
  if (!h->dg_in && hipMalloc((void**)&h->dg_in, sizeof(Inputs)) != hipSuccess)
    return fail(VBOC_ERR_NOMEM, "vboc_testing_test: hipMalloc of the batch descriptor");
  double* d = h->dg_scratch;
  auto take = [&](size_t n) { double* r = d; d += (n + 1) & ~(size_t)1; return r; };
  Inputs in;
  in.B = (int)groups; in.nmax = nm; in.head = nullptr;
  in.xg = take(G * (nm + 1) * NXR); in.ug = take(G * nm * NU); in.p = take(G * NP);
  in.lbx = take(G * NXR); in.ubx = take(G * NXR); in.lbu = take(G * NU); in.ubu = take(G * NU);
  in.lbx0 = take(G * NXR); in.ubx0 = take(G * NXR); in.lbxe = take(G * NXR); in.ubxe = take(G * NXR);
  in.xo = take(G * (nm + 1) * NXR); in.uo = take(G * nm * NU); in.cost = take(G);
  TtJobs J;
  J.st = take(G * st_d);
  J.st_doubles = st_d;
  int* ip = (int*)d;
  in.N = ip; ip += G;
  in.status = ip; ip += G;
  in.sqp_iter = ip; ip += G;
  in.qp_iter = ip; ip += G;
  if ((size_t)((char*)ip - (char*)h->dg_scratch) > need) return fail(VBOC_ERR_ARG, "vboc_testing_test: internal size error");
  J.ids = b->ids; J.count = b->B; J.N_start = b->N_start; J.nmax = nm; J.draw_stream = b->draw_stream;
  J.fail_mod = h->dg_fail_mod;
  J.seed = b->seed; J.tol = b->tol; J.dt = b->dt;
  for (int c = 0; c < 8; ++c) { J.xlo[c] = b->xlo[c]; J.xhi[c] = b->xhi[c]; }
  for (int c = 0; c < 4; ++c) J.ulim[c] = b->ulim[c];
  J.rows = b->rows; J.row_cnt = b->row_cnt; J.stats = b->stats;
  J.next = h->head; J.done = h->head + 1; J.err = h->head + 2;
  HIPCHK(hipMemsetAsync(h->head, 0, 256, st));
  HIPCHK(hipEventRecord(h->ev0, st));
  const hipError_t e = arm ? launch_tt<4, false, false>(h, J, in, groups, st) : launch_tt<2, false, true>(h, J, in, groups, st);
  if (e != hipSuccess) return fail(VBOC_ERR_HIP, std::string("vboc_testing_test: ") + hipGetErrorString(e));
  HIPCHK(hipEventRecord(h->ev1, st));
  h->launches = 1;
  h->coop_count = b->B;
  HIPCHK(hipMemcpyAsync(h->host_done, h->head, 14 * sizeof(unsigned), hipMemcpyDeviceToHost, st));
  HIPCHK(hipStreamSynchronize(st));
  const unsigned* c = h->host_done;
  if (c[3]) return fail(VBOC_ERR_ARG, "vboc_testing_test: a horizon passed the handle's nmax");
  if (c[1] != (unsigned)b->B) return fail(VBOC_ERR_HIP, "vboc_testing_test: not every problem finished");
  return VBOC_OK;
}

static int dg_wait(vboc_handle h, vboc_dg_batch_t* b, hipStream_t st) {
  hipError_t e = hipSetDevice(h->device);
  if (e == hipSuccess) e = hipMemcpyAsync(h->host_done, h->head, 14 * sizeof(unsigned), hipMemcpyDeviceToHost, st);
  if (e == hipSuccess) e = hipStreamSynchronize(st);
  h->dg_busy = false;
  if (e != hipSuccess) return fail(VBOC_ERR_HIP, std::string("vboc_data_generation: waiting for the launch: ") + hipGetErrorString(e));
  const unsigned* c = h->host_done;
  b->rows_used = (long long)(((unsigned long long)c[5] << 32) | c[4]);
  b->spec_solves = (long long)(((unsigned long long)c[11] << 32) | c[10]);
  b->spec_used = (long long)(((unsigned long long)c[13] << 32) | c[12]);
  if (c[2]) return fail(VBOC_ERR_NOMEM, "vboc_data_generation: the row pool (rows_cap) overflowed");
  if (c[3]) return fail(VBOC_ERR_HIP, "vboc_data_generation: a horizon exceeded nmax (internal error)");
  if (c[1] != (unsigned)b->B) return fail(VBOC_ERR_HIP, "vboc_data_generation: not every problem finished");
  return VBOC_OK;
}

int vboc_hjr_solve_batch(vboc_handle h, const vboc_hjr_batch_t* b, void* stream) {
  if (busy(h, "vboc_hjr_solve_batch")) return VBOC_ERR_ARG;
  if (!h || !b) return fail(VBOC_ERR_ARG, "vboc_hjr_solve_batch: NULL argument");
  if (h->nq > 3) return fail(VBOC_ERR_UNSUPPORTED, "vboc_hjr_solve_batch: defined for the pendulum chains (nq 1-3)");
  if (b->B < 0) return fail(VBOC_ERR_ARG, "vboc_hjr_solve_batch: B < 0");
  if (b->B == 0) return VBOC_OK;
  if (b->hidden != 100)
    return fail(VBOC_ERR_UNSUPPORTED, "vboc_hjr_solve_batch: NeuralNetCLS hidden size 100 (the reference's) only");
  if (!b->x0 || !b->W0 || !b->b0 || !b->W1 || !b->b1 || !b->W2 || !b->b2 || !b->status || !b->cost || !b->u ||
      !b->x1 || !b->sqp_iter || !b->qp_iter)
    return fail(VBOC_ERR_ARG, "vboc_hjr_solve_batch: NULL array");
  if (!(b->std > 0.0) || !(b->u_max > 0.0)) return fail(VBOC_ERR_ARG, "vboc_hjr_solve_batch: std and u_max must be > 0");
  HIPCHK(hipSetDevice(h->device));
  hipStream_t st = (hipStream_t)stream;
  Opts o;
  default_opts(o);
  o.tol_stat = 1e-6;
  o.qp_tol_stat = 1e-8;
  o.lm = h->nq == 1 ? 1e-2 : 1e-5;
  HjrNet net{b->W0, b->b0, b->W1, b->b1, b->W2, b->b2, b->mean, b->std};
  HjrJobs J{b->B, b->x0, b->u_max, b->status, b->cost, b->u, b->x1, b->sqp_iter, b->qp_iter};
  const dim3 grid((unsigned)((b->B + 63) / 64)), block(64);
  HIPCHK(hipEventRecord(h->ev0, st));
  switch (h->nq) {
    case 1: hipLaunchKernelGGL((k_hjr<1, 100>), grid, block, 0, st, net, o, J); break;
    case 2: hipLaunchKernelGGL((k_hjr<2, 100>), grid, block, 0, st, net, o, J); break;
    default: hipLaunchKernelGGL((k_hjr<3, 100>), grid, block, 0, st, net, o, J); break;
  }
  HIPCHK(hipGetLastError());
  HIPCHK(hipEventRecord(h->ev1, st));
  h->launches = 1;
  return VBOC_OK;
}

int vboc_rk4_batch(int nq, int B, double T, const double* x, const double* u, double* x_out, void* stream) {
  if (nq < 1 || nq > 4 || B < 0) return fail(VBOC_ERR_ARG, "vboc_rk4_batch: bad nq/B");
  if (B == 0) return VBOC_OK;
  if (!x || !u || !x_out) return fail(VBOC_ERR_ARG, "vboc_rk4_batch: NULL array");
  hipStream_t st = (hipStream_t)stream;
  const dim3 grid((B + 255) / 256), block(256);
  switch (nq) {
    case 1: hipLaunchKernelGGL(rk4_kernel<1>, grid, block, 0, st, B, T, x, u, x_out); break;
    case 2: hipLaunchKernelGGL(rk4_kernel<2>, grid, block, 0, st, B, T, x, u, x_out); break;
    case 3: hipLaunchKernelGGL(rk4_kernel<3>, grid, block, 0, st, B, T, x, u, x_out); break;
    default: hipLaunchKernelGGL(rk4_kernel<4>, grid, block, 0, st, B, T, x, u, x_out); break;
  }
  HIPCHK(hipGetLastError());
  return VBOC_OK;
}

int vboc_rk4_sens_batch_host(int nq, int B, double T, const double* x, const double* u, double* x_out, double* A,
                             double* Bm) {
  if (nq < 1 || nq > 4 || B < 0) return fail(VBOC_ERR_ARG, "vboc_rk4_sens_batch_host: bad nq/B");
  if (B == 0) return VBOC_OK;
  const size_t nx = 2 * nq;
  double *dx, *du, *dxo, *dA, *dB;
  HIPCHK(hipMalloc(&dx, B * nx * sizeof(double)));
  HIPCHK(hipMalloc(&du, B * nq * sizeof(double)));
  HIPCHK(hipMalloc(&dxo, B * nx * sizeof(double)));
  HIPCHK(hipMalloc(&dA, B * nx * nx * sizeof(double)));
  HIPCHK(hipMalloc(&dB, B * nx * nq * sizeof(double)));
  HIPCHK(hipMemcpy(dx, x, B * nx * sizeof(double), hipMemcpyHostToDevice));
  HIPCHK(hipMemcpy(du, u, B * nq * sizeof(double), hipMemcpyHostToDevice));
  const dim3 grid((B + 255) / 256), block(256);
  switch (nq) {
    case 1: hipLaunchKernelGGL(rk4_sens_kernel<1>, grid, block, 0, nullptr, B, T, dx, du, dxo, dA, dB); break;
    case 2: hipLaunchKernelGGL(rk4_sens_kernel<2>, grid, block, 0, nullptr, B, T, dx, du, dxo, dA, dB); break;
    case 3: hipLaunchKernelGGL(rk4_sens_kernel<3>, grid, block, 0, nullptr, B, T, dx, du, dxo, dA, dB); break;
    default: hipLaunchKernelGGL(rk4_sens_kernel<4>, grid, block, 0, nullptr, B, T, dx, du, dxo, dA, dB); break;
  }
  HIPCHK(hipGetLastError());
  HIPCHK(hipMemcpy(x_out, dxo, B * nx * sizeof(double), hipMemcpyDeviceToHost));
  HIPCHK(hipMemcpy(A, dA, B * nx * nx * sizeof(double), hipMemcpyDeviceToHost));
  HIPCHK(hipMemcpy(Bm, dB, B * nx * nq * sizeof(double), hipMemcpyDeviceToHost));
  (void)hipFree(dx); (void)hipFree(du); (void)hipFree(dxo); (void)hipFree(dA); (void)hipFree(dB);
  return VBOC_OK;
}

int vboc_rk4_batch_host(int nq, int B, double T, const double* x, const double* u, double* x_out) {
  if (nq < 1 || nq > 4 || B < 0) return fail(VBOC_ERR_ARG, "vboc_rk4_batch_host: bad nq/B");
  if (B == 0) return VBOC_OK;
  const size_t nx = 2 * nq;
  double *dx = nullptr, *du = nullptr, *dxo = nullptr;
  HIPCHK(hipMalloc(&dx, B * nx * sizeof(double)));
  HIPCHK(hipMalloc(&du, B * nq * sizeof(double)));
  HIPCHK(hipMalloc(&dxo, B * nx * sizeof(double)));
  HIPCHK(hipMemcpy(dx, x, B * nx * sizeof(double), hipMemcpyHostToDevice));
  HIPCHK(hipMemcpy(du, u, B * nq * sizeof(double), hipMemcpyHostToDevice));
  int rc = vboc_rk4_batch(nq, B, T, dx, du, dxo, nullptr);
  if (rc == 0) {
    HIPCHK(hipDeviceSynchronize());
    HIPCHK(hipMemcpy(x_out, dxo, B * nx * sizeof(double), hipMemcpyDeviceToHost));
  }
  (void)hipFree(dx);
  (void)hipFree(du);
  (void)hipFree(dxo);
  return rc;
}

}
```

Baseline: 20250.

## Keep per-stage constant vectors and feedforward gains in LDS for triple pendulum

Adds a layout variant for the fused-MFMA triple-pendulum path. In it, the per-stage affine constants c and the feedforward gains k_f live in shared memory rows next to the state vectors, instead of in the global per-stage records. The VBOC_FUSE default widens to enable both, which shrinks the hot record window streamed through the DMA ring and the group budget's hot-bytes estimate. The cost is more LDS per block (wider rows and slack) and separate attribute and size handling for the boundary kernel.

```diff
diff --git a/vboc_amd/csrc/coop.h b/vboc_amd/csrc/coop.h
--- a/vboc_amd/csrc/coop.h
+++ b/vboc_amd/csrc/coop.h
@@ -27,22 +27,38 @@
 #endif
 __host__ __device__ constexpr int rec_up(int v) { return (v + VBOC_REC_ALIGN - 1) / VBOC_REC_ALIGN * VBOC_REC_ALIGN; }
 
-template <int NQ>
+#ifndef VBOC_FUSE
+#define VBOC_FUSE 127
+#endif
+#ifndef VBOC_ACL_FUSED_NQ
+#define VBOC_ACL_FUSED_NQ (1 << 3)
+#endif
+#ifndef VBOC_RINV
+#define VBOC_RINV 1
+#endif
+__host__ __device__ constexpr int lds_vec_mask(int nq, bool fm, bool hc) {
+  return (nq == 3 && fm && !hc && (VBOC_FUSE & 31) == 31 && ((VBOC_ACL_FUSED_NQ >> 3) & 1) && VBOC_RINV) ? ((VBOC_FUSE >> 5) & 3)
+                                                                                                        : 0;
+}
+
+template <int NQ, int LV = 0>
 struct WaveLayout {
   static constexpr int NX = 2 * NQ, NU = NQ, NZ = 3 * NQ, M0 = NQ + 1;
+  static constexpr bool C_LDS = LV & 1, K_LDS = LV & 2;
   static constexpr bool IN_FIRST = NQ <= 3;
   static constexpr int OA = 0, OB = OA + NX * NX, P0 = OB + NX * NU, OE = IN_FIRST ? P0 : P0 + 4 * NZ, OD = OE + NX,
                        ODA = OD + NZ, OZ = IN_FIRST ? ODA + NZ : P0, ODZ = OZ + NZ, OQL = ODZ + NZ, OQU = OQL + NZ,
                        OK = P0 + 6 * NZ + NX, OKF = OK + NU * NX,
                        OLR = IN_FIRST ? OKF + NU + NU * NQ : OKF + NU, OM = IN_FIRST ? OKF + NU : OLR + NU * NU,
-                       OY = OKF + NU + NU * NU + NU * NQ, OPE = OY + NU * NQ, OC = OPE + NX,
-                       OACL = OC + NX, OX = OACL + NX * NX, OU = OX + NX, OPI = OU + NU, OLL = OPI + NX,
-                       OLU = OLL + NZ, OWPI = OLU + NZ, REC = rec_up(OWPI + NX);
+                       OY = OKF + NU + NU * NU + NU * NQ, OPE = OY + NU * NQ, OC = C_LDS ? OPE + NX + NX * NX : OPE + NX,
+                       OACL = C_LDS ? OPE + NX : OC + NX, OX = OPE + 2 * NX + NX * NX, OU = OX + NX, OPI = OU + NU,
+                       OLL = OPI + NX, OLU = OLL + NZ, OWPI = OLU + NZ, REC = rec_up(OWPI + NX);
+  static constexpr int HOT = C_LDS ? OC : OX;
   static_assert((IN_FIRST ? OQU : ODA) + NZ == OK, "the fields before K are A, B, e, D, DA, z, dz, lambda_l, lambda_u");
   static_assert(IN_FIRST ? (OM == OKF + NU && OLR == OM + NU * NQ && OY == OLR + NU * NU)
                          : (OLR == OKF + NU && OM == OLR + NU * NU && OY == OM + NU * NQ), "K, k_f, M / chol(Ru), Y");
-  static constexpr int W_FAC = OC, W_FIN = even_up(ODA), W_FINV = even_up(ODA + NZ), LO_VEC = OPE, W_VEC = OX - OPE,
-                       LO_FWD = OC, W_FWD = OX - OC, W_COS = even_up(OQU + NZ);
+  static constexpr int W_FAC = OPE + NX, W_FIN = even_up(ODA), W_FINV = even_up(ODA + NZ), LO_VEC = OPE,
+                       W_VEC = HOT - OPE, LO_FWD = C_LDS ? OACL : OC, W_FWD = HOT - LO_FWD, W_COS = even_up(OQU + NZ);
   static constexpr int P_FAC = (W_FAC + 127) / 128, P_VEC = (W_VEC + 127) / 128, P_FWD = (W_FWD + 127) / 128,
                        P_COS = (W_COS + 127) / 128;
   static constexpr int P_VMAX = P_VEC > P_FWD ? (P_VEC > P_COS ? P_VEC : P_COS) : (P_FWD > P_COS ? P_FWD : P_COS);
@@ -63,9 +79,12 @@
                        PE0 = Y0 + M0 * NQ, P = PE0 + NX, PA = P + NX * NX, PB = PA + NX * NX, APA = PB + NX * NU,
                        RU = APA + NX * NX, S = RU + NU * NU, PI = S + NU * NX, PV = PI + NX * NQ, DXV = PV + 2 * NX,
                        SC = DXV + 2 * NX, LINE = SC + NQ * NQ, ZERO = LINE + NQ, TRASH = ZERO + 16, PAR = TRASH + 64,
-                       XS = even_up(PAR + Par<NQ>::COUNT);
+                       HU = even_up(PAR + Par<NQ>::COUNT), XS = K_LDS ? HU + 128 : HU;
+  static constexpr int XR = K_LDS ? even_up(NX + NU) : NX, XKF = NX;
   static_assert(M0 * NX <= NX * NX, "stage-0 B'P reuses the PA scratch");
-  static constexpr size_t lds_bytes(int nmax) { return ((size_t)XS + (size_t)(nmax + 1) * NX) * sizeof(double); }
+  static constexpr size_t lds_bytes(int nmax) {
+    return ((size_t)XS + (size_t)(nmax + 1 + (C_LDS ? SLACK : 0)) * XR) * sizeof(double);
+  }
   static constexpr size_t region_doubles(int nmax) { return (size_t)REC * (nmax + 1 + SLACK); }
 };
 
@@ -217,13 +236,13 @@
 
 #define VREP(id, stmt) do { stmt; if constexpr (VBOC_REPEAT == (id)) { stmt; } } while (0)
 
-#ifndef VBOC_FUSE
-#define VBOC_FUSE 31
-#endif
-
-template <int NQ, bool FM = false, bool HC = false>
+
+template <int NQ, bool FM = false, bool HC = false, int LV = lds_vec_mask(NQ, FM, HC)>
 struct Coop {
-  using L = WaveLayout<NQ>;
+  using L = WaveLayout<NQ, LV>;
+  static constexpr bool CLDS = L::C_LDS, KLDS = L::K_LDS;
+  static constexpr int XR = L::XR;
+  __device__ __forceinline__ double& kfr(int k, int a) const { return s[L::XS + k * XR + L::XKF + a]; }
   using HL = Lane<NQ>;
   static_assert(!HC || (!FM && NQ >= 2 && NQ <= 3), "path constraint: pendulum chains, VALU factorisation");
   using PF = Par<NQ>;
@@ -951,16 +970,10 @@
   }
 
   static constexpr int CE = NX + NU, CP = CE + 1;
-#ifndef VBOC_ACL_FUSED_NQ
-#define VBOC_ACL_FUSED_NQ (1 << 3)
-#endif
   static constexpr bool ACL_FUSED = FM && ((VBOC_ACL_FUSED_NQ >> NQ) & 1);
   static constexpr int FJUNK = L::OX;
   static constexpr bool MFMA_OK = (NX <= 8) && (CP + NQ <= 16) && (FJUNK + 2 * NX + 2 <= L::RSF);
   static constexpr int HR0 = NX >> 2;
-#ifndef VBOC_RINV
-#define VBOC_RINV 1
-#endif
   static constexpr bool RINV = VBOC_RINV && FM && NU == 3;
   static constexpr bool VFUSE = FAC1 && ACL_FUSED && RINV && (VBOC_FUSE & 16);
   static_assert(!VFUSE || (L::W_FINV <= OK && L::W_FINV <= 128), "VFUSE: A .. DA in one LDS-DMA, in front of the outputs");
@@ -989,7 +1002,7 @@
 #define FS5(i) if constexpr (FSPL == 5) { SPROF(i) }
     SPROF_DECL(FSPL)
     const int c = t & 15, g = t >> 4;
-    constexpr int HS = L::XS;
+    constexpr int HS = L::HU;
     dbl4 Dm;
     UNR for (int r = 0; r < 4; ++r) {
       const int row = g + 4 * r;
@@ -1046,6 +1059,11 @@
     bool ok = true;
     double pcur = 0.0, kfv = 0.0;
     const int kfo = t < NU ? OKF + t : FJUNK;
+    const int kfx = t < NU ? L::XS + L::XKF + t : L::TRASH + t, kfs = t < NU ? XR : 0;
+    auto kf_out = [&](int sl, int k) {
+      if constexpr (KLDS) s[kfx + k * kfs] = kfv;
+      else s[fslot(sl) + kfo] = kfv;
+    };
     if constexpr (VFUSE) pcur = st(N, ODA + (t < NX ? t : NX - 1));
     auto vstep = [&](int sl) {
       const int kb = fslot(sl);
@@ -1083,7 +1101,7 @@
         vstep((j - 1) % L::NSF);
       } else if constexpr (ACL_FUSED) {
         acl_slot((j - 1) % L::NSF);
-        ring_wb<OK, L::OX>((j - 1) % L::NSF, k + 1);
+        ring_wb<OK, L::HOT>((j - 1) % L::NSF, k + 1);
       } else {
         ring_wb<OK, OC>((j - 1) % L::NSF, k + 1);
       }
@@ -1178,8 +1196,8 @@
       s[kb + pofs + 4] = pg[1];
       if constexpr (VFUSE) {
         if (j >= 1) {
-          s[fslot((j - 1) % L::NSF) + kfo] = kfv;
-          ring_wb<OK, L::OX>((j - 1) % L::NSF, k + 1);
+          kf_out((j - 1) % L::NSF, k + 1);
+          ring_wb<OK, L::HOT>((j - 1) % L::NSF, k + 1);
         }
       }
       lsync();
@@ -1200,11 +1218,11 @@
         if constexpr (VFUSE) {
           acl_slot((j - 1) % L::NSF);
           vstep((j - 1) % L::NSF);
-          s[fslot((j - 1) % L::NSF) + kfo] = kfv;
-          ring_wb<OK, L::OX>((j - 1) % L::NSF, 1);
+          kf_out((j - 1) % L::NSF, 1);
+          ring_wb<OK, L::HOT>((j - 1) % L::NSF, 1);
         } else if constexpr (ACL_FUSED) {
           acl_slot((j - 1) % L::NSF);
-          ring_wb<OK, L::OX>((j - 1) % L::NSF, 1);
+          ring_wb<OK, L::HOT>((j - 1) % L::NSF, 1);
         } else {
           ring_wb<OK, OC>((j - 1) % L::NSF, 1);
         }
@@ -1264,7 +1282,6 @@
     ldr<OK, NKK>(k, kk);
     ldr<OACL, NX * NX / 2>(k, ac);
     ldr<OPE, NX / 2>(k, pe);
-    gdbl2* dst = (gdbl2*)(g + (long long)k * REC + OC);
     double cv[NX];
     UNR for (int i = 0; i < NX; ++i) {
       double c = gv[i];
@@ -1272,6 +1289,11 @@
       UNR for (int q = 0; q < NX; ++q) c += ac[q * NX + i] * pe[q];
       cv[i] = c;
     }
+    if constexpr (CLDS) {
+      UNR for (int i = 0; i < NX; ++i) s[L::XS + k * XR + i] = cv[i];
+      return;
+    }
+    gdbl2* dst = (gdbl2*)(g + (long long)k * REC + OC);
     UNR for (int i = 0; i < NX; i += 2) {
       dbl2 vv;
       vv.x = cv[i];
@@ -1283,6 +1305,7 @@
   __device__ __forceinline__ bool vec(double (&w0)[M0], double (&nun)[NQ]) {
     fresh();
     SPROF_DECL(2)
+    static_assert(!CLDS || (L::S_VEC > 1 && L::S_FWD > 1 && (SWEPT || !PRE)), "CLDS: grouped sweeps, constants by prep_corr");
     if constexpr (PRE && !SWEPT) {
       constexpr int NKK = (NU * NX) / 2;
       for (int k = 1 + t; k < N; k += 64) {
@@ -1326,7 +1349,7 @@
         dma_s(g + (long long)(1 + G * S) * REC, voff, vslot(j & (L::NSV - 1)));
       };
       const int i = t < NX ? t : NX - 1;
-      const int xm = t < NX ? NX : 0, xb = t < NX ? L::XS + t : L::TRASH + t;
+      const int xm = t < NX ? XR : 0, xb = t < NX ? L::XS + t : L::TRASH + t;
       double pv[NX];
       UNR for (int q = 0; q < NX; ++q) pv[q] = rdlane(pcur, q);
       settle();
@@ -1341,7 +1364,8 @@
         const int kb = vslot(j & (L::NSV - 1));
         UNR for (int u = 0; u < S; ++u) {
           UNR for (int q = 0; q < NX; ++q) acl[u][q] = s[kb + u * W + (OACL - OPE) + q * NX + i];
-          cc[u] = s[kb + u * W + (OC - OPE) + i];
+          if constexpr (CLDS) cc[u] = s[L::XS + (1 + G * S + u) * XR + i];
+          else cc[u] = s[kb + u * W + (OC - OPE) + i];
           pe[u] = s[kb + u * W + i];
         }
         __builtin_amdgcn_sched_barrier(0);
@@ -1387,7 +1411,7 @@
       double p0 = cc, p1 = 0.0;
       UNR for (int q = 0; q < NX; q += 2) p0 += acl[q] * pv[q];
       UNR for (int q = 1; q < NX; q += 2) p1 += acl[q] * pv[q];
-      if (t < NX) s[L::XS + k * NX + t] = pe + pcur;
+      if (t < NX) s[L::XS + k * XR + t] = pe + pcur;
       pcur = p0 + p1;
       UNR for (int q = 0; q < NX; ++q) pv[q] = rdlane(pcur, q);
       UNR for (int q = 0; q < NX; ++q) acl[q] = an[q];
@@ -1406,7 +1430,11 @@
       constexpr int F0_ = OKF & ~1, NF = (OKF + NU - F0_ + 1) / 2, Y0_ = OY & ~1, NY = (OPE - Y0_ + 1) / 2;
       for (int k = 1 + t; k < N; k += 64) {
         double kf[2 * NF], yy[2 * NY];
-        ldr<F0_, NF>(k, kf);
+        if constexpr (KLDS) {
+          UNR for (int a = 0; a < NU; ++a) kf[(OKF - F0_) + a] = kfr(k, a);
+        } else {
+          ldr<F0_, NF>(k, kf);
+        }
         ldr<Y0_, NY>(k, yy);
         __builtin_amdgcn_sched_barrier(0);
         UNR for (int j = 0; j < NQ; ++j)
@@ -1424,7 +1452,7 @@
       double r[NU], Lm[NU * NU];
       UNR for (int a = 0; a < NU; ++a) {
         double x = gg.v[gg.OFF + a];
-        UNR for (int i = 0; i < NX; ++i) x += bb[i * NU + a] * s[L::XS + k * NX + i];
+        UNR for (int i = 0; i < NX; ++i) x += bb[i * NU + a] * s[L::XS + k * XR + i];
         r[a] = x;
       }
       UNR for (int e = 0; e < NU * NU; ++e) Lm[e] = ly[LR_ + e];
@@ -1440,7 +1468,8 @@
       }
       UNR for (int a = 0; a < NU; ++a) {
         r[a] = -r[a];
-        st(k, OKF + a) = r[a];
+        if constexpr (KLDS) kfr(k, a) = r[a];
+        else st(k, OKF + a) = r[a];
       }
       UNR for (int j = 0; j < NQ; ++j)
         UNR for (int a = 0; a < NU; ++a) lin[j] += ly[Y_ + a * NQ + j] * r[a];
@@ -1499,29 +1528,32 @@
       if (t < NX) {
         double x = rs * st(0, OE + t);
         UNR for (int a = 0; a < M0; ++a) x += s[L::F0 + t * M0 + a] * w0[a];
-        s[L::XS + NX + t] = x;
+        s[L::XS + XR + t] = x;
         s[L::DXV + t] = x;
       }
     }
     W3(0)
     {
-      constexpr int NBB = (NX * NU + 1) / 2, NFM = (OM + NU * NQ - OKF + 1) / 2;
+      constexpr int NBB = (NX * NU + 1) / 2, FB = KLDS ? (OM & ~1) : OKF, NFM = (OM + NU * NQ - FB + 1) / 2;
       for (int k = 1 + t; k < N; k += 64) {
         double e[NX], bb[2 * NBB], fm[2 * NFM];
         ldr<OE, NX / 2>(k, e);
         ldr<OB, NBB>(k, bb);
-        ldr<OKF, NFM>(k, fm);
+        ldr<FB, NFM>(k, fm);
+        double kf0[NU];
+        UNR for (int a = 0; a < NU; ++a) kf0[a] = KLDS ? kfr(k, a) : 0.0;
         __builtin_amdgcn_sched_barrier(0);
         double kfm[NU];
         UNR for (int a = 0; a < NU; ++a) {
-          double x = fm[a];
-          UNR for (int j = 0; j < NQ; ++j) x -= fm[(OM - OKF) + a * NQ + j] * nun[j];
+          double x = KLDS ? kf0[a] : fm[a];
+          UNR for (int j = 0; j < NQ; ++j) x -= fm[(OM - FB) + a * NQ + j] * nun[j];
           kfm[a] = x;
         }
-        if constexpr (KFM) {
+        if constexpr (KLDS) {
+          UNR for (int a = 0; a < NU; ++a) kfr(k, a) = kfm[a];
+        } else if constexpr (KFM) {
           UNR for (int a = 0; a < NU; ++a) st(k, OKF + a) = kfm[a];
         }
-        gdbl2* dst = (gdbl2*)(g + (long long)k * REC + OC);
         UNR for (int i = 0; i < NX; i += 2) {
           double v[2];
           UNR for (int h2 = 0; h2 < 2; ++h2) {
@@ -1529,10 +1561,16 @@
             UNR for (int a = 0; a < NU; ++a) c += bb[(i + h2) * NU + a] * kfm[a];
             v[h2] = c;
           }
-          dbl2 vv;
-          vv.x = v[0];
-          vv.y = v[1];
-          dst[i / 2] = vv;
+          if constexpr (CLDS) {
+            s[L::XS + (k + 1) * XR + i] = v[0];
+            s[L::XS + (k + 1) * XR + i + 1] = v[1];
+          } else {
+            gdbl2* dst = (gdbl2*)(g + (long long)k * REC + OC);
+            dbl2 vv;
+            vv.x = v[0];
+            vv.y = v[1];
+            dst[i / 2] = vv;
+          }
         }
       }
       __syncthreads();
@@ -1549,7 +1587,7 @@
         dma_s(g + (long long)(1 + G * S) * REC, voff, vslot(j & (L::NSV - 1)));
       };
       const int i = t < NX ? t : NX - 1;
-      const int xm = t < NX ? NX : 0, xb = t < NX ? L::XS + NX + t : L::TRASH + t;
+      const int xm = t < NX ? XR : 0, xb = t < NX ? L::XS + XR + t : L::TRASH + t;
       double dx[NX];
       UNR for (int q = 0; q < NX; ++q) dx[q] = s[L::DXV + q];
       settle();
@@ -1562,8 +1600,9 @@
         vmwait<L::DV>();
         const int kb = vslot(j & (L::NSV - 1));
         UNR for (int u = 0; u < S; ++u) {
-          UNR for (int q = 0; q < NX; ++q) acl[u][q] = s[kb + u * W + (OACL - OC) + i * NX + q];
-          cc[u] = s[kb + u * W + i];
+          UNR for (int q = 0; q < NX; ++q) acl[u][q] = s[kb + u * W + (OACL - L::LO_FWD) + i * NX + q];
+          if constexpr (CLDS) cc[u] = s[L::XS + (2 + j * S + u) * XR + i];
+          else cc[u] = s[kb + u * W + i];
         }
         __builtin_amdgcn_sched_barrier(0);
         UNR for (int u = 0; u < S; ++u) {
@@ -1609,7 +1648,7 @@
         UNR for (int q = 0; q < NX; q += 2) p0 += acl[q] * dx[q];
         UNR for (int q = 1; q < NX; q += 2) p1 += acl[q] * dx[q];
         const double dn = p0 + p1;
-        if (t < NX) s[L::XS + (k + 1) * NX + t] = dn;
+        if (t < NX) s[L::XS + (k + 1) * XR + t] = dn;
         UNR for (int q = 0; q < NX; ++q) dx[q] = rdlane(dn, q);
         UNR for (int q = 0; q < NX; ++q) acl[q] = an[q];
         cc = cn;
@@ -1621,7 +1660,7 @@
     W6(4)
     typename Lane<NQ>::MinRatio mr{1.0, CORR ? o.tau : 1.0};
     double a0 = 0.0, a1 = 0.0, a2 = 0.0;
-    constexpr int NKM = KFM ? (OKF + NU - OK + 1) / 2 : (OY - OK + 1) / 2;
+    constexpr int NKM = KLDS ? (OKF - OK + 1) / 2 : KFM ? (OKF + NU - OK + 1) / 2 : (OY - OK + 1) / 2;
     for (int k = t; k <= N; k += 64) {
       IP r;
       double km[2 * NKM];
@@ -1637,11 +1676,12 @@
       if (k == 0) {
         UNR for (int i = 0; i < NZ; ++i) d[i] = rec[OT + i];
       } else {
-        UNR for (int i = 0; i < NX; ++i) d[i] = s[L::XS + k * NX + i];
+        UNR for (int i = 0; i < NX; ++i) d[i] = s[L::XS + k * XR + i];
         UNR for (int a = 0; a < NU; ++a) {
           double x = 0.0;
           if (k < N) {
-            x = km[OKF - OK + a];
+            if constexpr (KLDS) x = kfr(k, a);
+            else x = km[OKF - OK + a];
             if constexpr (!KFM) {
               UNR for (int j = 0; j < NQ; ++j) x -= km[OM - OK + a * NQ + j] * nun[j];
             }
@@ -1761,7 +1801,7 @@
       const double dz = st(N, ODZ + i);
       const double lam = o.lm * dz - st(N, OQL + i) + st(N, OQU + i) +
                          (i >= NQ ? par(PF::QNU + (i >= NQ ? i - NQ : 0)) : 0.0);
-      s[L::XS + (N - 1) * NX + i] = lam;
+      s[L::XS + (N - 1) * XR + i] = lam;
       s[L::DXV + i] = lam;
       fin = isfinite(dz);
     }
@@ -1801,7 +1841,7 @@
       const double x = p0 + p1;
       if (t < NX) {
         s[wb + t] = x;
-        s[L::XS + (k - 1) * NX + t] = x;
+        s[L::XS + (k - 1) * XR + t] = x;
       }
       UNR for (int q = 0; q < NX; ++q) ac[q] = an[q];
       cc = cn;
@@ -1809,7 +1849,7 @@
     }
     __syncthreads();
     for (int k = t; k < N; k += 64) {
-      UNR for (int i = 0; i < NX; ++i) st(k, ODA + i) = s[L::XS + k * NX + i];
+      UNR for (int i = 0; i < NX; ++i) st(k, ODA + i) = s[L::XS + k * XR + i];
     }
     __syncthreads();
     return fin;
@@ -2040,7 +2080,7 @@
 void k_wave(Work w, Opts o, Inputs in, SlotState ss, WaveJobs jb) {
   extern __shared__ __attribute__((aligned(16))) double smem[];
   const int t = (int)threadIdx.x;
-  Coop<NQ, FM, HC> C(smem, gptr(jb.regions) + (long long)blockIdx.x * jb.region_doubles, w, o, t);
+  Coop<NQ, FM, HC, 0> C(smem, gptr(jb.regions) + (long long)blockIdx.x * jb.region_doubles, w, o, t);
   if constexpr (HC) C.gh = gptr(jb.hc) + (long long)blockIdx.x * jb.hc_doubles;
   for (;;) {
     unsigned idx = 0;
@@ -2096,7 +2136,7 @@
       atomicAdd(ss.done, 1u);
     }
   }
-  if constexpr (NQ == 3 && FM && !HC && Coop<NQ, FM, HC>::VFUSE) asm volatile(".rept 96\n\ts_nop 0\n\t.endr");
+  if constexpr (NQ == 3 && FM && !HC && Coop<NQ, FM, HC, 0>::VFUSE) asm volatile(".rept 96\n\ts_nop 0\n\t.endr");
 }
 
 __global__ void k_list(SlotState ss, int* list, unsigned* cnt) {
diff --git a/vboc_amd/csrc/vboc_solver.hip b/vboc_amd/csrc/vboc_solver.hip
--- a/vboc_amd/csrc/vboc_solver.hip
+++ b/vboc_amd/csrc/vboc_solver.hip
@@ -1367,6 +1367,7 @@
   long long n_regions = 0, region_doubles = 0, group_cap = 0;
   double mall_mib = 256.0;
   size_t wave_lds = 0;
+  size_t wave_lds_lv = 0;
   bool coop_ok = false;
   long long coop_count = 0;
   double* ft_regions = nullptr;
@@ -1513,9 +1514,12 @@
   return hipGetLastError() == hipSuccess ? 0 : -2;
 }
 
-static long long wave_group_budget(const vboc_solver* h, int nmax) {
-  const long long hot = (long long)(h->nq == 1 ? WaveLayout<1>::OX
-                                    : (h->nq == 2 ? WaveLayout<2>::OX : (h->nq == 3 ? WaveLayout<3>::OX : WaveLayout<4>::OX))) *
+static long long wave_group_budget(const vboc_solver* h, int nmax, bool dg) {
+  const bool lv = dg && h->nq == 3 && h->factor_mfma;
+  const long long hot = (long long)(h->nq == 1 ? WaveLayout<1>::HOT
+                                    : (h->nq == 2 ? WaveLayout<2>::HOT
+                                       : (h->nq == 3 ? (lv ? WaveLayout<3, lds_vec_mask(3, true, false)>::HOT : WaveLayout<3>::HOT)
+                                                     : WaveLayout<4>::HOT))) *
                         (long long)(nmax + 1) * (long long)sizeof(double);
   const long long g = (long long)(0.92 * h->mall_mib * 1024.0 * 1024.0) / (hot > 0 ? hot : 1);
   return g < 256 ? 256 : g;
@@ -1524,7 +1528,7 @@
 static hipError_t launch_wave(vboc_solver* h, const WaveJobs& jb, long long jobs, hipStream_t st, const Work& w,
                               const Inputs& in, const SlotState& ss) {
   long long groups = jobs < h->n_regions ? jobs : h->n_regions;
-  const long long cap = h->group_cap > 0 ? h->group_cap : (h->mall_mib > 0 ? wave_group_budget(h, in.nmax) : 0);
+  const long long cap = h->group_cap > 0 ? h->group_cap : (h->mall_mib > 0 ? wave_group_budget(h, in.nmax, false) : 0);
   if (cap > 0 && groups > cap) groups = cap;
   if (groups < 1) return hipSuccess;
   h->last_groups = groups;
@@ -1553,8 +1557,9 @@
                            bool testing = false) {
   const void* fn = testing ? (const void*)k_ts<NQ, FM> : (const void*)k_dg<NQ, FM>;
   bool& attr = h->dg_attr[(FM ? 1 : 0) + (testing ? 2 : 0)];
+  const size_t lds = lds_vec_mask(NQ, FM, false) ? h->wave_lds_lv : h->wave_lds;
   if (!attr) {
-    hipError_t e = hipFuncSetAttribute(fn, hipFuncAttributeMaxDynamicSharedMemorySize, (int)h->wave_lds);
+    hipError_t e = hipFuncSetAttribute(fn, hipFuncAttributeMaxDynamicSharedMemorySize, (int)lds);
     if (e != hipSuccess) return e;
     attr = true;
   }
@@ -1564,10 +1569,10 @@
   if (e == hipSuccess) e = hipStreamSynchronize(st);
   if (e != hipSuccess) return e;
   if (testing)
-    hipLaunchKernelGGL((k_ts<NQ, FM>), dim3((unsigned)groups), dim3(64), h->wave_lds, st, h->w, h->o, in,
+    hipLaunchKernelGGL((k_ts<NQ, FM>), dim3((unsigned)groups), dim3(64), lds, st, h->w, h->o, in,
                        (const Inputs*)h->dg_in, (const DgJobs*)h->dg_jobs, jb);
   else
-    hipLaunchKernelGGL((k_dg<NQ, FM>), dim3((unsigned)groups), dim3(64), h->wave_lds, st, h->w, h->o, in,
+    hipLaunchKernelGGL((k_dg<NQ, FM>), dim3((unsigned)groups), dim3(64), lds, st, h->w, h->o, in,
                        (const Inputs*)h->dg_in, (const DgJobs*)h->dg_jobs, jb);
   return hipGetLastError();
 }
@@ -1645,6 +1650,7 @@
     h->wave_lds = nq == 1 ? WaveLayout<1>::lds_bytes(nmax)
                           : (nq == 2 ? WaveLayout<2>::lds_bytes(nmax)
                                      : (nq == 3 ? WaveLayout<3>::lds_bytes(nmax) : WaveLayout<4>::lds_bytes(nmax)));
+    h->wave_lds_lv = nq == 3 ? WaveLayout<3, lds_vec_mask(3, true, false)>::lds_bytes(nmax) : h->wave_lds;
     h->region_doubles = nq == 1 ? (long long)WaveLayout<1>::region_doubles(nmax)
                                 : (nq == 2 ? (long long)WaveLayout<2>::region_doubles(nmax)
                                            : (nq == 3 ? (long long)WaveLayout<3>::region_doubles(nmax)
@@ -1660,7 +1666,7 @@
     if (cus < 1) cus = 256;
     h->n_regions = (long long)per_cu * cus;
     if (h->n_regions > 16384) h->n_regions = 16384;
-    if (h->wave_lds > 160 * 1024) h->n_regions = 0;
+    if (h->wave_lds > 160 * 1024 || h->wave_lds_lv > 160 * 1024) h->n_regions = 0;
     h->coop_ok = h->n_regions > 0 &&
                  hipFuncSetAttribute(fn, hipFuncAttributeMaxDynamicSharedMemorySize, (int)h->wave_lds) == hipSuccess &&
                  hipMalloc((void**)&h->regions, sizeof(double) * (size_t)h->region_doubles * (size_t)h->n_regions) ==
@@ -2299,7 +2305,7 @@
   HIPCHK(hipSetDevice(h->device));
   long long groups = b->B < h->n_regions ? b->B : h->n_regions;
   const long long cap = h->group_cap > 0 ? h->group_cap
-                                         : (h->mall_mib > 0 ? wave_group_budget(h, b->N_start + 10) : 0);
+                                         : (h->mall_mib > 0 ? wave_group_budget(h, b->N_start + 10, true) : 0);
   if (cap > 0 && groups > cap) groups = cap;
   h->last_groups = groups;
   const int nq = h->nq, NXR = 2 * nq + 1, NU = nq, NP = nq + 1, NX = 2 * nq, nm = h->nmax;
@@ -2454,7 +2460,7 @@
   HIPCHK(hipSetDevice(h->device));
   hipStream_t st = (hipStream_t)stream;
   long long groups = b->B < h->n_regions ? b->B : h->n_regions;
-  const long long cap = h->group_cap > 0 ? h->group_cap : (h->mall_mib > 0 ? wave_group_budget(h, b->N_start + 10) : 0);
+  const long long cap = h->group_cap > 0 ? h->group_cap : (h->mall_mib > 0 ? wave_group_budget(h, b->N_start + 10, false) : 0);
   if (cap > 0 && groups > cap) groups = cap;
   h->last_groups = groups;
   const int nq = h->nq, NXR = 2 * nq + 1, NU = nq, NP = nq + 1, nm = h->nmax;
```

After: 21520, median of 6. 1.06x the previous value.
